# Daniel-Lin-S/decode_tonal_langauge

Hardware: AMD Instinct MI355X
Metric: mel-frames/sec (train step) SynthesisModelCNN, 128ch x 400t batch256 (higher is better)
Workload: dtype f32; 1 GPU; SynthesisModelCNN 128ch x 400t -> 80 mel, 4 tones x 2 syllables, L=5, global batch 256 (strong scaling: 256 windows on rank 0), dropout 0.5, NAdam, 1,376,768,720 params; per_gpu_batch=256, global_batch=256, parallelism=dp1, init=drawn on every rank

## Files before the change

decode_tonal_langauge_amd/_cnn_engine.py:

```python
from __future__ import annotations

import ctypes as C
import os
import math
from typing import Dict, List, Optional

import torch

from . import _kernels, _lib
from ._lib import (EPI_C1WGRAD, EPI_GY, EPI_LRELU, EPI_MASK, EPI_MASKY, EPI_POOL, EPI_POOLV, EPI_STORE, LOAD_DIRECT, LOAD_UNPOOL, LOAD_V,
                   LOAD_Y, NtParams, TnParams, check, ptr)


def _r4(n: int) -> int:
    return (n + 3) // 4 * 4


class _Stage:

    def __init__(self, idx, cin, cout, k, pool, tin, tp_in):
        self.idx, self.cin, self.cout, self.k, self.pool = idx, cin, cout, k, pool
        self.tin, self.tp_in = tin, tp_in
        self.tc = tin - k + 1
        self.tout = self.tc // 2 if pool else self.tc
        self.tp_out = tp_in // 2 if pool else tp_in


class CnnEngine:
    F63_CAPABLE = True

    def __init__(self, output_dim: int, n_channels: int, n_timepoints: int, lstm_channels: int,
                 conv_channels: int, dropout: float, negative_slope: float, stage_defs, concat_widths):
        if negative_slope < 0:
            raise ValueError("the MI355X path needs negative_slope >= 0 (max-pool / LeakyReLU are fused)")
        self.lib = _lib.load()
        self.out_dim = output_dim
        self.C = n_channels
        self.T = n_timepoints
        self.Lc = lstm_channels
        self.Cc = conv_channels
        self.p_drop = float(dropout)
        self.slope = float(negative_slope)
        self.cslope = 0.1
        k1 = stage_defs[0][1]
        npool_after = sum(1 for s in stage_defs[1:] if s[2])
        tc1 = n_timepoints - k1 + 1
        self.k1 = k1
        self.c1 = stage_defs[0][0]
        self.tout1 = tc1 // 2
        if not stage_defs[0][2]:
            raise ValueError("first stage must pool")
        align = 1 << npool_after
        self.tp1 = max(align, (self.tout1 + align - 1) // align * align)
        _kernels.validate()
        self.wino63 = (self.F63_CAPABLE and _kernels.get("wino") == "6"
                       and self._f63_covers(stage_defs, n_timepoints))
        tp1_default = self.tp1
        if self.wino63:
            self.tp1 = (self.tout1 + 11) // 12 * 12
        self.f63_yprod = (self.wino63 and _kernels.get("f63_yprod") != "0" and stage_defs[0][0] % 256 == 0
                          and self.tp1 >= 12)
        self.f63_yprod3 = (self.wino63 and _kernels.get("f63_yprod") != "0" and stage_defs[1][0] % 256 == 0)
        self.stages: List[_Stage] = []
        cin, tin, tp = self.c1, self.tout1, self.tp1
        for i, (cout, k, pool) in enumerate(stage_defs[1:], start=2):
            st = _Stage(i, cin, cout, k, pool, tin, tp)
            if st.tout < 1:
                raise ValueError("n_timepoints too small for the conv stack")
            if self.wino63 and i == 3:
                st.tp_out = tp1_default // 4
            self.stages.append(st)
            cin, tin, tp = cout, st.tout, st.tp_out
        self.gy4 = self._gy_applies()
        self.lat = tin
        self.tp5 = tp
        self.H = self.lat * n_channels * lstm_channels
        self.ld5 = _r4(conv_channels)
        self.ldx = _r4(conv_channels + lstm_channels)
        self.concat_dims = []
        cin_t, cin_ld = conv_channels + lstm_channels, self.ldx
        for w in concat_widths:
            self.concat_dims.append((cin_t, cin_ld, w, _r4(w)))
            cin_t, cin_ld = w, _r4(w)
        self.ldy5 = self.concat_dims[-1][3]
        self.kflat = n_channels * self.tp5 * self.ldy5
        self.ldd = _r4(output_dim)
        self.lowrank_param = "label_lstm.weight_hh_l0"
        self.lstm_shard = None
        self._sh = None
        self.timers = None
        mode = _kernels.get("wino")
        self.wino43 = mode != "0"
        self.store_p1 = _kernels.get("store_p1") == "1"
        self.fuse_c1 = True
        self.wino_vout = True
        self.tn_bm = 0
        self._side = None
        self._B = None
        self.generation = 0
        self._saved_generation = -1

    def _alloc(self, B: int, dev):
        if self._B == B and self._dev == dev:
            return
        self._B, self._dev = B, dev
        S = B * self.C
        self.S = S
        f32 = dict(dtype=torch.float32, device=dev)
        z = lambda *s: torch.zeros(*s, **f32)
        zi = lambda *s: torch.zeros(*s, dtype=torch.int32, device=dev)
        self._v_ready = {}
        self._gy_A = None
        self._vhalo = {}
        self.P = {}
        if not (self.wino63 or self._conv1_writes_v()) or self.store_p1:
            self.P[1] = z(S * self.tp1, self.c1)
        self.bits = {1: zi(S * self.tp1, self.c1 // 32)}
        self.sbits = {1: zi(S * self.tp1, self.c1 // 32)}
        for st in self.stages:
            rows = S * st.tp_out
            ld = st.cout if st.pool else self.ld5
            no_rows = (self.wino63 and st.idx == 2) or (self._writes_v(st) and not self._f63(st))
            if not no_rows or self.store_p1:
                self.P[st.idx] = z(rows, ld)
            if st.pool:
                self.bits[st.idx] = zi(rows, st.cout // 32)
                self.sbits[st.idx] = zi(rows, st.cout // 32)
        rows5 = S * self.tp5
        self.rows5 = rows5
        self.Xc = z(rows5, self.ldx)
        self.Y = [z(rows5, d[3]) for d in self.concat_dims]
        self.out_slab = None
        self.Yt = {}
        self._y_ready = {}
        self.V = {}
        self.Vd = {}
        self._vd_ready = {}
        self.G = None

    def _alloc_bwd(self):
        if self.G is not None:
            return
        dev = self._dev
        f32 = dict(dtype=torch.float32, device=dev)
        z = lambda *s: torch.zeros(*s, **f32)
        S = self.S
        self.G = {}
        if not self.wino63 and not (self.fuse_c1 and self._c1_fusable() and self._v43(self.stages[0])):
            self.G[1] = z(S * self.tp1, self.c1)
        for st in self.stages:
            if not (self.f63_yprod and st.idx == 2) and not (self.gy4 and st.idx == 3):
                self.G[st.idx] = z(S * st.tp_out, st.cout if st.pool else self.ld5)
        self.GY = [z(self.rows5, d[3]) for d in self.concat_dims]
        self.dXc = z(self.rows5, self.ldx)

    def _side_stream(self, dev):
        if self._side is None or self._side.device != dev:
            self._side = torch.cuda.Stream(device=dev)
        return self._side

    def _stream(self):
        return torch.cuda.current_stream().cuda_stream

    def enable_timers(self, on: bool = True):
        self.timers = {} if on else None

    def _tick(self, name):
        if getattr(self, "timers", None) is None or name is None:
            return None
        ev = (torch.cuda.Event(enable_timing=True), torch.cuda.Event(enable_timing=True))
        self.timers.setdefault(name, []).append(ev)
        ev[0].record()
        return ev

    def timer_summary(self):
        torch.cuda.synchronize()
        out = {}
        for k, evs in (self.timers or {}).items():
            ms = [a.elapsed_time(b) for a, b in evs]
            out[k] = (len(ms), sum(ms) / max(len(ms), 1))
        return out

    def _permute(self, src, dst, dims, strides, lims=None, nz=1, zs=0, src_off=0, bias=None):
        d = (C.c_int64 * 4)(*dims)
        s = (C.c_int64 * 4)(*strides)
        l = (C.c_int64 * 4)(*(lims if lims is not None else dims))
        check(self.lib.tl_permute_reduce(src.data_ptr() + 4 * src_off, dst.data_ptr(), d, s, l, nz, zs, ptr(bias),
                                         self._stream()), "tl_permute_reduce")

    def _nt(self, tag=None, fn="tl_gemm_nt_window", **kw):
        p = NtParams()
        p.splitk, p.bm, p.J, p.Tp, p.slope = 1, 128, 1, 1, 0.0
        for k, v in kw.items():
            setattr(p, k, v)
        ev = self._tick(tag)
        check(getattr(self.lib, fn)(C.byref(p), self._stream()), fn)
        if ev:
            ev[1].record()

    def _tn(self, tag=None, fn="tl_gemm_tn_window", **kw):
        p = TnParams()
        p.splitk, p.J, p.Tp, p.Tvalid = 1, 1, 1, 1
        for k, v in kw.items():
            setattr(p, k, v)
        ev = self._tick(tag)
        check(getattr(self.lib, fn)(C.byref(p), self._stream()), fn)
        if ev:
            ev[1].record()

    @staticmethod
    def _splitk(tiles: int, ksteps: int, target: int = 2048) -> int:
        return int(max(1, min(ksteps, (target + tiles - 1) // tiles, 1024)))

    @staticmethod
    def _splitk_rounds(tiles: int, ksteps: int, slots: int = 512, max_sk: int = 32, min_rounds: float = 1.9) -> int:
        cands = []
        for sk in range(1, max(1, min(max_sk, ksteps)) + 1):
            n = tiles * sk
            cands.append((sk, n, n / (-(-n // slots) * slots)))
        full = [c for c in cands if c[2] >= 0.95]
        for sk, n, _ in full:
            if n >= min_rounds * slots:
                return sk
        if full:
            return full[-1][0]
        return max(cands, key=lambda c: c[2])[0]

    def _pack_conv(self, w, cin_ld, flip_for_dgrad):
        O, I, J, _ = w.shape
        if not flip_for_dgrad:
            dst = torch.empty(J, O, cin_ld, dtype=torch.float32, device=w.device)
            self._permute(w, dst, (1, J, O, cin_ld), (0, 1, I * J, J), (1, J, O, I))
            return dst
        old = _r4(O)
        dst = torch.empty(J, cin_ld, old, dtype=torch.float32, device=w.device)
        self._permute(w, dst, (1, J, cin_ld, old), (0, -1, J, I * J), (1, J, I, O), src_off=J - 1)
        return dst


    @staticmethod
    def _f63_covers(stage_defs, T) -> bool:
        if len(stage_defs) < 4:
            return False
        (c1, k1, p1), (c2, k2, p2), (c3, k3, p3) = stage_defs[0], stage_defs[1], stage_defs[2]
        tout1 = (T - k1 + 1) // 2
        tout2 = (tout1 - 2) // 2
        tout3 = (tout2 - 2) // 2
        return (p1 and p2 and p3 and k2 == 3 and k3 == 3 and 1 <= k1 <= 3 and c1 in (128, 256, 512, 1024)
                and c2 % 128 == 0 and c3 % 64 == 0 and tout3 >= 1 and T >= 2 * tout1 + 2)

    def _f63(self, st) -> bool:
        return self.wino63 and st.idx in (2, 3)

    def _nt63_rows(self) -> int:
        return int(self.lib.tl_wino63_nt_tile_rows())

    def _v_hex_buffer(self, store, idx, rows, cin):
        nh = rows // 6
        nh_pad = (nh + 24 + 127) // 128 * 128
        V = store.get(idx)
        if V is None or V.shape[0] != nh_pad or V.shape[1] != 8 or V.shape[2] != cin:
            V = store[idx] = torch.zeros(nh_pad, 8, cin, dtype=torch.float32, device=self._dev)
        return V

    def _pack_wino63(self, w, forward: bool):
        O, I = w.shape[0], w.shape[1]
        dst = torch.empty(8, O, I, dtype=torch.float32, device=w.device) if forward else \
            torch.empty(8, I, O, dtype=torch.float32, device=w.device)
        check(self.lib.tl_wino63_weights(ptr(w), ptr(dst) if forward else None, None if forward else ptr(dst), O, I, I, O,
                                         self._stream()), "tl_wino63_weights")
        return dst

    def f63_issue_factor(self, st) -> float:
        return (st.tp_in // 6) * 8.0 / (st.tc * 3.0)

    def _stage_forward63(self, st, w, bia) -> None:
        S = self.S
        wp = self._pack_wino63(w, True)
        V = self._v_ready[st.idx - 1]
        if st.idx == 2 and self.store_p1 and 2 not in self.P:
            self.P[2] = torch.zeros(S * st.tp_out, st.cout, dtype=torch.float32, device=self._dev)
        Pout = self.P.get(st.idx) if (st.idx != 2 or self.store_p1) else None
        kw = dict(A=ptr(V), A_rows=V.shape[0], lda=V.shape[2], loader=LOAD_V, Bw=ptr(wp), bias=ptr(bia), out=ptr(Pout),
                  M=S * st.tp_in, N=st.cout, K=st.cin, ldb=st.cin, ldo=Pout.shape[1] if Pout is not None else st.cout, J=3,
                  row_shift=0, Tp=st.tp_in, slope=self.slope, obits=ptr(self.bits[st.idx]), osign=ptr(self.sbits[st.idx]),
                  ld_obits=st.cout // 32, Tvalid=2 * st.tout)
        if st.idx == 2:
            rows_out = S * st.tp_out
            Vn = self._v_hex_buffer(self.V, 2, rows_out, st.cout)
            ntm = -(-(S * st.tp_in) // self._nt63_rows())
            if not hasattr(self, "_vhalo"):
                self._vhalo = {}
            halo = self._vhalo.get(2)
            if halo is None or halo.shape[0] != ntm or halo.shape[2] != st.cout:
                halo = self._vhalo[2] = torch.zeros(ntm, 2, st.cout, dtype=torch.float32, device=self._dev)
            kw.update(epilogue=EPI_POOLV, vout=ptr(Vn), vhalo=ptr(halo), vout_quads=Vn.shape[0], ld_vout=Vn.shape[2])
            self._nt(tag="conv2_fwd", fn="tl_conv3_wino63v_nt", **kw)
            check(self.lib.tl_wino63_v_fixup(ptr(Vn), ptr(halo), rows_out // 6, ntm, st.tp_out, st.cout, Vn.shape[2],
                                             self._stream()), "tl_wino63_v_fixup")
            self._v_ready[2] = Vn
        else:
            if Pout is None:
                raise RuntimeError("F(6,3) stage 3 writes pooled rows: its output buffer was not allocated")
            kw.update(epilogue=EPI_POOL, out_tp=st.tp_out)
            self._nt(tag="conv3_fwd", fn="tl_conv3_wino63v_nt", **kw)

    def _stage_wgrad63(self, st, gw, gb) -> None:
        S = self.S
        f32 = dict(dtype=torch.float32, device=self._dev)
        rows_in = S * st.tp_in
        nd = st.cout
        ldg = nd
        V = self._v_ready[st.idx - 1]
        tiles = (st.cin // 64) * (nd // 64)
        sk = self._splitk(tiles, (rows_in + 35) // 36, 4096)
        slab = torch.empty(sk, 8 * st.cin, ldg, **f32)
        bias_part = torch.empty(sk, nd, **f32)
        if (st.idx == 3 and self.f63_yprod3 and self._y_ready.get(3) != self.generation):
            Gs = self.G[3]
            Y3 = self._v_hex_buffer(self.Yt, 3, rows_in, nd)
            Vd3 = self._v_hex_buffer(self.Vd, 3, rows_in, nd)
            ev = self._tick("conv3_yvd")
            check(self.lib.tl_wino63_unpool_yvd(ptr(Gs), ptr(self.bits[3]), ptr(Y3), ptr(Vd3), rows_in, Gs.shape[0], st.tp_in,
                                                st.tp_out, 2 * st.tout, nd, Gs.shape[1], st.cout // 32, nd, self._stream()),
                  "tl_wino63_unpool_yvd")
            if ev:
                ev[1].record()
            self._y_ready[3] = self.generation
            self._vd_ready[3] = self.generation
        if self._y_ready.get(st.idx) == self.generation:
            Y = self.Yt[st.idx]
            self._y_ready[st.idx] = -1
            self._tn(tag=f"conv{st.idx}_wgrad", fn="tl_conv3_wino63v_tn", A=ptr(V), B=ptr(Y), slab=ptr(slab), Krows=rows_in,
                     A_rows=V.shape[0], B_rows=Y.shape[0], Mdim=st.cin, Ndim=nd, lda=V.shape[2], ldb=Y.shape[2], ldc=ldg, J=3,
                     Tp=st.tp_in, splitk=sk, slab_stride=8 * st.cin * ldg, loader=LOAD_Y, Tvalid=2 * st.tout,
                     colsum=ptr(bias_part))
        else:
            Gs = self.G[st.idx]
            Vd = self._v_hex_buffer(self.Vd, st.idx, rows_in, nd)
            self._tn(tag=f"conv{st.idx}_wgrad", fn="tl_conv3_wino63v_tn", A=ptr(V), B=ptr(Gs), slab=ptr(slab), Krows=rows_in,
                     A_rows=V.shape[0], B_rows=Gs.shape[0], Mdim=st.cin, Ndim=nd, lda=V.shape[2], ldb=Gs.shape[1], ldc=ldg, J=3,
                     Tp=st.tp_in, splitk=sk, slab_stride=8 * st.cin * ldg, loader=LOAD_UNPOOL, bbits=ptr(self.bits[st.idx]),
                     ld_bbits=st.cout // 32, Tvalid=2 * st.tout, colsum=ptr(bias_part), vd=ptr(Vd), ld_vd=nd, g_tp=st.tp_out)
            self._vd_ready[st.idx] = self.generation
        if sk > 1:
            red = torch.empty(8 * st.cin, ldg, **f32)
            n = 8 * st.cin * ldg
            self._permute(slab, red, (1, 1, 1, n), (0, 0, 0, 1), nz=sk, zs=n)
        else:
            red = slab
        check(self.lib.tl_wino63_wgrad_finalize(ptr(red), ptr(gw), st.cout, st.cin, ldg, self._stream()),
              "tl_wino63_wgrad_finalize")
        self._permute(bias_part, gb, (1, 1, 1, st.cout), (0, 0, 0, 1), nz=sk, zs=nd)

    def _gy_stage(self, st) -> bool:
        return self.gy4 and st.idx == 4

    def _gy_applies(self) -> bool:
        if not (self.wino63 and self.f63_yprod3 and len(self.stages) >= 3):
            return False
        below, st = self.stages[1], self.stages[2]
        return (_kernels.get("conv4_dgrad") == "nt63" and st.k == 1 and st.pool and self._f63(below)
                and st.cout % 32 == 0 and st.cout >= 40 and st.cin % 32 == 0 and (below.tp_in // 2) % 3 == 0)

    def _stage_dgrad_gy(self, st, w):
        S = self.S
        below = self.stages[1]
        tpg = below.tp_in // 2
        rows = S * tpg
        f32 = dict(dtype=torch.float32, device=self._dev)
        nh = -(-rows // 6)
        nh_pad = (nh + 127) // 128 * 128
        A = getattr(self, "_gy_A", None)
        if A is None or A.shape[0] != nh_pad or A.shape[2] != st.cout:
            A = self._gy_A = torch.zeros(nh_pad, 8, st.cout, **f32)
        Gs = self.G[st.idx]
        ev = self._tick(f"conv{st.idx}_dgrad")
        check(self.lib.tl_wino63_unpool_rows6(ptr(Gs), ptr(self.bits[st.idx]), ptr(A), rows, Gs.shape[0], tpg, st.tp_out,
                                              2 * st.tout, st.cout, Gs.shape[1], st.cout // 32, st.cout, 0, self._stream()),
              "tl_wino63_unpool_rows6")
        taps = torch.empty(st.cout // 8, 8, st.cin, 8, **f32)
        check(self.lib.tl_wino63_weights1(ptr(w), ptr(taps), st.cout, st.cin, st.cout, self._stream()), "tl_wino63_weights1")
        rows3 = S * below.tp_in
        Y3 = self._v_hex_buffer(self.Yt, below.idx, rows3, below.cout)
        Vd3 = self._v_hex_buffer(self.Vd, below.idx, rows3, below.cout)
        ntm = -(-rows // self._nt63_rows())
        if not hasattr(self, "_vhalo"):
            self._vhalo = {}
        halo = self._vhalo.get("d3")
        if halo is None or halo.shape[0] != ntm or halo.shape[2] != below.cout:
            halo = self._vhalo["d3"] = torch.zeros(ntm, 2, below.cout, **f32)
        self._nt(tag=None, fn="tl_conv1_wino63v_dgrad_nt", A=ptr(A), A_rows=A.shape[0], lda=A.shape[2], loader=LOAD_V,
                 Bw=ptr(taps), M=rows, N=st.cin, K=st.cout, ldb=st.cout, ldo=st.cin, J=1, row_shift=0, Tp=tpg, slope=self.slope,
                 auxbits=ptr(self.sbits[below.idx]), ld_auxbits=self.sbits[below.idx].shape[1], abits=ptr(self.bits[below.idx]),
                 ld_abits=below.cout // 32, out_tp=below.tp_out, Tvalid_in=2 * below.tout, epilogue=EPI_GY, out=None,
                 vout=ptr(Y3), vout2=ptr(Vd3), vhalo=ptr(halo), vout_quads=Y3.shape[0], ld_vout=Y3.shape[2])
        check(self.lib.tl_wino63_vd_fixup(ptr(Vd3), ptr(halo), rows // 3, ntm, below.tp_in // 6, below.cout, Vd3.shape[2],
                                          self._stream()), "tl_wino63_vd_fixup")
        if ev:
            ev[1].record()
        self._y_ready[below.idx] = self.generation
        self._vd_ready[below.idx] = self.generation
        return None

    def _stage_dgrad63(self, st, w):
        S = self.S
        rows_in = S * st.tp_in
        if self._vd_ready.get(st.idx) != self.generation:
            raise RuntimeError("F(6,3) input gradient: the stage's weight-gradient pass (which writes Vd) must run first")
        self._vd_ready[st.idx] = -1
        Vd = self.Vd[st.idx]
        wd = self._pack_wino63(w, False)
        kw = dict(A=ptr(Vd), A_rows=Vd.shape[0], lda=Vd.shape[2], loader=LOAD_V, Bw=ptr(wd), M=rows_in, N=st.cin,
                  K=st.cout, ldb=st.cout, ldo=st.cin, J=3, row_shift=-2, Tp=st.tp_in, slope=self.slope,
                  auxbits=ptr(self.sbits[st.idx - 1]), ld_auxbits=self.sbits[st.idx - 1].shape[1])
        if st.idx == 3 and self.f63_yprod:
            below = self.stages[0]
            rows2 = S * below.tp_in
            Y2 = self._v_hex_buffer(self.Yt, 2, rows2, below.cout)
            Vd2 = self._v_hex_buffer(self.Vd, 2, rows2, below.cout)
            ntm = -(-rows_in // self._nt63_rows())
            if not hasattr(self, "_vhalo"):
                self._vhalo = {}
            halo = self._vhalo.get("d2")
            if halo is None or halo.shape[0] != ntm or halo.shape[2] != below.cout:
                halo = self._vhalo["d2"] = torch.zeros(ntm, 2, below.cout, dtype=torch.float32, device=self._dev)
            self._nt(tag="conv3_dgrad", fn="tl_conv3_wino63v_nt", epilogue=EPI_MASKY, out=None, vout=ptr(Y2), vout2=ptr(Vd2),
                     vhalo=ptr(halo), vout_quads=Y2.shape[0], ld_vout=Y2.shape[2], abits=ptr(self.bits[2]),
                     ld_abits=below.cout // 32, Tvalid_in=2 * below.tout, **kw)
            check(self.lib.tl_wino63_vd_fixup(ptr(Vd2), ptr(halo), rows_in // 3, ntm, below.tp_in // 6, below.cout, Vd2.shape[2],
                                              self._stream()), "tl_wino63_vd_fixup")
            self._y_ready[2] = self.generation
            self._vd_ready[2] = self.generation
            return None
        if st.idx == 3:
            self._nt(tag="conv3_dgrad", fn="tl_conv3_wino63v_nt", epilogue=EPI_MASK, out=ptr(self.G[2]), **kw)
            return None
        ntm = -(-rows_in // self._nt63_rows())
        part = torch.empty(ntm, (self.k1 + 1) * self.c1, dtype=torch.float32, device=self._dev)
        self._nt(tag="conv2_dgrad", fn="tl_conv3_wino63v_nt", epilogue=EPI_C1WGRAD, out=None, c1x=ptr(self._x),
                 c1bits=ptr(self.bits[1]), c1partial=ptr(part), c1T=self.T, c1kt=self.k1, Tvalid=self.tout1, **kw)
        return part

    def _c1_fusable(self) -> bool:
        return self.k1 <= 3 and self.T >= 2 * self.tout1 + 2

    def _v43(self, st) -> bool:
        return (self.wino43 and st.k == 3 and st.pool and st.cin % 64 == 0 and st.cout % 32 == 0 and st.tp_in % 4 == 0
                and _r4(st.cout) % 16 == 0)

    def _tn_bm(self, st) -> int:
        wide = st.cin % 128 == 0
        dma8 = wide and _r4(st.cout) % 64 == 0 and (st.cout // 32) % 2 == 0
        if self.tn_bm == 127:
            return 127 if wide else 64
        if self.tn_bm in (0, 128):
            return 128 if dma8 else 64
        return 64

    def _conv1_writes_v(self) -> bool:
        return (self._v43(self.stages[0]) and self.tp1 % 4 == 0 and self.c1 in (128, 256, 512, 1024)
                and (self.fuse_c1 and self._c1_fusable()))

    def _writes_v(self, st) -> bool:
        if not (self.wino_vout and st.pool and st.idx - 1 < len(self.stages)):
            return False
        nxt = self.stages[st.idx - 1]
        return self._v43(st) and self._v43(nxt) and st.tp_in % 8 == 0 and nxt.cin == st.cout

    def _pin(self, st):
        return self.P.get(st.idx - 1)

    def _v_buffer(self, idx, rows, cin):
        nq = rows // 4
        nq_pad = (nq + 127) // 128 * 128
        V = self.V.get(idx)
        if V is None or V.shape[0] != nq_pad or V.shape[2] != cin:
            V = self.V[idx] = torch.zeros(nq_pad, 6, cin, dtype=torch.float32, device=self._dev)
        return V

    def _input_transform(self, st):
        src = self.P[st.idx - 1]
        V = self._v_buffer(st.idx - 1, src.shape[0], st.cin)
        ev = self._tick(f"conv{st.idx}_xform")
        check(self.lib.tl_wino43_input_transform(ptr(src), ptr(V), src.shape[0], st.tp_in, st.cin, src.shape[1], st.cin,
                                                 self._stream()), "tl_wino43_input_transform")
        if ev:
            ev[1].record()
        return V

    def wgrad_issue_factor(self, st) -> float:
        if self._f63(st):
            return self.f63_issue_factor(st)
        return 0.5 if self._v43(st) else 1.0

    def kernel_families(self):
        if self.wino63:
            self._fam_share = {}
            st2, st3 = self.stages[0], self.stages[1]
            f6 = "Winograd F(6,3) on pre-transformed operands, LDS-DMA"
            tn = "wino63v_tn4_kernel<true>" if st3.cin % 256 == 0 and st3.tp_in >= 12 else "wino63v_tn_kernel<true>"
            tn2 = "wino63v_tn4_kernel<true>" if st2.cin % 256 == 0 else "wino63v_tn_kernel<true>"
            fams = {f"wino63v_nt_kernel<POOLV> (conv2 forward, {f6}; writes V of its pooled output for conv3)": ["conv2_fwd"],
                    f"wino63v_nt_kernel<POOL> (conv3 forward, {f6})": ["conv3_fwd"],
                    f"wino63v_nt_kernel<C1WGRAD> (conv2 input gradient + conv1 weight gradient, {f6})": ["conv2_dgrad"],
                    }
            if self.f63_yprod3:
                gy = self.gy4
                src = "the epilogue of conv4's input gradient" if gy else "wino63_unpool_yvd_kernel"
                fams[f"wino63v_tn4y_kernel (conv3 weight gradient, {f6}: both operands by LDS-DMA, no transform in the kernel; Y3 / Vd3 "
                     f"from {src})"] = ["conv3_wgrad"]
            else:
                fams[f"{tn} (conv3 weight gradient, {f6}; also writes Vd)"] = ["conv3_wgrad"]
            if self.f63_yprod:
                fams[f"wino63v_nt_kernel<MASKY> (conv3 input gradient, {f6}; writes Y and Vd of conv2 instead of the gradient rows)"] = ["conv3_dgrad"]
                fams[f"wino63v_tn4y_kernel (conv2 weight gradient, {f6}: both operands by LDS-DMA, no transform in the kernel)"] = ["conv2_wgrad"]
            else:
                fams[f"wino63v_nt_kernel<MASK> (conv3 input gradient, {f6})"] = ["conv3_dgrad"]
                fams[f"{tn2} (conv2 weight gradient, {f6}; also writes Vd)"] = ["conv2_wgrad"]
            issued = {k: self.f63_issue_factor(st2 if "conv2" in k else st3) for k in fams}
            return fams, issued
        self._fam_share = {}
        if not all(self._v43(st) for st in self.stages[:2]):
            fams = {"nt_window_kernel<128,UNPOOL,MASK> (conv input-gradient)": ["conv2_dgrad", "conv3_dgrad", "conv4_dgrad"],
                    "nt_window_kernel<128,DIRECT,POOL> (conv forward)": ["conv2_fwd", "conv3_fwd", "conv4_fwd"],
                    "tn3_kernel<UNPOOL> (conv weight-gradient)": ["conv2_wgrad", "conv3_wgrad"]}
            return fams, {k: 1.0 for k in fams}
        form = "Winograd F(4,3) on pre-transformed operands, LDS-DMA"
        fused = self.fuse_c1 and self._c1_fusable()
        bm = self._tn_bm(self.stages[0])
        extra = {}
        if bm == 128:
            tn = f"wino43v_tn8_kernel<true> (conv2/conv3 weight gradient, {form}; also writes Vd for the input gradient)"
        else:
            ntm = (self.stages[0].cin + 63) // 64
            tn = f"wino43v_tn_kernel<false, 2> (conv2/conv3 weight gradient, C_in tiles 1..{ntm - 1} of {ntm}, {form})"
            vdn = f"wino43v_tn_kernel<true, 2> (conv2/conv3 weight gradient, C_in tile 0 of {ntm}, {form}, + writes Vd for the input gradient)"
            extra[vdn] = ["conv2_wgrad_vd", "conv3_wgrad_vd"]
            self._fam_share = {tn: (ntm - 1) / ntm, vdn: 1.0 / ntm}
        fams = {tn: ["conv2_wgrad", "conv3_wgrad"]}
        if self._writes_v(self.stages[0]):
            fams[f"wino43v_nt_kernel<POOLV> (conv2 forward, {form}; writes V of its pooled output for conv3 instead of the raw rows)"] = ["conv2_fwd"]
            fams[f"wino43v_nt_kernel<POOL> (conv3 forward, {form})"] = ["conv3_fwd"]
        else:
            fams[f"wino43v_nt_kernel<POOL> (conv2/conv3 forward, {form})"] = ["conv2_fwd", "conv3_fwd"]
        fams.update(extra)
        if fused:
            fams[f"wino43v_nt_kernel<UNPOOL,C1WGRAD> (conv2 input gradient + conv1 weight gradient, {form})"] = ["conv2_dgrad"]
            fams[f"wino43v_nt_kernel<UNPOOL,MASK> (conv3 input gradient, {form})"] = ["conv3_dgrad"]
        else:
            fams[f"wino43v_nt_kernel<UNPOOL,MASK> (conv2/conv3 input gradient, {form})"] = ["conv2_dgrad", "conv3_dgrad"]
        return fams, {k: 0.5 for k in fams}

    def _pack_wino43(self, w, forward: bool):
        O, I = w.shape[0], w.shape[1]
        dst = torch.empty(6, O, I, dtype=torch.float32, device=w.device) if forward else \
            torch.empty(6, I, O, dtype=torch.float32, device=w.device)
        check(self.lib.tl_wino43_weights(ptr(w), ptr(dst) if forward else None, None if forward else ptr(dst), O, I, I, O,
                                         self._stream()), "tl_wino43_weights")
        return dst

    STAGE_NAMES = {2: "ecog_conv_block.3", 3: "ecog_conv_block.6", 4: "ecog_conv_block.9", 5: "ecog_conv_block.12"}

    def stage_forward(self, st: _Stage, w: torch.Tensor, bia: torch.Tensor) -> None:
        if self._f63(st):
            return self._stage_forward63(st, w, bia)
        S = self.S
        v43 = self._v43(st)
        wp = self._pack_wino43(w, True) if v43 else self._pack_conv(w, st.cin, False)
        src = self._pin(st)
        vout = self._writes_v(st)
        if vout and self.store_p1 and st.idx not in self.P:
            self.P[st.idx] = torch.zeros(S * st.tp_out, st.cout, dtype=torch.float32, device=self._dev)
        Pout = self.P.get(st.idx) if (not vout or self.store_p1) else None
        kw = dict(A=ptr(src), Bw=ptr(wp), bias=ptr(bia), out=ptr(Pout), M=S * st.tp_in,
                  A_rows=S * st.tp_in, N=st.cout, K=st.cin, lda=st.cin, ldb=st.cin,
                  ldo=Pout.shape[1] if Pout is not None else st.cout, J=st.k, row_shift=0, Tp=st.tp_in, slope=self.slope,
                  loader=LOAD_DIRECT)
        if st.pool:
            kw.update(epilogue=EPI_POOL, obits=ptr(self.bits[st.idx]), osign=ptr(self.sbits[st.idx]),
                      ld_obits=st.cout // 32, Tvalid=2 * st.tout)
        else:
            kw.update(epilogue=EPI_LRELU, Tvalid=st.tout)
        if not v43:
            self._nt(tag=f"conv{st.idx}_fwd", fn="tl_gemm_nt_window", **kw)
            return
        V = self._v_ready.get(st.idx - 1)
        if V is None:
            V = self._v_ready[st.idx - 1] = self._input_transform(st)
        kw.update(A=ptr(V), A_rows=V.shape[0], lda=V.shape[2], loader=LOAD_V)
        if vout:
            rows_out = S * st.tp_out
            Vn = self._v_buffer(st.idx, rows_out, st.cout)
            ntm = (S * st.tp_in + 511) // 512
            halo = self._vhalo.get(st.idx)
            if halo is None or halo.shape[0] != ntm or halo.shape[2] != st.cout:
                halo = self._vhalo[st.idx] = torch.zeros(ntm, 2, st.cout, dtype=torch.float32, device=self._dev)
# ... 22 lines not shown
            flat = part.view(-1)
            for c0 in range(0, zs, 1024):
                nc = min(1024, zs - c0)
                self._colsum(flat[c0:], nblk, nc, zs, 1, 1, red[c0:c0 + nc])
            self._permute(red, gw, (1, 1, self.c1, self.k1), (0, 0, 1, self.c1))
            self._permute(red, gb, (1, 1, 1, self.c1), (0, 0, 0, 1), src_off=self.k1 * self.c1)
        else:
            self._permute(part, gw, (1, 1, self.c1, self.k1), (0, 0, 1, self.c1), nz=nblk, zs=zs)
            self._permute(part, gb, (1, 1, 1, self.c1), (0, 0, 0, 1), nz=nblk, zs=zs, src_off=self.k1 * self.c1)

    def stage_wgrad(self, st: _Stage, gw: torch.Tensor, gb: torch.Tensor) -> None:
        if self._f63(st):
            return self._stage_wgrad63(st, gw, gb)
        S = self.S
        f32 = dict(dtype=torch.float32, device=self._dev)
        Xin = self._pin(st)
        Gs = self.G[st.idx]
        rows_in = S * st.tp_in
        ldg = Gs.shape[1]
        nd = _r4(st.cout)
        if self._v43(st):
            tiles = ((st.cin + 63) // 64) * ((nd + 63) // 64)
            bm = self._tn_bm(st)
            sk = self._splitk(tiles, (rows_in + 31) // 32, 4096 if bm in (127, 128) else 8192)
            slab = torch.empty(sk, 6 * st.cin, ldg, **f32)
            bias_part = torch.empty(sk, nd, **f32)
            V = self._v_ready.get(st.idx - 1)
            if V is None:
                V = self._v_ready[st.idx - 1] = self._input_transform(st)
            nq_pad = (rows_in // 4 + 127) // 128 * 128
            Vd = self.Vd.get(st.idx)
            if Vd is None or Vd.shape[0] != nq_pad or Vd.shape[2] != nd:
                Vd = self.Vd[st.idx] = torch.zeros(nq_pad, 6, nd, **f32)
            kw = dict(A=ptr(V), B=ptr(Gs), slab=ptr(slab), Krows=rows_in, A_rows=V.shape[0], B_rows=Gs.shape[0],
                      Mdim=st.cin, Ndim=nd, lda=V.shape[2], ldb=ldg, ldc=ldg, J=3, Tp=st.tp_in, splitk=sk,
                      slab_stride=6 * st.cin * ldg, loader=LOAD_UNPOOL, bbits=ptr(self.bits[st.idx]),
                      ld_bbits=st.cout // 32, Tvalid=2 * st.tout, colsum=ptr(bias_part), bm=bm, vd=ptr(Vd), ld_vd=nd)
            self._vd_ready[st.idx] = self.generation
            if self.timers is not None and bm != 128:
                self._tn(tag=f"conv{st.idx}_wgrad_vd", fn="tl_conv3_wino43v_tn", part=1, **kw)
                self._tn(tag=f"conv{st.idx}_wgrad", fn="tl_conv3_wino43v_tn", part=2, **kw)
            else:
                self._tn(tag=f"conv{st.idx}_wgrad", fn="tl_conv3_wino43v_tn", **kw)
            if sk > 1:
                red = torch.empty(6 * st.cin, ldg, **f32)
                n = 6 * st.cin * ldg
                self._permute(slab, red, (1, 1, 1, n), (0, 0, 0, 1), nz=sk, zs=n)
            else:
                red = slab
            check(self.lib.tl_wino43_wgrad_finalize(ptr(red), ptr(gw), st.cout, st.cin, ldg, self._stream()),
                  "tl_wino43_wgrad_finalize")
            self._permute(bias_part, gb, (1, 1, 1, st.cout), (0, 0, 0, 1), nz=sk, zs=nd)
            return
        if st.k == 3:
            tiles = ((st.cin + 127) // 128) * ((nd + 63) // 64)
        else:
            tiles = st.k * ((st.cin + 127) // 128) * ((nd + 127) // 128)
        sk = self._splitk(tiles, (rows_in + 31) // 32, 1024)
        slab = torch.empty(sk, st.k * st.cin, ldg, **f32)
        kw = dict(A=ptr(Xin), B=ptr(Gs), slab=ptr(slab), Krows=rows_in, A_rows=Xin.shape[0], B_rows=Gs.shape[0],
                  Mdim=st.cin, Ndim=nd, lda=st.cin, ldb=ldg, ldc=ldg, J=st.k, Tp=st.tp_in, splitk=sk,
                  slab_stride=st.k * st.cin * ldg)
        if st.pool:
            kw.update(loader=LOAD_UNPOOL, bbits=ptr(self.bits[st.idx]), ld_bbits=st.cout // 32, Tvalid=2 * st.tout)
        else:
            kw.update(loader=LOAD_DIRECT, Tvalid=st.tout)
        fold = (not st.pool) and st.k == 1 and rows_in > 512 and st.cin > 32
        bpart = torch.empty(sk, nd, **f32) if fold else None
        if fold:
            kw.update(colsum=ptr(bpart))
        self._tn(tag=f"conv{st.idx}_wgrad", **kw)
        if sk > 1:
            red = torch.empty(st.k * st.cin, ldg, **f32)
            n = st.k * st.cin * ldg
            self._permute(slab, red, (1, 1, 1, n), (0, 0, 0, 1), nz=sk, zs=n)
        else:
            red = slab
        self._permute(red, gw, (1, st.cout, st.cin, st.k), (0, 1, ldg, st.cin * ldg))
        if fold:
            self._permute(bpart, gb, (1, 1, 1, st.cout), (0, 0, 0, 1), nz=sk, zs=nd)
        else:
            self._colsum(Gs, Gs.shape[0], st.cout, ldg, st.tp_out, st.tout, gb)

    def stage_dgrad(self, st: _Stage, w: torch.Tensor):
        if self._f63(st):
            return self._stage_dgrad63(st, w)
        if self._gy_stage(st):
            return self._stage_dgrad_gy(st, w)
        S = self.S
        Xin = self._pin(st)
        Gs = self.G[st.idx]
        rows_in = S * st.tp_in
        ldg = Gs.shape[1]
        v43 = self._v43(st)
        wd = self._pack_wino43(w, False) if v43 else self._pack_conv(w, st.cin, True)
        kd = wd.shape[2]
        fuse = st.idx == 2 and v43 and self.fuse_c1 and self._c1_fusable()
        kw = dict(A=ptr(Gs), Bw=ptr(wd), aux=ptr(Xin), out=None if fuse else ptr(self.G[st.idx - 1]), M=rows_in,
                  A_rows=Gs.shape[0], N=st.cin, K=kd, lda=ldg, ldb=kd, ldo=st.cin, ldaux=st.cin, J=st.k,
                  row_shift=-(st.k - 1), Tp=st.tp_in, epilogue=EPI_MASK, slope=self.slope)
        if (st.idx - 1) in self.sbits:
            kw.update(auxbits=ptr(self.sbits[st.idx - 1]), ld_auxbits=self.sbits[st.idx - 1].shape[1])
        if st.pool:
            kw.update(loader=LOAD_UNPOOL, abits=ptr(self.bits[st.idx]), ld_abits=st.cout // 32,
                      Tvalid_in=2 * st.tout)
        else:
            kw.update(loader=LOAD_DIRECT)
        if not v43:
            self._nt(tag=f"conv{st.idx}_dgrad", fn="tl_gemm_nt_window", **kw)
            return None
        part = None
        if fuse:
            ntm = (rows_in + 511) // 512
            part = torch.empty(ntm, (self.k1 + 1) * self.c1, dtype=torch.float32, device=self._dev)
            kw.update(epilogue=EPI_C1WGRAD, out=None, c1x=ptr(self._x), c1bits=ptr(self.bits[1]), c1partial=ptr(part),
                      c1T=self.T, c1kt=self.k1, Tvalid=self.tout1)
        if self._vd_ready.get(st.idx) != self.generation or st.idx not in self.Vd:
            raise RuntimeError("F(4,3) input gradient: the stage's weight-gradient pass (which writes Vd) must run first")
        Vd = self.Vd[st.idx]
        kw.update(A=ptr(Vd), A_rows=Vd.shape[0], lda=Vd.shape[2], loader=LOAD_V)
        self._vd_ready[st.idx] = -1
        self._nt(tag=f"conv{st.idx}_dgrad", fn="tl_conv3_wino43v_nt", **kw)
        return part

    def _lstm_forward(self, prm, xu, U, L, dev, training, label_table) -> None:
        lib, st_ = self.lib, self._stream()
        H = self.H
        f32 = dict(dtype=torch.float32, device=dev)
        self._act = torch.empty(L, U, 4 * H, **f32)
        self._c = torch.empty(L, U, H, **f32)
        self._h = torch.empty(L, U, H, **f32)
        hh = torch.empty(U, 4 * H, **f32) if L > 1 else None
        w_ih, w_hh = prm["label_lstm.weight_ih_l0"], prm["label_lstm.weight_hh_l0"]
        b_ih, b_hh = prm["label_lstm.bias_ih_l0"], prm["label_lstm.bias_hh_l0"]
        bm = 32 if U <= 64 else 128
        self._sh = None
        if (self.lstm_shard is not None and label_table is not None and training and L > 1 and (L - 1) * U <= 64
                and (4 * H) % (4 * self.lstm_shard[1]) == 0):
            rk, wd = self.lstm_shard
            self._sh = (rk * (4 * H // wd), 4 * H // wd, wd)
        nloc = self._sh[1] if self._sh else 4 * H
        sk_f = self._splitk_rounds(((U + bm - 1) // bm) * ((nloc + 127) // 128), (H + 31) // 32, min_rounds=8.9) if L > 1 else 1
        slab_f = torch.empty(sk_f, U, nloc, **f32) if sk_f > 1 else None
        if self._sh:
            from . import parallel
            hh_loc = torch.empty(U, nloc, **f32)
            hh_all = torch.empty(self._sh[2], U, nloc, **f32)
        for t in range(L):
            if t > 0 and self._sh:
                r0, R, wd = self._sh
                self._nt(A=ptr(self._h[t - 1]), Bw=w_hh.data_ptr() + 4 * r0 * H, out=ptr(slab_f if sk_f > 1 else hh_loc),
                         M=U, A_rows=U, N=R, K=H, lda=H, ldb=H, ldo=R, loader=LOAD_DIRECT, epilogue=EPI_STORE, bm=bm,
                         splitk=sk_f, slab_stride=U * R)
                if sk_f > 1:
                    self._permute(slab_f, hh_loc, (1, 1, 1, U * R), (0, 0, 0, 1), nz=sk_f, zs=U * R)
                parallel.all_gather_blocks(hh_all, hh_loc)
                self._permute(hh_all, hh, (1, U, wd, R), (0, R, U * R, 1))
            elif t > 0:
                self._nt(A=ptr(self._h[t - 1]), Bw=ptr(w_hh), out=ptr(slab_f if sk_f > 1 else hh), M=U, A_rows=U,
                         N=4 * H, K=H, lda=H, ldb=H, ldo=4 * H, loader=LOAD_DIRECT, epilogue=EPI_STORE, bm=bm,
                         splitk=sk_f, slab_stride=U * 4 * H)
                if sk_f > 1:
                    n = U * 4 * H
                    self._permute(slab_f, hh, (1, 1, 1, n), (0, 0, 0, 1), nz=sk_f, zs=n)
            check(lib.tl_lstm_cell_fwd(ptr(hh) if t > 0 else None, ptr(xu[t]), ptr(w_ih), ptr(b_ih), ptr(b_hh),
                                       ptr(self._c[t - 1]) if t > 0 else None, ptr(self._act[t]), ptr(self._c[t]),
                                       ptr(self._h[t]), U, H, 2, 4 * H, st_), "tl_lstm_cell_fwd")

    def forward(self, prm: Dict[str, torch.Tensor], x: torch.Tensor, labels: torch.Tensor, training: bool,
# ... 212 lines not shown
        for i in range(len(self.concat_dims) - 1, -1, -1):
            order += [f"concat_conv_block.{2 * i}.weight", f"concat_conv_block.{2 * i}.bias"]
        order += ["label_lstm.weight_ih_l0", "label_lstm.bias_ih_l0", "label_lstm.bias_hh_l0"]
        for st in reversed(self.stages):
            order += [self.STAGE_NAMES[st.idx] + ".weight", self.STAGE_NAMES[st.idx] + ".bias"]
        order += ["ecog_conv_block.0.weight", "ecog_conv_block.0.bias"]
        return order

    def backward(self, prm: Dict[str, torch.Tensor], dout: torch.Tensor, grads: Dict[str, torch.Tensor],
                 gather_whh=None, whh_factors: bool = False, reduce_rows=None, on_factors=None, on_grad_ready=None) -> None:
        self.whh_factors = None
        if self._saved_generation != self.generation:
            raise RuntimeError("SynthesisModelCNN backward: the forward intermediates were overwritten by a later "
                               "forward pass (one forward/backward pair at a time per model)")
        self._alloc_bwd()
        lib, st_ = self.lib, self._stream()
        B, S, dev = self._B, self.S, self._dev
        f32 = dict(dtype=torch.float32, device=dev)
        H, U, L = self.H, self._U, self._L
        rows5 = self.rows5

        colsum = self._colsum

        gw = grads["output_layer.weight"]
        slab = torch.empty(self.ldd, self.kflat, **f32)
        self._tn(A=ptr(dout), B=ptr(self.Y[-1]), slab=ptr(slab), Krows=B, A_rows=B, B_rows=B, Mdim=self.ldd,
                 Ndim=self.kflat, lda=self.ldd, ldb=self.kflat, ldc=self.kflat, loader=LOAD_DIRECT)
        latC = self.lat * self.C
        self._permute(slab, gw, (self.out_dim, self.Cc, self.lat, self.C),
                      (self.kflat, 1, self.ldy5, self.tp5 * self.ldy5))
        colsum(dout, B, self.out_dim, self.ldd, 1, 1, grads["output_layer.bias"])
        if on_grad_ready is not None:
            on_grad_ready("output_layer")
        wpt = torch.empty(self.kflat, self.ldd, **f32)
        self._permute(prm["output_layer.weight"], wpt, (self.C, self.tp5, self.ldy5, self.ldd),
                      (1, self.C, latC, self.Cc * latC), (self.C, self.lat, self.Cc, self.out_dim))
        self._nt(A=ptr(dout), Bw=ptr(wpt), aux=ptr(self.Y[-1]), out=ptr(self.GY[-1]), M=B, A_rows=B, N=self.kflat,
                 K=self.ldd, lda=self.ldd, ldb=self.ldd, ldo=self.kflat, ldaux=self.kflat, loader=LOAD_DIRECT,
                 epilogue=EPI_MASK, slope=self.cslope)
        del wpt
        for i in range(len(self.concat_dims) - 1, -1, -1):
            cin_t, cin_ld, cout_t, cout_ld = self.concat_dims[i]
            src = self.Xc if i == 0 else self.Y[i - 1]
            Gi = self.GY[i]
            name = f"concat_conv_block.{2 * i}"
            tiles = ((cin_ld + 127) // 128) * ((cout_ld + 127) // 128)
            sk = self._splitk(tiles, (rows5 + 31) // 32, 512)
            slab = torch.empty(sk, cin_ld, cout_ld, **f32)
            fold = rows5 > 512 and cin_ld > 32
            bpart = torch.empty(sk, cout_ld, **f32) if fold else None
            self._tn(A=ptr(src), B=ptr(Gi), slab=ptr(slab), Krows=rows5, A_rows=rows5, B_rows=rows5, Mdim=cin_ld,
                     Ndim=cout_ld, lda=cin_ld, ldb=cout_ld, ldc=cout_ld, loader=LOAD_DIRECT, Tp=self.tp5,
                     Tvalid=self.lat, splitk=sk, slab_stride=cin_ld * cout_ld, colsum=ptr(bpart))
            self._permute(slab, grads[name + ".weight"], (1, 1, cout_t, cin_t), (0, 0, 1, cout_ld), nz=sk,
                          zs=cin_ld * cout_ld)
            if fold:
                self._permute(bpart, grads[name + ".bias"], (1, 1, 1, cout_t), (0, 0, 0, 1), nz=sk, zs=cout_ld)
            else:
                colsum(Gi, rows5, cout_t, cout_ld, self.tp5, self.lat, grads[name + ".bias"])
            wd = self._pack_conv(prm[name + ".weight"], cin_ld, True)
            if i > 0:
                self._nt(A=ptr(Gi), Bw=ptr(wd), aux=ptr(src), out=ptr(self.GY[i - 1]), M=rows5, A_rows=rows5,
                         N=cin_ld, K=cout_ld, lda=cout_ld, ldb=cout_ld, ldo=cin_ld, ldaux=cin_ld, loader=LOAD_DIRECT,
                         epilogue=EPI_MASK, slope=self.cslope)
            else:
                self._nt(A=ptr(Gi), Bw=ptr(wd), out=ptr(self.dXc), M=rows5, A_rows=rows5, N=cin_ld, K=cout_ld,
                         lda=cout_ld, ldb=cout_ld, ldo=cin_ld, loader=LOAD_DIRECT, epilogue=EPI_STORE)
        dh_ext = torch.empty(U, H, **f32)
        check(lib.tl_concat_unpack_bwd(ptr(self.dXc), ptr(self.P[5]), None, ptr(self._uid), ptr(self.G[5]),
                                       ptr(dh_ext), B, U, self.C, self.tp5, self.lat, self.Cc, self.Lc, self.ld5, H,
                                       self.ldx, self.slope, self._p_drop_used, self._seed_used, self._drop_row0,
                                       st_), "tl_concat_unpack_bwd")
        side = None
        if side is not None:
            dh_ext.record_stream(side)
            side.wait_stream(torch.cuda.current_stream())
            with torch.cuda.stream(side):
                self._lstm_backward(prm, grads, dh_ext, gather_whh, whh_factors, reduce_rows, on_factors)
        else:
            self._lstm_backward(prm, grads, dh_ext, gather_whh, whh_factors, reduce_rows, on_factors)
        for st in reversed(self.stages):
            name = self.STAGE_NAMES[st.idx]
            self.stage_wgrad(st, grads[name + ".weight"], grads[name + ".bias"])
            part = self.stage_dgrad(st, prm[name + ".weight"])
        if part is None:
            nblk = int(min(2048, S))
            part = torch.empty(nblk, (self.k1 + 1) * self.c1, **f32)
            check(lib.tl_conv1_wgrad(ptr(self._x), ptr(self.G[1]), ptr(self.bits[1]), ptr(part), nblk, S, self.T, self.k1,
                                     self.c1, self.tp1, self.tout1, st_), "tl_conv1_wgrad")
        self._reduce_c1_partials(part, grads["ecog_conv_block.0.weight"], grads["ecog_conv_block.0.bias"])
        if side is not None:
            torch.cuda.current_stream().wait_stream(side)
```

decode_tonal_langauge_amd/_kernels.py:

```python
from __future__ import annotations

import os
from typing import Callable, Dict, Tuple, Union

_Allowed = Union[frozenset, Callable[[str], bool]]


def _int(lo: int, hi: int) -> Callable[[str], bool]:
    def ok(v: str) -> bool:
        try:
            return lo <= int(v) <= hi
        except ValueError:
            return False
    return ok


_B = frozenset({"0", "1"})
KEYS: Dict[str, Tuple[str, _Allowed, str, str]] = {
    "wino": ("TONAL_WINO", frozenset({"6", "4", "0"}), "6",
             "conv2 / conv3: 6 Winograd F(6,3) on pre-transformed operands (F(4,3) V form where the stack does not allow it), "
             "4 the F(4,3) V form, 0 direct MFMA kernels (also the fallback for every shape neither form covers)"),
    "f63_yprod": ("TONAL_F63_YPROD", _B, "1", "F(6,3): the backward operands Y / Vd of stages 2 and 3 come pre-transformed out of the "
                                              "input-gradient epilogue of the stage above (0: the weight-gradient kernels un-pool and "
                                              "transform the gradient rows themselves)"),
    "conv4_dgrad": ("TONAL_CONV4_DGRAD", frozenset({"nt63", "gemm"}), "nt63",
                    "F(6,3): the one-tap stage behind conv3 - nt63: its input gradient on the NT63 kernel, writing Y3 / Vd3 "
                    "(no gradient rows, no tl_wino63_unpool_yvd); gemm: one-tap GEMM + tl_wino63_unpool_yvd"),
    "store_p1": ("TONAL_STORE_P1", _B, "0", "keep the raw pooled rows of stages 1 / 2 beside V (tests)"),
    "conv7": ("TONAL_CONV7", frozenset({"wino63", "direct"}), "wino63", "the CNN-RNN classifier's 7-tap convolutions"),
    "whh_dh": ("TONAL_WHH_DH", _B, "1", "single process: the W_hh NAdam pass also produces the last BPTT product dh_1 = dgates_2 . W_hh "
                                        "(0: a W_hh stream of its own for it)"),
    "whh_stream": ("TONAL_WHH_STREAM", _B, "1", "label LSTM backward: dgates . W_hh as a pure stream of the weight (tl_lstm_gw; 0: the skinny "
                                                "MFMA GEMM with split-K slabs, also the form for more than 8 distinct label rows)"),
    "graph": ("TONAL_GRAPH", _B, "1", "SynthesisLite step replayed as a HIP graph"),
    "lstm_shard": ("TONAL_LSTM_SHARD", _B, "1", "data parallel: label LSTM sharded by gate rows"),
    "hilbert": ("TONAL_HILBERT", frozenset({"auto", "ols", "ols_full", "sym", "taps", "fft"}), "auto",
                "Hilbert bank: force a path (ols band-limited overlap-save, ols_full all 1024 bins per band, sym / taps the "
                "time-domain kernels with / without Hermitian symmetry, fft the DFT-domain form)"),
    "hilbert_f32": ("TONAL_HILBERT_F32", _B, "0", "float32 recordings: fp32 transforms end to end (default: fp64 math)"),
    "butter": ("TONAL_BUTTER", frozenset({"seq", "scan"}), "seq",
               "zero-phase Butterworth: seq the sequential recurrence (bit-identical to scipy's loop), scan the time-parallel "
               "block scan (2e-8 - 5e-8 from it: the size of the reference's own rounding; ~20 x faster)"),
}
_LEGACY = {v[0]: k for k, v in KEYS.items()}
_cache: Tuple[str, Dict[str, str]] = ("", {})


def _check(key: str, value: str) -> str:
    allowed = KEYS[key][1]
    ok = allowed(value) if callable(allowed) else value in allowed
    if not ok:
        what = "an integer in range" if callable(allowed) else "one of " + ", ".join(sorted(allowed))
        raise ValueError(f"TONAL_KERNELS: {key}={value!r} is not a value this switch takes ({what})")
    return value


def _parsed() -> Dict[str, str]:
    global _cache
    raw = os.environ.get("TONAL_KERNELS", "")
    if raw == _cache[0]:
        return _cache[1]
    out: Dict[str, str] = {}
    for item in raw.split(","):
        item = item.strip()
        if not item:
            continue
        key, sep, value = item.partition("=")
        key, value = key.strip(), value.strip()
        if not sep or key not in KEYS:
            raise ValueError(f"TONAL_KERNELS: unknown setting {item!r}; keys: " + ", ".join(sorted(KEYS)))
        out[key] = _check(key, value)
    _cache = (raw, out)
    return out


def get(key: str, default: str = None) -> str:
    legacy, _allowed, table_default, _doc = KEYS[key]
    spec = _parsed()
    if key in spec:
        return spec[key]
    if legacy in os.environ:
        if os.environ.get("TONAL_AB") != "1":
            raise RuntimeError(f"{legacy} is an A/B switch of the test suite and is ignored by the product: use "
                               f"TONAL_KERNELS={key}={os.environ[legacy]} (or set TONAL_AB=1 to run an A/B comparison)")
        return _check(key, os.environ[legacy])
    return table_default if default is None else default


def validate() -> None:
    _parsed()
    if os.environ.get("TONAL_AB") != "1":
        for legacy, key in _LEGACY.items():
            if legacy in os.environ:
                get(key)
```

decode_tonal_langauge_amd/_lib.py:

```python
from __future__ import annotations

import ctypes as C
import os
from typing import Optional

_HERE = os.path.dirname(os.path.abspath(__file__))
LIB_PATH = os.environ.get("TONAL_HIP_LIB", os.path.join(_HERE, "libtonal_hip.so"))

LOAD_DIRECT, LOAD_UNPOOL, LOAD_V = 0, 1, 2
EPI_STORE, EPI_LRELU, EPI_POOL, EPI_MASK, EPI_C1WGRAD, EPI_POOLV, EPI_MASKY, EPI_GY = 0, 1, 2, 3, 4, 5, 6, 7
LOAD_Y = 3


class NtParams(C.Structure):
    _fields_ = [
        ("A", C.c_void_p), ("abits", C.c_void_p), ("Bw", C.c_void_p), ("bias", C.c_void_p), ("aux", C.c_void_p),
        ("out", C.c_void_p), ("obits", C.c_void_p),
        ("M", C.c_int64), ("A_rows", C.c_int64),
        ("N", C.c_int), ("K", C.c_int),
        ("lda", C.c_int), ("ldb", C.c_int), ("ldo", C.c_int), ("ldaux", C.c_int), ("ld_abits", C.c_int),
        ("ld_obits", C.c_int),
        ("J", C.c_int), ("row_shift", C.c_int),
        ("Tp", C.c_int), ("Tvalid", C.c_int), ("Tvalid_in", C.c_int),
        ("slope", C.c_float),
        ("loader", C.c_int), ("epilogue", C.c_int),
        ("splitk", C.c_int), ("slab_stride", C.c_int64),
        ("bm", C.c_int),
        ("osign", C.c_void_p), ("auxbits", C.c_void_p), ("ld_auxbits", C.c_int),
        ("c1x", C.c_void_p), ("c1bits", C.c_void_p), ("c1partial", C.c_void_p), ("c1T", C.c_int), ("c1kt", C.c_int),
        ("vout", C.c_void_p), ("vhalo", C.c_void_p), ("vout_quads", C.c_int64), ("ld_vout", C.c_int),
        ("out_tp", C.c_int), ("vout2", C.c_void_p),
    ]


class TnParams(C.Structure):
    _fields_ = [
        ("A", C.c_void_p), ("B", C.c_void_p), ("bbits", C.c_void_p), ("slab", C.c_void_p),
        ("Krows", C.c_int64), ("A_rows", C.c_int64), ("B_rows", C.c_int64),
        ("Mdim", C.c_int), ("Ndim", C.c_int),
        ("lda", C.c_int), ("ldb", C.c_int), ("ldc", C.c_int), ("ld_bbits", C.c_int),
        ("J", C.c_int), ("Tp", C.c_int), ("Tvalid", C.c_int), ("loader", C.c_int),
        ("splitk", C.c_int), ("slab_stride", C.c_int64),
        ("colsum", C.c_void_p),
        ("vd", C.c_void_p), ("ld_vd", C.c_int), ("part", C.c_int), ("bm", C.c_int), ("g_tp", C.c_int),
    ]


_P = C.c_void_p
_I = C.c_int
_L = C.c_int64
_F = C.c_float

SIGNATURES = {
    "tl_last_error": (C.c_char_p, []),
    "tl_version": (_I, []),
    "tl_device_count": (_I, []),
    "tl_gemm_nt_window": (_I, [C.POINTER(NtParams), _P]),
    "tl_gemm_tn_window": (_I, [C.POINTER(TnParams), _P]),
    "tl_wino43_weights": (_I, [_P, _P, _P, _I, _I, _I, _I, _P]),
    "tl_wino63_xform2": (_I, [_P, _P, _P, _L, _I, _I, _I, _I, _I, _P]),
    "tl_wino63_weights7": (_I, [_P, _P, _I, _I, _I, _P]),
    "tl_conv7_wino63v_nt": (_I, [C.POINTER(NtParams), _P]),
    "tl_wino63_unpool_rows6": (_I, [_P, _P, _P, _L, _L, _I, _I, _I, _I, _I, _I, _I, _I, _P]),
    "tl_wino63_weights1": (_I, [_P, _P, _I, _I, _I, _P]),
    "tl_conv1_wino63v_dgrad_nt": (_I, [C.POINTER(NtParams), _P]),
    "tl_comm_unique_id": (_I, [_P]),
    "tl_comm_init": (_I, [C.POINTER(C.c_void_p), _I, _I, _P]),
    "tl_comm_destroy": (_I, [_P]),
    "tl_allreduce": (_I, [_P, _P, _P, _L, _I, _P]),
    "tl_reduce_scatter": (_I, [_P, _P, _P, _L, _P]),
    "tl_all_gather": (_I, [_P, _P, _P, _L, _P]),
    "tl_wino43_wgrad_finalize": (_I, [_P, _P, _I, _I, _I, _P]),
    "tl_wino43_input_transform": (_I, [_P, _P, _L, _I, _I, _I, _I, _P]),
    "tl_conv3_wino43v_nt": (_I, [C.POINTER(NtParams), _P]),
    "tl_wino43_v_fixup": (_I, [_P, _P, _L, _L, _I, _I, _I, _P]),
    "tl_wino43_unpool_transform": (_I, [_P, _P, _P, _L, _L, _I, _I, _I, _I, _I, _I, _P]),
    "tl_conv3_wino43v_tn": (_I, [C.POINTER(TnParams), _P]),
    "tl_wino63_weights": (_I, [_P, _P, _P, _I, _I, _I, _I, _P]),
    "tl_conv3_wino63v_nt": (_I, [C.POINTER(NtParams), _P]),
    "tl_wino63_nt_tile_rows": (_I, []),
    "tl_wino63_v_fixup": (_I, [_P, _P, _L, _L, _I, _I, _I, _P]),
    "tl_conv3_wino63v_tn": (_I, [C.POINTER(TnParams), _P]),
    "tl_wino63_wgrad_finalize": (_I, [_P, _P, _I, _I, _I, _P]),
    "tl_wino63_vd_fixup": (_I, [_P, _P, _L, _L, _I, _I, _I, _P]),
    "tl_wino63_unpool_yvd": (_I, [_P, _P, _P, _P, _L, _L, _I, _I, _I, _I, _I, _I, _I, _P]),
    "tl_conv1_fwd_v6": (_I, [_P, _P, _P, _P, _P, _P, _P, _L, _I, _I, _I, _I, _I, _F, _P]),
    "tl_sizeof_nt_params": (_I, []),
    "tl_sizeof_tn_params": (_I, []),
    "tl_conv1_fwd": (_I, [_P, _P, _P, _P, _P, _P, _L, _I, _I, _I, _I, _I, _F, _P]),
    "tl_conv1_fwd_v": (_I, [_P, _P, _P, _P, _P, _P, _P, _L, _I, _I, _I, _I, _I, _F, _P]),
    "tl_dropout_scale": (_I, [_P, _L, _F, C.c_uint64, _P]),
    "tl_conv1_wgrad": (_I, [_P, _P, _P, _P, _I, _L, _I, _I, _I, _I, _I, _P]),
    "tl_permute_reduce": (_I, [_P, _P, C.POINTER(_L), C.POINTER(_L), C.POINTER(_L), _I, _L, _P, _P]),
    "tl_colsum": (_I, [_P, _P, _I, _L, _I, _I, _I, _I, _P]),
    "tl_lstm_cell_fwd": (_I, [_P, _P, _P, _P, _P, _P, _P, _P, _P, _I, _I, _I, _I, _P]),
    "tl_lstm_gw": (_I, [_P, _P, _P, _I, _L, _I, _L, _L, _I, _P]),
    "tl_lstm_infer_seq_fused": (_I, [_P, _L, _P, _P, _P, _P, _I, _I, _I, C.POINTER(C.c_int), _P]),
    "tl_lstm_cell_bwd": (_I, [_P, _P, _P, _P, _P, _P, _P, _P, _P, _I, _I, _I, _P]),
    "tl_lstm_ih_grad": (_I, [_P, _P, _P, _P, _P, _I, _I, _I, _I, _P]),
    "tl_concat_pack": (_I, [_P, _P, _P, _P, _I, _I, _I, _I, _I, _I, _I, _I, _I, _F, C.c_uint64, _L, _P]),
    "tl_concat_unpack_bwd": (_I, [_P, _P, _P, _P, _P, _P, _I, _I, _I, _I, _I, _I, _I, _I, _I, _I, _F, _F,
                                  C.c_uint64, _L, _P]),
    "tl_l1_mcd": (_I, [_P, _P, _P, _P, _I, _I, _I, _I, _F, _P]),
    "tl_nadam": (_I, [_P, _P, _P, _P, _L, _F, _F, _F, _F, _F, _F, _F, _F, _P]),
    "tl_nadam_multi": (_I, [_P, _I, _L, _F, _F, _F, _F, _F, _F, _F, _F, _P]),
    "tl_nadam_multi_chunk": (_I, []),
    "tl_sum_slabs2": (_I, [_P, _P, _L, _P, _P, _L, _I, _P]),
    "tl_set_step_scalars": (_I, [_P, _P, _F, _F, _F, C.c_uint64, _P]),
    "tl_stage_step": (_I, [_P, _P, _F, _F, _F, C.c_uint64, _P, _P, _P, _I, _P]),
    "tl_nadam_multi_dev": (_I, [_P, _I, _L, _P, _F, _F, _F, _F, _F, _P]),
    "tl_nadam_lowrank": (_I, [_P, _P, _P, _P, _P, _I, _I, _I, _I, _I, _F, _F, _F, _F, _F, _F, _F, _F, _P]),
    "tl_nadam_lowrank_dh": (_I, [_P, _P, _P, _P, _P, _I, _I, _I, _I, _I, _F, _F, _F, _F, _F, _F, _F, _F, _P, _I, _I, _P]),
    "tl_tone_dynamics": (_I, [_P, _P, _P, _P, _P, _I, _I, _I, _P]),
    "tl_splitk_bias_lrelu": (_I, [_P, _P, _P, _I, _L, _I, _F, _P]),
    "tl_labels_from_scores": (_I, [_P, _P, _P, _P, _P, _P, _P, _P, _I, _I, _I, _I, _I, _I, _P]),
    "tl_lite_conv_fwd": (_I, [_P, _P, _P, _P, _P, _I, _I, _I, _I, _I, _I, _P]),
    "tl_lite_bn_finalize": (_I, [_P, _P, _P, _P, _P, _I, _I, _L, _I, _F, _F, _I, _P, _P]),
    "tl_lite_bn_act_pool_fwd": (_I, [_P, _P, _P, _P, _P, _P, _I, _I, _I, _F, _P]),
    "tl_lite_bn_act_pool_bwd": (_I, [_P, _P, _P, _P, _P, _P, _P, _P, _P, _P, _I, _I, _I, _F, _I, _P]),
    "tl_lite_conv_bwd": (_I, [_P, _P, _P, _P, _P, _P, _I, _I, _I, _I, _I, _I, _P]),
    "tl_lite_lstm_fwd": (_I, [_P, _P, _P, _P, _P, _P, _P, _P, _I, _I, _I, _I, _P]),
    "tl_lite_lstm_bwd": (_I, [_P, _P, _P, _P, _P, _I, _I, _I, _I, _P]),
    "tl_lite_cat": (_I, [_P, _P, _P, _I, _I, _I, _I, _I, _F, C.c_uint64, _P]),
    "tl_lite_uncat": (_I, [_P, _P, _P, _I, _I, _I, _I, _F, C.c_uint64, _P]),
    "tl_lite_cat_dev": (_I, [_P, _P, _P, _I, _I, _I, _I, _I, _F, _P, _P]),
    "tl_lite_uncat_dev": (_I, [_P, _P, _P, _I, _I, _I, _I, _F, _P, _P]),
    "tl_row_zscore": (_I, [_P, _I, _P, _P, _I, _L, _L, _L, _I, _P]),
    "tl_car": (_I, [_P, _I, _P, _P, _I, _L, _I, _P]),
    "tl_rolling_zscore": (_I, [_P, _I, _P, _I, _L, _I, _I, _P]),
    "tl_fft_resample": (_I, [_P, _I, _P, _I, _L, _L, _P, _P, _P, _I, _P, _P, _P, _I, _P, _P]),
    "tl_gauss_envelope": (_I, [_P, _I, _P, _P, _I, _L, _I, _I, _I, _I, _P]),
    "tl_gauss_envelope_sym": (_I, [_P, _I, _P, _P, _I, _L, _I, _I, _I, _P]),
    "tl_linear_rows": (_I, [_P, _P, _P, _P, _I, _I, _I, _L, _I, _P]),
    "tl_hilbert_ols": (_I, [_P, _I, _P, _P, _P, _I, _L, _I, _I, _I, _I, _P]),
    "tl_hilbert_ols_bl": (_I, [_P, _I, _P, _P, _P, _P, _I, _L, _I, _I, _I, _I, _P]),
    "tl_hilbert_fft": (_I, [_P, _I, _P, _I, _L, _P, _I, _P, _P, _P, _I, _I, _P, _P]),
    "tl_filtfilt_f64": (_I, [_P, _I, _P, _P, _P, _P, _P, _I, _L, _I, _P]),
    "tl_filtfilt_scan_f64": (_I, [_P, _I, _P, _P, _P, _P, _I, _P, _P, _P, _I, _L, _I, _I, _P]),
    "tl_sosfilt_f64": (_I, [_P, _I, _P, _P, _I, _L, _I, _P]),
    "tl_fir_bank": (_I, [_P, _I, _P, _P, _I, _I, _L, _I, _I, _P]),
    "tl_fir_bank_ols": (_I, [_P, _I, _P, _P, _P, _I, _I, _L, _I, _I, _P]),
}

_lib: Optional[C.CDLL] = None


def load() -> C.CDLL:
    global _lib
    if _lib is not None:
        return _lib
    import torch
    if not os.path.exists(LIB_PATH):
        raise RuntimeError(
            f"{LIB_PATH} not found: build it with `python -c 'import __graft_entry__ as g; g.build()'` "
            "(or `make -C decode_tonal_langauge_amd/csrc`). This package has no CPU fallback.")
    lib = C.CDLL(LIB_PATH)
    for name, (res, args) in SIGNATURES.items():
        fn = getattr(lib, name)
        fn.restype = res
        fn.argtypes = args
    if lib.tl_sizeof_nt_params() != C.sizeof(NtParams) or lib.tl_sizeof_tn_params() != C.sizeof(TnParams):
# ... 26 lines not shown
```

decode_tonal_langauge_amd/csrc/tonal_wino43_epi.h:

```cpp
#pragma once
#include "tonal_common.h"

namespace tl {

enum { W_LOAD_DIRECT = 0, W_LOAD_UNPOOL = 1, W_LOAD_V = 2 };
enum { W_EPI_LRELU = 1, W_EPI_POOL = 2, W_EPI_MASK = 3, W_EPI_C1W = 4, W_EPI_POOLV = 5, W_EPI_MASKY = 6, W_EPI_GY = 7 };

struct c1w_acc {
  float s[3], b;
  __device__ __forceinline__ void clear() { s[0] = s[1] = s[2] = b = 0.f; }
};
struct c1w_cursor {
  long long wofs, xo;
  int t;
  __device__ __forceinline__ void init(const tl_nt_params& p, long long R, int colbase) {
    const long long seq = R / p.Tp;
    t = (int)(R - seq * p.Tp);
    wofs = R * (long long)p.ld_auxbits + (colbase >> 5);
    xo = seq * (long long)p.c1T + 2 * t;
  }
  __device__ __forceinline__ void advance(const tl_nt_params& p, int rows) {
    t += rows;
    wofs += (long long)rows * p.ld_auxbits;
    xo += 2 * rows;
    while (t >= p.Tp) {
      t -= p.Tp;
      xo += p.c1T - 2 * p.Tp;
    }
  }
};
__device__ __forceinline__ void c1w_row(c1w_acc& a, const tl_nt_params& p, const c1w_cursor& c, int h, float y, int lr) {
  const long long w = c.wofs + (long long)h * p.ld_auxbits;
  const bool pos = (p.auxbits[w] >> lr) & 1u;
  const bool am = (p.c1bits[w] >> lr) & 1u;
  const float* xp = p.c1x + c.xo + 2 * h;
  const float x0 = xp[0], x1 = xp[1], x2 = xp[2], x3 = xp[3];
  const float dz = pos ? y : y * p.slope;
  a.s[0] = fmaf(dz, am ? x1 : x0, a.s[0]);
  if (p.c1kt > 1) a.s[1] = fmaf(dz, am ? x2 : x1, a.s[1]);
  if (p.c1kt > 2) a.s[2] = fmaf(dz, am ? x3 : x2, a.s[2]);
  a.b += dz;
}
__device__ __forceinline__ void c1w_row_vals(c1w_acc& a, const tl_nt_params& p, uint32_t sword, uint32_t cword, float x0,
                                             float x1, float x2, float x3, float y, int lr) {
  const bool pos = (sword >> lr) & 1u;
  const bool am = (cword >> lr) & 1u;
  const float dz = pos ? y : y * p.slope;
  a.s[0] = fmaf(dz, am ? x1 : x0, a.s[0]);
  if (p.c1kt > 1) a.s[1] = fmaf(dz, am ? x2 : x1, a.s[1]);
  if (p.c1kt > 2) a.s[2] = fmaf(dz, am ? x3 : x2, a.s[2]);
  a.b += dz;
}
template <int NWM, int NCOL>
__device__ __forceinline__ void c1w_reduce_store(const tl_nt_params& p, float* red, const c1w_acc& a, int wm, int cl,
                                                 int lh, long long tile, int col, bool colok) {
  float v[4] = {a.s[0], a.s[1], a.s[2], a.b};
#pragma unroll
  for (int j = 0; j < 4; ++j) v[j] += __shfl_xor(v[j], 32);
  if (lh == 0) {
#pragma unroll
    for (int j = 0; j < 4; ++j) red[(wm * NCOL + cl) * 4 + j] = v[j];
  }
  __syncthreads();
  if (wm == 0 && lh == 0 && colok) {
#pragma unroll
    for (int j = 0; j < 4; ++j) {
      float t = 0.f;
#pragma unroll
      for (int w = 0; w < NWM; ++w) t += red[(w * NCOL + cl) * 4 + j];
      v[j] = t;
    }
    float* dst = p.c1partial + tile * (long long)(p.c1kt + 1) * p.N;
    for (int j = 0; j < p.c1kt; ++j) dst[(long long)j * p.N + col] = v[j];
    dst[(long long)p.c1kt * p.N + col] = v[3];
  }
  __syncthreads();
}


template <int EPI, bool FULL = false>
__device__ __forceinline__ void wino43_epilogue(const tl_nt_params& p, const f32x16 (&acc)[6], float* lds, long long R0,
                                                int n0, int wm, int wn, int lr, int lh, long long tm) {
  const long long Q0 = (R0 >> 2) + wm * 32 + 4 * lh;
  const int col = n0 + wn * 32 + lr;
  const int colbase = n0 + wn * 32;
  const bool colok = FULL || col < p.N;
  float bv = 0.f;
  if constexpr (EPI == W_EPI_POOL || EPI == W_EPI_LRELU) bv = (colok && p.bias) ? p.bias[col] : 0.f;
  uint32_t wbits = 0, wsign = 0;
// ... 115 lines not shown
```

decode_tonal_langauge_amd/csrc/tonal_wino63.hip:

```cpp
#include "tonal_common.h"
#include "tonal_wino43_epi.h"
#include "tonal_wino43v_epi.h"
#include "tonal_wino63_epi.h"
#include "tonal_wino63_kloop.h"
#include <type_traits>

namespace tl {

typedef __attribute__((address_space(3))) void lds_void6_t;
__device__ __forceinline__ void dma16h(__amdgpu_buffer_rsrc_t rs, char* lds_dst, unsigned voff, unsigned soff) {
  __builtin_amdgcn_raw_ptr_buffer_load_lds(rs, (lds_void6_t*)lds_dst, 16, voff, soff, 0, 0);
}

typedef int v6_i32x4 __attribute__((ext_vector_type(4)));
__device__ __forceinline__ v6_i32x4 v6_rsrc_words(const void* base, long long bytes) {
  const unsigned long long a = (unsigned long long)base;
  const long long n = bytes < 0 ? 0 : (bytes < 0x7fffffffLL ? bytes : 0x7fffffffLL);
  return v6_i32x4{(int)(unsigned)a, (int)(unsigned)((a >> 32) & 0xffffu), (int)n, 0x00020000};
}

__device__ __forceinline__ long long v6_at(long long hex, int i, int c, int kc8) {
  return ((((hex >> 1) * kc8 + (c >> 3)) * 8 + i) * 2 + (hex & 1)) * 8 + (c & 7);
}

__global__ void wino63_weights_kernel(const float* __restrict__ w, float* __restrict__ fwd, float* __restrict__ dgr, int O,
                                      int I, int ld_f, int ld_d) {
  const long long n_f = (long long)O * ld_f, n_d = (long long)I * ld_d;
  const long long idx = (long long)blockIdx.x * blockDim.x + threadIdx.x;
  auto emit = [](float* dst, int R, int r, int k, float g0, float g1, float g2) {
    float* d0 = dst + (((long long)(k >> 3) * 8) * R + r) * 8 + (k & 7);
    const long long n = (long long)R * 8;
    const float s = g0 + g2;
    d0[0] = -g0;
    d0[n] = (-2.f / 9.f) * (s + g1);
    d0[2 * n] = (-2.f / 9.f) * (s - g1);
    const float a = fmaf(4.f, g2, g0), b = 2.f * g1;
    d0[3 * n] = (1.f / 90.f) * (a + b);
    d0[4 * n] = (1.f / 90.f) * (a - b);
    const float c = fmaf(4.f, g0, g2), d = 2.f * g1;
    d0[5 * n] = (8.f / 45.f) * (c + d);
    d0[6 * n] = (8.f / 45.f) * (c - d);
    d0[7 * n] = g2;
  };
  if (fwd != nullptr && idx < n_f) {
    const int o = (int)(idx / ld_f), i = (int)(idx % ld_f);
    float g0 = 0.f, g1 = 0.f, g2 = 0.f;
    if (i < I) {
      const float* s = w + ((long long)o * I + i) * 3;
      g0 = s[0], g1 = s[1], g2 = s[2];
    }
    emit(fwd, O, o, i, g0, g1, g2);
  }
  if (dgr != nullptr && idx < n_d) {
    const int i = (int)(idx / ld_d), o = (int)(idx % ld_d);
    float g0 = 0.f, g1 = 0.f, g2 = 0.f;
    if (o < O) {
      const float* s = w + ((long long)o * I + i) * 3;
      g0 = s[2], g1 = s[1], g2 = s[0];
    }
    emit(dgr, I, i, o, g0, g1, g2);
  }
}

__global__ void wino63_wgrad_finalize_kernel(const float* __restrict__ red, float* __restrict__ gw, int O, int I, int ld) {
  const long long idx = (long long)blockIdx.x * blockDim.x + threadIdx.x;
  if (idx >= (long long)O * I) return;
  const int i = (int)(idx / O), o = (int)(idx % O);
  const long long plane = (long long)I * ld;
  const float* s = red + (long long)i * ld + o;
  float m[8];
#pragma unroll
  for (int t = 0; t < 8; ++t) m[t] = s[t * plane];
  const float a12 = m[1] + m[2], s12 = m[1] - m[2], a34 = m[3] + m[4], s34 = m[3] - m[4], a56 = m[5] + m[6], s56 = m[5] - m[6];
  float* d = gw + ((long long)o * I + i) * 3;
  d[0] = -m[0] - (2.f / 9.f) * a12 + (1.f / 90.f) * a34 + (32.f / 45.f) * a56;
  d[1] = -(2.f / 9.f) * s12 + (1.f / 45.f) * s34 + (16.f / 45.f) * s56;
  d[2] = -(2.f / 9.f) * a12 + (2.f / 45.f) * a34 + (8.f / 45.f) * a56 + m[7];
}

__global__ void wino63_weights7_kernel(const float* __restrict__ w, float* __restrict__ fwd, int O, int I, int taps) {
  const long long idx = (long long)blockIdx.x * blockDim.x + threadIdx.x;
  if (idx >= 3LL * O * I) return;
  const int k = (int)(idx % (3LL * I)), o = (int)(idx / (3LL * I));
  const int seg = k / I, i = k - seg * I;
  const float* s = w + ((long long)o * I + i) * taps + 3 * seg;
  const float g0 = 3 * seg < taps ? s[0] : 0.f, g1 = 3 * seg + 1 < taps ? s[1] : 0.f, g2 = 3 * seg + 2 < taps ? s[2] : 0.f;
  float* d0 = fwd + (((long long)(k >> 3) * 8) * O + o) * 8 + (k & 7);
  const long long n = (long long)O * 8;
  const float sm = g0 + g2;
  d0[0] = -g0;
  d0[n] = (-2.f / 9.f) * (sm + g1);
  d0[2 * n] = (-2.f / 9.f) * (sm - g1);
  const float a = fmaf(4.f, g2, g0), b = 2.f * g1;
  d0[3 * n] = (1.f / 90.f) * (a + b);
  d0[4 * n] = (1.f / 90.f) * (a - b);
  const float c = fmaf(4.f, g0, g2), d = 2.f * g1;
  d0[5 * n] = (8.f / 45.f) * (c + d);
  d0[6 * n] = (8.f / 45.f) * (c - d);
  d0[7 * n] = g2;
}

__global__ __launch_bounds__(256, 4) void wino63_xform2_kernel(const float* __restrict__ P, float* __restrict__ V0, float* __restrict__ V1,
                                                             long long nhex, int hps, int Tp, int Tvalid, int C, int ldp, int ldv) {
  const int tpp = C >> 1;
  const long long idx = (long long)blockIdx.x * blockDim.x + threadIdx.x;
  const long long pair = idx / tpp;
  const int tl_ = (int)(idx - pair * tpp);
  const int half = tl_ & 1, hpar = (tl_ >> 1) & 1, kc = tl_ >> 2;
  const int c = 8 * kc + 4 * half;
  const long long hg = 2 * pair + hpar;
  if (hg >= nhex) return;
  const long long seq = hg / hps;
  const int hs = (int)(hg - seq * hps);
  const float* src = P + (seq * Tp + 6LL * hs) * (long long)ldp + c;
  f32x4 d[11];
#pragma unroll
  for (int j = 0; j < 11; ++j) {
    d[j] = f32x4{0.f, 0.f, 0.f, 0.f};
    if (6 * hs + j < Tvalid) d[j] = *reinterpret_cast<const f32x4*>(src + (long long)j * ldp);
  }
  f32x4 o0[8], o1[8];
#pragma unroll
  for (int k = 0; k < 4; ++k) {
    float a[8], b[8], va[8], vb[8];
#pragma unroll
    for (int j = 0; j < 8; ++j) {
      a[j] = d[j][k];
      b[j] = d[j + 3][k];
    }
    wino63_bt(a, va);
    wino63_bt(b, vb);
#pragma unroll
    for (int j = 0; j < 8; ++j) {
      o0[j][k] = va[j];
      o1[j][k] = vb[j];
    }
  }
  const long long at = v6_at(hg, 0, c, ldv >> 3);
#pragma unroll
  for (int j = 0; j < 8; ++j) *reinterpret_cast<f32x4*>(V0 + at + 16 * j) = o0[j];
#pragma unroll
  for (int j = 0; j < 8; ++j) *reinterpret_cast<f32x4*>(V1 + at + 16 * j) = o1[j];
}

__global__ __launch_bounds__(256, 4) void wino63_v_fixup_kernel(float* __restrict__ V, const float* __restrict__ halo, long long hexes,
                                                              long long tiles, int Tq, int C, int ldv) {
  const int c4n = C >> 2;
  const long long idx = (long long)blockIdx.x * blockDim.x + threadIdx.x;
  if (idx >= tiles * c4n) return;
  const long long t = idx / c4n;
  const int c = (int)(idx - t * c4n) * 4;
  const long long q = t * 64 + 63;
  if (q >= hexes) return;
  float* v = V + v6_at(q, 0, c, ldv >> 3);
  f32x4 d[8];
#pragma unroll
  for (int j = 0; j < 6; ++j) d[j] = *reinterpret_cast<const f32x4*>(v + 16 * j);
  const int tq = (int)((6 * q) % Tq);
  if (tq + 6 < Tq && t + 1 < tiles) {
    d[6] = *reinterpret_cast<const f32x4*>(halo + ((t + 1) * 2) * (long long)C + c);
    d[7] = *reinterpret_cast<const f32x4*>(halo + ((t + 1) * 2 + 1) * (long long)C + c);
  } else {
    d[6] = d[7] = f32x4{0.f, 0.f, 0.f, 0.f};
  }
  f32x4 o[8];
#pragma unroll
  for (int k = 0; k < 4; ++k) {
    float dd[8], vv[8];
#pragma unroll
    for (int j = 0; j < 8; ++j) dd[j] = d[j][k];
    wino63_bt(dd, vv);
#pragma unroll
    for (int j = 0; j < 8; ++j) o[j][k] = vv[j];
  }
#pragma unroll
  for (int j = 0; j < 8; ++j) *reinterpret_cast<f32x4*>(v + 16 * j) = o[j];
}

constexpr int V6_BH = 128, V6_BN = 64, V6_BK = 8;
constexpr int V6_ROWB = V6_BK * 4;
constexpr int V6_A_BYTES = 8 * V6_BH * V6_ROWB;
constexpr int V6_B_BYTES = 8 * V6_BN * V6_ROWB;
constexpr int V6_STAGE = V6_A_BYTES + V6_B_BYTES;
constexpr int V6_ROWS = 6 * V6_BH;
#ifndef V6_PRIO
#define V6_PRIO 0
#endif
#ifndef V6_RDSCHED
#define V6_RDSCHED -1
#endif
#ifndef V6_ABL
#define V6_ABL 0
#endif
#ifndef V6_STAMP
#define V6_STAMP 0
#endif
#if V6_STAMP
constexpr int V6_STAMP_TILES = 96, V6_STAMP_SLOTS = 16;
__device__ unsigned long long v6_stamp_buf[256 * V6_STAMP_TILES * V6_STAMP_SLOTS];
#define V6_STAMP_AT(k)                                                                                                         \
  do {                                                                                                                         \
    if (tid == 0 && stamp_tile < V6_STAMP_TILES && blockIdx.x < 256)                                                           \
      v6_stamp_buf[((long long)blockIdx.x * V6_STAMP_TILES + stamp_tile) * V6_STAMP_SLOTS + (k)] =                             \
          ((k) == 0 || (k) == 7) ? __builtin_amdgcn_s_memrealtime() : __builtin_amdgcn_s_memtime();                           \
  } while (0)
#else
#define V6_STAMP_AT(k) do { } while (0)
#endif

#ifndef V6_GY_SIX
#define V6_GY_SIX 1
#endif
template <int EPI>
__global__ __launch_bounds__(512, 2) void wino63v_nt_kernel(const tl_nt_params p) {
  __shared__ __attribute__((aligned(1024))) char lds[3 * V6_STAGE + ((EPI == W_EPI_POOLV || EPI == W_EPI_MASKY || EPI == W_EPI_GY) ? 4096 : EPI == W_EPI_C1W ? 16384 : 0)];
  const int tid = threadIdx.x;
  const int lane = tid & 63;
  const int wave = __builtin_amdgcn_readfirstlane(tid >> 6);
  const int wm = wave >> 1, wn = wave & 1;
  const int lr = lane & 31, lh = lane >> 5;

#if V6_PRIO
  if (wave >= 4) __builtin_amdgcn_s_setprio(1);
#endif
  const int ntn = (p.N + V6_BN - 1) / V6_BN;
  const long long ntm = (p.M + V6_ROWS - 1) / V6_ROWS;
  const long long nwg = ntm * ntn;
  constexpr bool SEG3 = EPI == W_EPI_LRELU;
  constexpr bool SIX = EPI == W_EPI_GY && V6_GY_SIX;
  const int kseg = p.K / V6_BK;
  const int nsteps = SEG3 ? 3 * kseg : kseg;
  f32x16 acc[8];
  f32x4 faL[4], fbL[4], faH[4], fbH[4];

  const int prow = lane >> 1;
  const int src_chunk = (lane & 1) ^ ((lane >> 4) & 1);
  const v6_i32x4 rsB = v6_rsrc_words(p.Bw, (SIX && wave >= 6) ? 0 : 8LL * p.N * p.ldb * 4);
  const unsigned lds0 = (unsigned)(unsigned long long)(lds_void6_t*)lds;
  const unsigned dst_a0 = lds0 + (unsigned)(wave * V6_BH * V6_ROWB);
  const unsigned dst_b0 = lds0 + (unsigned)(V6_A_BYTES + wave * V6_BN * V6_ROWB);
  const int hex_of_row = (prow & 3) | ((prow >> 3) << 2) | (((prow >> 2) & 1) << 4);
  const int kc8 = p.lda >> 3;
  unsigned avoff[4], bv_lane[2];
#pragma unroll
  for (int t = 0; t < 4; ++t) avoff[t] = (unsigned)(v6_at(t * 32 + hex_of_row, wave, src_chunk * 4, kc8) * 4);
  unsigned avoff1[4];
#pragma unroll
  for (int t = 0; t < 4; ++t) avoff1[t] = SEG3 ? (unsigned)(v6_at(t * 32 + hex_of_row + 1, wave, src_chunk * 4, kc8) * 4) : avoff[t];
#pragma unroll
  for (int t = 0; t < 2; ++t) bv_lane[t] = (unsigned)((((long long)wave * p.N + t * 32 + prow) * 8 + src_chunk * 4) * 4);
  const unsigned b_step = (unsigned)p.N * 256u;

  struct tile_t {
    long long tm, R0;
    int n0;
    v6_i32x4 rsA, rsA1;
    unsigned bvoff[2];
  };
  const long long a_tile_bytes = (long long)V6_BH * 8 * p.lda * 4, a_total_bytes = p.A_rows * 8LL * p.lda * 4;
  auto place = [&](tile_t& t, long long tm, int tn) {
    t.tm = tm;
    t.R0 = tm * V6_ROWS;
    t.n0 = tn * V6_BN;
    const long long ab = tm * a_tile_bytes;
    t.rsA = v6_rsrc_words(reinterpret_cast<const char*>(p.A) + ab, (SIX && wave >= 6) ? 0 : a_total_bytes - ab);
    t.rsA1 = SEG3 ? v6_rsrc_words(reinterpret_cast<const char*>(p.aux) + ab, a_total_bytes - ab) : t.rsA;
    if (t.n0 + V6_BN <= p.N) {
      const unsigned nb4 = (unsigned)t.n0 * 32u;
#pragma unroll
      for (int k = 0; k < 2; ++k) t.bvoff[k] = bv_lane[k] + nb4;
    } else {
#pragma unroll
      for (int k = 0; k < 2; ++k) {
        int n = t.n0 + k * 32 + prow;
        if (n > p.N - 1) n = p.N - 1;
        t.bvoff[k] = (unsigned)((((long long)wave * p.N + n) * 8 + src_chunk * 4) * 4);
      }
    }
  };
  tile_t cur;
  {
    long long bid = blockIdx.x;
    const long long q = nwg / 8, r = nwg % 8, x = bid % 8, i = bid / 8;
    bid = (x < r ? x * (q + 1) : r * (q + 1) + (x - r) * q) + i;
    place(cur, bid / ntn, (int)(bid % ntn));
  }
  const int walk = (int)(gridDim.x >> 3), walk_q = walk / ntn, walk_r = walk - walk_q * ntn;
  auto advance = [&](const tile_t& c) -> tile_t {
    tile_t t = c;
    int tn = c.n0 / V6_BN + walk_r;
    long long tm = c.tm + walk_q;
    if (tn >= ntn) {
      tn -= ntn;
      ++tm;
    }
    place(t, tm, tn);
    return t;
  };
  auto next3 = [](int s) { return s == 2 ? 0 : s + 1; };

  const int cphys = (lh ^ ((lr >> 3) & 1)) << 4;
  const unsigned a_row = lds0 + (unsigned)((wm * 32 + lr) * V6_ROWB + cphys);
  const unsigned b_row = lds0 + (unsigned)((wn * 32 + lr) * V6_ROWB + cphys);
  int stg = 0;

  struct dma_src {
    v6_i32x4 ra;
    unsigned va[4], vb[2], sa, sb;
  };
  auto src_of = [&](const tile_t& t, int step) {
    dma_src d;
    int ks = step;
    if constexpr (SEG3) {
      const int seg = (step >= kseg ? 1 : 0) + (step >= 2 * kseg ? 1 : 0);
      ks = step - seg * kseg;
#pragma unroll
      for (int k = 0; k < 4; ++k) {
        d.ra[k] = seg == 1 ? t.rsA1[k] : t.rsA[k];
        d.va[k] = seg == 2 ? avoff1[k] : avoff[k];
      }
    } else {
      d.ra = t.rsA;
#pragma unroll
      for (int k = 0; k < 4; ++k) d.va[k] = avoff[k];
    }
    d.vb[0] = t.bvoff[0];
    d.vb[1] = t.bvoff[1];
#pragma unroll
    for (int k = 0; k < 4; ++k) d.ra[k] = __builtin_amdgcn_readfirstlane(d.ra[k]);
    d.sa = (unsigned)__builtin_amdgcn_readfirstlane(ks * 512);
    d.sb = (unsigned)__builtin_amdgcn_readfirstlane((int)((unsigned)step * b_step));
    return d;
  };
#define V6K_INPUTS(src, dst, wimm)                                                                                             \
  [a] "v"(a_row + (unsigned)stg * (unsigned)V6_STAGE), [b] "v"(b_row + (unsigned)stg * (unsigned)V6_STAGE),                    \
      [va0] "v"((src).va[0]), [va1] "v"((src).va[1]), [va2] "v"((src).va[2]), [va3] "v"((src).va[3]), [vb0] "v"((src).vb[0]), \
      [vb1] "v"((src).vb[1]), [ra] "s"((src).ra), [rb] "s"(rsB), [m0a] "s"(dst_a0 + (unsigned)(dst) * (unsigned)V6_STAGE),     \
      [m0b] "s"(dst_b0 + (unsigned)(dst) * (unsigned)V6_STAGE), [sa] "s"((src).sa), [sb] "s"((src).sb), [w] "n"(wimm)
#pragma clang diagnostic ignored "-Winline-asm"
#define V6K_STMT_R(REGS, TEXT, tl_, step, dst, wimm)                                                                     \
  do {                                                                                                                   \
    const dma_src src_ = src_of(tl_, step);                                                                              \
    asm volatile(TEXT : REGS(acc, faL, fbL, faH, fbH) : V6K_INPUTS(src_, dst, wimm) : "memory", "scc", "m0");                  \
  } while (0)
#define V6K_STMT(TEXT, tl_, step, dst, wimm) V6K_STMT_R(V6K_REGS, TEXT, tl_, step, dst, wimm)
  auto issue = [&](const tile_t& tl_, int step, int dst) {
    const dma_src src_ = src_of(tl_, step);
    asm volatile(V6K_ISSUE : : V6K_INPUTS(src_, dst, 0) : "memory", "scc", "m0");
  };
  constexpr bool early = V6_RDSCHED == 1 || (V6_RDSCHED < 0 && (EPI == W_EPI_POOLV || EPI == W_EPI_C1W));
  constexpr int NST = v6_stores<EPI>();
  constexpr int first_n = NST + 6 > 63 ? 63 : NST + 6;
  constexpr int first_wait = (first_n & 15) | (7 << 4) | (0 << 8) | ((first_n >> 4) << 14);

  issue(cur, 0, 0);
  issue(cur, 1, 1);
  __builtin_amdgcn_s_waitcnt(0x0f70);
#if V6_STAMP
  int stamp_tile = 0;
#endif
  for (long long vb = blockIdx.x; vb < nwg; vb += gridDim.x) {
    __builtin_amdgcn_s_barrier();
    asm volatile("" ::: "memory");
    V6_STAMP_AT(0);
    V6_STAMP_AT(1);
    auto prefetch = [&] {
      if constexpr (EPI == W_EPI_POOL || EPI == W_EPI_POOLV || EPI == W_EPI_LRELU) return v5_prefetch_pool(p, cur.n0, wn, lr);
      else if constexpr (EPI == W_EPI_MASK) return v6_prefetch_mask(p, cur.R0, cur.n0, wm, wn, lr, lh);
      else if constexpr (EPI == W_EPI_MASKY) return v6_prefetch_masky(p, cur.R0, cur.n0, wm, wn, lr, lh);
      else if constexpr (EPI == W_EPI_GY) return v6_prefetch_masky<true>(p, cur.R0, cur.n0, wm, wn, lr, lh);
      else return v6_prefetch_c1w(p, cur.R0, cur.n0, wm, wn, lr, lh);
    };
    decltype(prefetch()) pre;
#define V6K_RUN(KIND, RSFX, tl_, step, dst, wimm)                                                                              \
  do {                                                                                                                         \
    if constexpr (SIX) V6K_STMT_R(V6K6_REGS##RSFX, V6K6_##KIND##_L, tl_, step, dst, wimm);                                     \
    else if constexpr (early) V6K_STMT_R(V6K_REGS##RSFX, V6K_##KIND##_E, tl_, step, dst, wimm);                                \
    else V6K_STMT_R(V6K_REGS##RSFX, V6K_##KIND##_L, tl_, step, dst, wimm);                                                     \
  } while (0)
    if constexpr (SIX) V6K_STMT_R(V6K6_REGS_FIRST, V6K6_FIRST, cur, 2, stg == 0 ? 2 : stg - 1, first_wait);
    else V6K_STMT_R(V6K_REGS_FIRST, V6K_FIRST, cur, 2, stg == 0 ? 2 : stg - 1, first_wait);
    stg = next3(stg);
    V6K_RUN(STEP1, _STEP1, cur, 3, stg == 0 ? 2 : stg - 1, 0);
    stg = next3(stg);
    V6_STAMP_AT(2);
    {
      int s = 2;
      do {
        V6K_RUN(NORM, , cur, s + 2, stg == 0 ? 2 : stg - 1, 0);
        stg = next3(stg);
      } while (++s + 2 < nsteps);
    }
    V6_STAMP_AT(3);
    V6K_RUN(PRELAST, , cur, 0, 0, 0);
    stg = next3(stg);
    pre = prefetch();
    V6K_RUN(LAST, , cur, 0, 0, 0);
    stg = next3(stg);
#undef V6K_RUN
    V6_STAMP_AT(4);

#if V6_ABL & 2
    {
      float t = 0.f;
#pragma unroll
      for (int i = 0; i < 8; ++i)
#pragma unroll
        for (int e = 0; e < 16; ++e) t += acc[i][e];
      if (t == 12345.678f) p.out[tid] = t;
    }
#endif
    const tile_t done = cur;
    const long long nb = vb + gridDim.x;
    const int last_stage = stg == 0 ? 2 : stg - 1;
    __builtin_amdgcn_s_waitcnt(0x0f70);
    if (nb < nwg) {
      cur = advance(cur);
      issue(cur, 0, stg);
      issue(cur, 1, next3(stg));
    }
    __builtin_amdgcn_sched_barrier(0);
#if V6_STAMP
    unsigned long long* est = (tid == 0 && stamp_tile < V6_STAMP_TILES && blockIdx.x < 256)
                                  ? v6_stamp_buf + ((long long)blockIdx.x * V6_STAMP_TILES + stamp_tile) * V6_STAMP_SLOTS : nullptr;
#else
    constexpr unsigned long long* est = nullptr;
#endif
#if !(V6_ABL & 2)
    float* scratch = reinterpret_cast<float*>(lds + last_stage * V6_STAGE);
    (void)scratch;
    const bool full = done.R0 + V6_ROWS <= p.M && done.n0 + V6_BN <= p.N;
    if constexpr (EPI == W_EPI_POOL) {
      if (full) v6_epilogue_pool<false, true>(p, acc, pre, nullptr, done.R0, done.n0, wm, wn, lr, lh, done.tm, est);
      else v6_epilogue_pool<false, false>(p, acc, pre, nullptr, done.R0, done.n0, wm, wn, lr, lh, done.tm, est);
    } else if constexpr (EPI == W_EPI_POOLV) {
      float* xch = reinterpret_cast<float*>(lds + 3 * V6_STAGE);
      if (full) v6_epilogue_pool<true, true>(p, acc, pre, xch, done.R0, done.n0, wm, wn, lr, lh, done.tm, est);
      else v6_epilogue_pool<true, false>(p, acc, pre, xch, done.R0, done.n0, wm, wn, lr, lh, done.tm, est);
    } else if constexpr (EPI == W_EPI_LRELU) {
      if (full) v6_epilogue_lrelu<true>(p, acc, pre, done.R0, done.n0, wm, wn, lr, lh);
      else v6_epilogue_lrelu<false>(p, acc, pre, done.R0, done.n0, wm, wn, lr, lh);
    } else if constexpr (EPI == W_EPI_MASK) {
      if (full) v6_epilogue_mask<true>(p, acc, pre, done.R0, done.n0, wm, wn, lr, lh);
      else v6_epilogue_mask<false>(p, acc, pre, done.R0, done.n0, wm, wn, lr, lh);
    } else if constexpr (EPI == W_EPI_MASKY) {
      float* xch = reinterpret_cast<float*>(lds + 3 * V6_STAGE);
      if (full) v6_epilogue_masky<true>(p, acc, pre, xch, done.R0, done.n0, wm, wn, lr, lh, done.tm, est);
      else v6_epilogue_masky<false>(p, acc, pre, xch, done.R0, done.n0, wm, wn, lr, lh, done.tm, est);
    } else if constexpr (EPI == W_EPI_GY) {
      float* xch = reinterpret_cast<float*>(lds + 3 * V6_STAGE);
      if (full) v6_epilogue_masky<true, true>(p, acc, pre, xch, done.R0, done.n0, wm, wn, lr, lh, done.tm, est);
      else v6_epilogue_masky<false, true>(p, acc, pre, xch, done.R0, done.n0, wm, wn, lr, lh, done.tm, est);
    } else {
      v6_epilogue_c1w(p, acc, pre, reinterpret_cast<float*>(lds + 3 * V6_STAGE) + wave * 512, scratch, done.R0, done.n0, wm, wn,
                      lr, lh, done.tm);
    }
#endif
    V6_STAMP_AT(5);
    {
      constexpr int n = NST + 6 > 63 ? 63 : NST + 6;
      __builtin_amdgcn_s_waitcnt((n & 15) | (7 << 4) | (15 << 8) | ((n >> 4) << 14));
    }
    V6_STAMP_AT(6);
    V6_STAMP_AT(7);
#if V6_STAMP
    ++stamp_tile;
#endif
  }
}

#if V6_STAMP
}
extern "C" int tl_debug_v6_stamps(unsigned long long* dst, int clear) {
  if (dst && hipMemcpyFromSymbol(dst, HIP_SYMBOL(tl::v6_stamp_buf), sizeof(tl::v6_stamp_buf)) != hipSuccess) return -1;
  if (clear) {
    void* p = nullptr;
    if (hipGetSymbolAddress(&p, HIP_SYMBOL(tl::v6_stamp_buf)) != hipSuccess) return -1;
    if (hipMemset(p, 0, sizeof(tl::v6_stamp_buf)) != hipSuccess) return -1;
  }
  return 0;
}
namespace tl {
#endif


constexpr int T6_BN = 64, T6_H = 6;
constexpr int T6_PLANE = T6_H * 64;
constexpr int T6_TILE = 8 * T6_PLANE;
constexpr int T6_NA = 4, T6_NG = 6;
constexpr int T6_GW = T6_H * 4 * 64;
constexpr int T6_GT = T6_GW + 64;
#ifndef T6_ABL
#define T6_ABL 0
#endif

template <bool WVD>
__global__ __launch_bounds__(512, 1) void wino63v_tn_kernel(const tl_tn_params p, int mtn) {
  constexpr int NA = T6_NA, NG = T6_NG, GW = T6_GW, GT = T6_GT;
  __shared__ __attribute__((aligned(1024))) float lds[(NA * 2 + 2) * T6_TILE + NG * GT];
  float* As = lds;
  float* Bs = lds + NA * 2 * T6_TILE;
  float* Gs = Bs + 2 * T6_TILE;
  const int tid = threadIdx.x, lane = tid & 63;
  const int wave = __builtin_amdgcn_readfirstlane(tid >> 6);
  const int wm = wave >> 1, wn = wave & 1, lr = lane & 31, lh = lane >> 5;
  const int ntn = p.Ndim / T6_BN;
  const long long tiles = (long long)mtn * ntn;
  const long long nwg = tiles * p.splitk;
  long long bid = (long long)blockIdx.y * gridDim.x + blockIdx.x;
  {
    const long long q = nwg / 8, r = nwg % 8, x = bid % 8, i = bid / 8;
    bid = (x < r ? x * (q + 1) : r * (q + 1) + (x - r) * q) + i;
  }
  const int z = __builtin_amdgcn_readfirstlane((int)(bid / tiles));
  const int tt = __builtin_amdgcn_readfirstlane((int)(bid % tiles));
  const int mi = __builtin_amdgcn_readfirstlane(tt / ntn);
  const int m0 = mi * 128, n0 = __builtin_amdgcn_readfirstlane((tt % ntn) * T6_BN);

  const long long hexes_all = p.Krows / 6;
  const long long ksteps_all = (hexes_all + T6_H - 1) / T6_H;
  const long long per = __builtin_amdgcn_readfirstlane((int)((ksteps_all + p.splitk - 1) / p.splitk));
  const long long ks_begin = z * per;
  long long ks_end = ks_begin + per;
  if (ks_end > ksteps_all) ks_end = ksteps_all;
  const int nsteps = ks_end > ks_begin ? (int)(ks_end - ks_begin) : 0;

  f32x16 acc[8];
#pragma unroll
  for (int i = 0; i < 8; ++i)
#pragma unroll
    for (int e = 0; e < 16; ++e) acc[i][e] = 0.f;
// ... 1015 lines not shown
    };
    wb = or8(nib << sh);
    ws = or8(nsg << sh);
  };
  const long long h0 = seq * Th;
  const int q0 = (int)((hpar - h0) & 1) + 2 * psub;
  const int trips = (Th + 2 * ppp - 1) / (2 * ppp) + 1;
  const bool word_writer = sh == 0;
  for (int i = 0; i < trips; ++i) {
    const int q = q0 + 2 * ppp * i;
    const bool live = q < Th;
    f32x4 d[8];
    uint32_t wb[8], ws[8];
#pragma unroll
    for (int j = 0; j < 8; ++j) row(6 * q + j, live && 6 * q + j < Tp, d[j], wb[j], ws[j]);
    if (live) {
      const long long row0 = seq * Tp + 6 * q;
#pragma unroll
      for (int j = 0; j < 6; ++j) {
        if (P != nullptr) *reinterpret_cast<f32x4*>(P + (row0 + j) * C1 + o) = d[j];
        if (word_writer) {
          bits[(row0 + j) * (C1 >> 5) + (o >> 5)] = wb[j];
          if (sign != nullptr) sign[(row0 + j) * (C1 >> 5) + (o >> 5)] = ws[j];
        }
      }
      f32x4 ov[8];
#pragma unroll
      for (int k = 0; k < 4; ++k) {
        float dd[8], vv[8];
#pragma unroll
        for (int j = 0; j < 8; ++j) dd[j] = d[j][k];
        wino63_bt(dd, vv);
#pragma unroll
        for (int j = 0; j < 8; ++j) ov[j][k] = vv[j];
      }
#if C1V_TEST == 1
      float* dst = V + (h0 + q) * 8LL * C1 + o;
#pragma unroll
      for (int j = 0; j < 8; ++j) *reinterpret_cast<f32x4*>(dst + (long long)j * C1) = ov[j];
#elif C1V_TEST == 2
      float* dst = V + v6_at(h0 + q, 0, o, C1 >> 3);
#pragma unroll
      for (int j = 0; j < 8; ++j) __builtin_nontemporal_store(ov[j], reinterpret_cast<f32x4*>(dst + 16 * j));
#elif C1V_TEST == 3
      (void)ov;
      if (o == 12345) V[0] = ov[0][0] + ov[7][3];
#elif C1V_TEST == 4
      const int upper = (tl_ >> 2) & 1;
      const int om = 8 * (kc ^ 1) + 4 * (half ^ 1);
      float* dst = V + v6_at(h0 + q, 0, o, C1 >> 3) + 16 * upper;
      float* mdst = V + v6_at((h0 + q) ^ 1, 0, om, C1 >> 3) + 16 * upper;
#pragma unroll
      for (int s2 = 0; s2 < 4; ++s2) {
        f32x4 own, got;
#pragma unroll
        for (int k = 0; k < 4; ++k) {
          const float send = upper ? ov[2 * s2][k] : ov[2 * s2 + 1][k];
          own[k] = upper ? ov[2 * s2 + 1][k] : ov[2 * s2][k];
          got[k] = __builtin_bit_cast(float, __builtin_amdgcn_update_dpp(0, __builtin_bit_cast(int, send), 0x141, 0xf, 0xf, false));
        }
        *reinterpret_cast<f32x4*>((upper ? mdst : dst) + 32 * s2) = upper ? got : own;
        *reinterpret_cast<f32x4*>((upper ? dst : mdst) + 32 * s2) = upper ? own : got;
      }
#else
      float* dst = V + v6_at(h0 + q, 0, o, C1 >> 3);
#pragma unroll
      for (int j = 0; j < 8; ++j) *reinterpret_cast<f32x4*>(dst + 16 * j) = ov[j];
#endif
    }
  }
}

}

extern "C" int tl_wino63_weights(const float* w, float* fwd, float* dgr, int O, int I, int ld_f, int ld_d, void* stream) {
  using namespace tl;
  TL_REQUIRE(w != nullptr && (fwd != nullptr || dgr != nullptr), "wino63_weights: null pointer");
  TL_REQUIRE(O > 0 && I > 0, "wino63_weights: bad sizes");
  TL_REQUIRE((fwd == nullptr || (ld_f >= I && ld_f % 8 == 0)) && (dgr == nullptr || (ld_d >= O && ld_d % 8 == 0)),
             "wino63_weights: leading dimensions must cover the reduction length and be multiples of 8");
  const long long nf = (long long)O * ld_f, nd = (long long)I * ld_d;
  const long long n = nf > nd ? nf : nd;
  TL_REQUIRE((n + 255) / 256 < (1LL << 31), "wino63_weights: too large");
  hipLaunchKernelGGL(wino63_weights_kernel, dim3((unsigned)((n + 255) / 256)), dim3(256), 0, (hipStream_t)stream, w, fwd, dgr, O,
                     I, ld_f, ld_d);
  return check_launch("wino63_weights");
}

extern "C" int tl_wino63_wgrad_finalize(const float* red, float* gw, int O, int I, int ld, void* stream) {
  using namespace tl;
  TL_REQUIRE(red && gw && O > 0 && I > 0 && ld >= O, "wino63_wgrad_finalize: bad arguments");
  const long long n = (long long)O * I;
  hipLaunchKernelGGL(wino63_wgrad_finalize_kernel, dim3((unsigned)((n + 255) / 256)), dim3(256), 0, (hipStream_t)stream, red, gw,
                     O, I, ld);
  return check_launch("wino63_wgrad_finalize");
}

extern "C" int tl_wino63_v_fixup(float* V, const float* vhalo, int64_t hexes, int64_t tiles, int Tq, int C, int ldv, void* stream) {
  using namespace tl;
  TL_REQUIRE(V && vhalo, "wino63_v_fixup: null pointer");
  TL_REQUIRE(hexes > 0 && tiles > 0 && Tq > 0 && Tq % 6 == 0, "wino63_v_fixup: hexes, tiles > 0 and Tq %% 6 == 0 needed");
  TL_REQUIRE(C > 0 && C % 4 == 0 && ldv >= C && ldv % 8 == 0, "wino63_v_fixup: C %% 4 and ldv %% 8 needed");
  const long long n = (long long)tiles * (C / 4);
  TL_REQUIRE((n + 255) / 256 < (1LL << 31), "wino63_v_fixup: grid too large");
  hipLaunchKernelGGL(wino63_v_fixup_kernel, dim3((unsigned)((n + 255) / 256)), dim3(256), 0, (hipStream_t)stream, V, vhalo,
                     (long long)hexes, (long long)tiles, Tq, C, ldv);
  return check_launch("wino63_v_fixup");
}

extern "C" int tl_wino63_vd_fixup(float* Vd, const float* vhalo, int64_t hexes, int64_t tiles, int hexes_per_seq, int C, int ldv,
                                  void* stream) {
  using namespace tl;
  TL_REQUIRE(Vd && vhalo, "wino63_vd_fixup: null pointer");
  TL_REQUIRE(hexes > 0 && tiles > 0 && hexes_per_seq > 0, "wino63_vd_fixup: hexes, tiles, hexes per sequence > 0 needed");
  TL_REQUIRE(C > 0 && C % 4 == 0 && ldv >= C && ldv % 8 == 0, "wino63_vd_fixup: C %% 4 and ldv %% 8 needed");
  const long long n = (long long)tiles * (C / 4);
  TL_REQUIRE((n + 255) / 256 < (1LL << 31), "wino63_vd_fixup: grid too large");
  hipLaunchKernelGGL(wino63_vd_fixup_kernel, dim3((unsigned)((n + 255) / 256)), dim3(256), 0, (hipStream_t)stream, Vd, vhalo,
                     (long long)hexes, (long long)tiles, hexes_per_seq, C, ldv);
  return check_launch("wino63_vd_fixup");
}

extern "C" int tl_wino63_unpool_yvd(const float* G, const uint32_t* bits, float* Y, float* Vd, int64_t conv_rows, int64_t g_rows,
                                    int Tp, int g_tp, int Tvalid, int C, int ldg, int ld_bits, int ldv, void* stream) {
  using namespace tl;
  TL_REQUIRE(G && bits && Y && Vd, "wino63_unpool_yvd: null pointer");
  TL_REQUIRE(Tp > 0 && Tp % 6 == 0 && conv_rows > 0 && conv_rows % Tp == 0 && Tvalid % 2 == 0 && Tvalid <= Tp,
             "wino63_unpool_yvd: Tp %% 6 == 0, whole sequences, an even Tvalid <= Tp needed");
  TL_REQUIRE(g_tp > 0 && 2 * g_tp >= Tvalid && g_rows >= (conv_rows / Tp) * (long long)g_tp, "wino63_unpool_yvd: G holds fewer rows than sequences x g_tp");
  TL_REQUIRE(C > 0 && C % 8 == 0 && ldg >= C && ldg % 4 == 0 && ldv >= C && ldv % 8 == 0 && ld_bits * 32 >= C,
             "wino63_unpool_yvd: C %% 8, ldg %% 4, ldv %% 8 needed, bits row must cover C");
  const long long nhex = conv_rows / 6;
  const long long n = ((nhex + 1) / 2) * (C / 2);
  TL_REQUIRE((n + 255) / 256 < (1LL << 31), "wino63_unpool_yvd: grid too large");
  hipLaunchKernelGGL(wino63_unpool_yvd_kernel, dim3((unsigned)((n + 255) / 256)), dim3(256), 0, (hipStream_t)stream, G, bits, Y, Vd,
                     nhex, (long long)g_rows, Tp / 6, g_tp, Tvalid, C, ldg, ld_bits, ldv);
  return check_launch("wino63_unpool_yvd");
}

extern "C" int tl_wino63_weights7(const float* w, float* fwd, int O, int I, int taps, void* stream) {
  using namespace tl;
  TL_REQUIRE(w && fwd && O > 0 && I > 0 && I % 8 == 0 && taps >= 7 && taps <= 9, "wino63_weights7: I %% 8 == 0 and 7..9 taps needed");
  const long long n = 3LL * O * I;
  TL_REQUIRE((n + 255) / 256 < (1LL << 31), "wino63_weights7: grid too large");
  hipLaunchKernelGGL(wino63_weights7_kernel, dim3((unsigned)((n + 255) / 256)), dim3(256), 0, (hipStream_t)stream, w, fwd, O, I, taps);
  return check_launch("wino63_weights7");
}

extern "C" int tl_wino63_xform2(const float* P, float* V0, float* V1, int64_t rows, int Tp, int Tvalid, int C, int ldp, int ldv,
                                void* stream) {
  using namespace tl;
  TL_REQUIRE(P && V0 && V1, "wino63_xform2: null pointer");
  TL_REQUIRE(Tp > 0 && Tp % 6 == 0 && rows > 0 && rows % Tp == 0 && Tvalid >= 0 && Tvalid <= Tp, "wino63_xform2: Tp %% 6 == 0, whole sequences, Tvalid <= Tp needed");
  TL_REQUIRE(C > 0 && C % 8 == 0 && ldp >= C && ldp % 4 == 0 && ldv >= C && ldv % 8 == 0, "wino63_xform2: C %% 8, ldp %% 4, ldv %% 8 needed");
  const long long nhex = rows / 6;
  const long long n = ((nhex + 1) / 2) * (C / 2);
  TL_REQUIRE((n + 255) / 256 < (1LL << 31), "wino63_xform2: grid too large");
  hipLaunchKernelGGL(wino63_xform2_kernel, dim3((unsigned)((n + 255) / 256)), dim3(256), 0, (hipStream_t)stream, P, V0, V1, nhex,
                     Tp / 6, Tp, Tvalid, C, ldp, ldv);
  return check_launch("wino63_xform2");
}

extern "C" int tl_conv7_wino63v_nt(const tl_nt_params* pp, void* stream) {
  using namespace tl;
  TL_REQUIRE(pp != nullptr, "conv7_wino63: null params");
  const tl_nt_params& p = *pp;
  TL_REQUIRE(p.A && p.aux && p.Bw && p.out, "conv7_wino63: null V0 (A) / V1 (aux) / Bw / out");
  TL_REQUIRE(p.loader == W_LOAD_V && p.epilogue == W_EPI_LRELU && p.row_shift == 0 && p.splitk <= 1,
             "conv7_wino63: loader 2 (pre-transformed operands), LRELU epilogue, row_shift 0, no split-K");
  TL_REQUIRE(p.J >= 7 && p.J <= 9, "conv7_wino63: 7..9 taps (three segments)");
  TL_REQUIRE(p.M > 0 && p.M % 6 == 0 && p.N > 0 && p.N % 32 == 0 && p.K >= 16 && p.K % 8 == 0, "conv7_wino63: M %% 6, N %% 32, K %% 8, K >= 16 needed");
  TL_REQUIRE(p.lda >= p.K && p.lda % 8 == 0 && p.ldb >= 3 * p.K && p.ldb % 8 == 0 && p.ldo >= p.N, "conv7_wino63: bad leading dimensions");
  TL_REQUIRE(p.A_rows % 2 == 0 && p.Tp > 0 && p.Tp % 6 == 0 && p.M % p.Tp == 0, "conv7_wino63: V holds hex pairs; Tp %% 6, whole sequences");
  TL_REQUIRE(8LL * p.N * p.ldb * 4 < (1LL << 31), "conv7_wino63: tap set larger than a buffer resource");
  TL_REQUIRE(128LL * 8 * p.lda * 4 + 4LL * p.K < (1LL << 31) && p.M + V6_ROWS < (1LL << 31), "conv7_wino63: tile span / M too large");
  TL_REQUIRE(p.slope >= 0.f && p.slope <= 1.f, "conv7_wino63: LeakyReLU slope must lie in [0, 1]");
  const long long ntm = (p.M + V6_ROWS - 1) / V6_ROWS;
  const long long nwg = ntm * ((p.N + V6_BN - 1) / V6_BN);
  TL_REQUIRE(nwg < (1LL << 31), "conv7_wino63: grid too large");
  TL_REQUIRE(p.A_rows >= ntm * V6_BH, "conv7_wino63: V0 / V1 must hold whole 128-hex tiles (pad them with zero hexes)");
  const long long ngrid = nwg < 256 ? nwg : 256;
  hipLaunchKernelGGL((wino63v_nt_kernel<W_EPI_LRELU>), dim3((unsigned)ngrid), dim3(512), 0, (hipStream_t)stream, p);
  return check_launch("conv7_wino63");
}

extern "C" int tl_wino63_nt_tile_rows(void) { return tl::V6_ROWS; }

extern "C" int tl_conv3_wino63v_nt(const tl_nt_params* pp, void* stream) {
  using namespace tl;
  TL_REQUIRE(pp != nullptr, "wino63v_nt: null params");
  const tl_nt_params& p = *pp;
  TL_REQUIRE(p.A && p.Bw && (p.out || p.epilogue == W_EPI_C1W || p.epilogue == W_EPI_POOLV || p.epilogue == W_EPI_MASKY), "wino63v_nt: null V/Bw/out");
  TL_REQUIRE(p.loader == W_LOAD_V, "wino63v_nt: loader 2 (pre-transformed operand) only");
  TL_REQUIRE(p.J == 3 && p.splitk <= 1, "wino63v_nt: 3 taps, no split-K");
  TL_REQUIRE(p.M > 0 && p.M % 6 == 0 && p.N > 0 && p.K >= 40 && p.K % 8 == 0, "wino63v_nt: M %% 6, K %% 8, K >= 40 needed");
  TL_REQUIRE(p.lda >= p.K && p.ldb >= p.K && p.lda % 8 == 0 && p.ldb % 8 == 0, "wino63v_nt: bad leading dimensions (multiples of 8)");
  TL_REQUIRE(p.A_rows % 2 == 0, "wino63v_nt: V holds hex pairs");
  TL_REQUIRE(p.Tp > 0 && p.Tp % 6 == 0 && p.M % p.Tp == 0, "wino63v_nt: Tp must be a positive multiple of 6, M whole sequences");
  TL_REQUIRE(8LL * p.N * p.ldb * 4 < (1LL << 31), "wino63v_nt: tap set larger than a buffer resource");
  TL_REQUIRE(128LL * 8 * p.lda * 4 + 4LL * p.K < (1LL << 31), "wino63v_nt: tile span too large");
  const long long ntm = (p.M + V6_ROWS - 1) / V6_ROWS;
  const long long nwg = ntm * ((p.N + V6_BN - 1) / V6_BN);
  TL_REQUIRE(nwg < (1LL << 31), "wino63v_nt: grid too large");
  TL_REQUIRE(p.N % 32 == 0 && p.M + V6_ROWS < (1LL << 31), "wino63v_nt: N %% 32 == 0 and M < 2^31 - 768 needed");
  TL_REQUIRE(p.slope >= 0.f && p.slope <= 1.f, "wino63v_nt: LeakyReLU slope must lie in [0, 1]");
  TL_REQUIRE(p.A_rows >= ntm * V6_BH, "wino63v_nt: V must hold whole 128-hex tiles (pad it with zero hexes)");
  hipStream_t st = (hipStream_t)stream;
  const long long ngrid = nwg < 256 ? nwg : 256;
  if (p.epilogue == W_EPI_POOL) {
    TL_REQUIRE(p.row_shift == 0 && p.out && p.ldo >= p.N, "wino63v_nt: forward needs row_shift 0 and an output");
    TL_REQUIRE(p.obits != nullptr && p.Tvalid % 2 == 0 && p.Tvalid <= p.Tp, "wino63v_nt: POOL needs obits and an even Tvalid");
    TL_REQUIRE(p.ld_obits * 32 >= p.N, "wino63v_nt: POOL: ld_obits too small");
    TL_REQUIRE(p.out_tp >= 0 && (p.out_tp == 0 || 2 * p.out_tp >= p.Tvalid), "wino63v_nt: out_tp must cover the valid pooled rows");
    const long long orows = (p.M / p.Tp) * (long long)(p.out_tp > 0 ? p.out_tp : p.Tp / 2);
    TL_REQUIRE(orows * (long long)p.ldo * 4 < (1LL << 40), "wino63v_nt: output too large");
    hipLaunchKernelGGL((wino63v_nt_kernel<W_EPI_POOL>), dim3((unsigned)ngrid), dim3(512), 0, st, p);
  } else if (p.epilogue == W_EPI_POOLV) {
    TL_REQUIRE(p.row_shift == 0 && (p.out == nullptr || p.ldo >= p.N), "wino63v_nt: forward needs row_shift 0");
    TL_REQUIRE(p.obits != nullptr && p.Tvalid % 2 == 0 && p.Tvalid <= p.Tp, "wino63v_nt: POOLV needs obits and an even Tvalid");
    TL_REQUIRE(p.ld_obits * 32 >= p.N && p.Tp % 12 == 0, "wino63v_nt: POOLV needs Tp %% 12 == 0 (output hexes inside one sequence)");
    TL_REQUIRE(p.vout && p.vhalo && p.ld_vout >= p.N && p.ld_vout % 8 == 0 && p.vout_quads >= p.M / 12 && p.vout_quads % 2 == 0,
               "wino63v_nt: POOLV needs vout (>= M / 12 hexes, whole pairs, ld_vout %% 8 == 0) and vhalo");
    TL_REQUIRE(64LL * 8 * p.ld_vout * 4 < (1LL << 31), "wino63v_nt: ld_vout too large");
    hipLaunchKernelGGL((wino63v_nt_kernel<W_EPI_POOLV>), dim3((unsigned)ngrid), dim3(512), 0, st, p);
  } else if (p.epilogue == W_EPI_MASK) {
    TL_REQUIRE(p.row_shift == -2 && p.ldo >= p.N, "wino63v_nt: input gradient needs row_shift -2");
    TL_REQUIRE(p.auxbits != nullptr, "wino63v_nt: MASK needs auxbits (the sign bits of the stage input)");
    hipLaunchKernelGGL((wino63v_nt_kernel<W_EPI_MASK>), dim3((unsigned)ngrid), dim3(512), 0, st, p);
  } else if (p.epilogue == W_EPI_MASKY) {
    TL_REQUIRE(p.row_shift == -2 && p.auxbits != nullptr && p.abits != nullptr, "wino63v_nt: epilogue 6 needs row_shift -2, auxbits and abits");
    TL_REQUIRE(p.ld_abits * 32 >= p.N && p.Tvalid_in % 2 == 0 && p.Tvalid_in <= 2 * p.Tp, "wino63v_nt: epilogue 6: bad abits / Tvalid_in");
    TL_REQUIRE(p.vout && p.vout2 && p.vhalo && p.ld_vout >= p.N && p.ld_vout % 8 == 0 && p.vout_quads >= p.M / 3 && p.vout_quads % 2 == 0,
               "wino63v_nt: epilogue 6 needs vout / vout2 (>= M / 3 hexes, whole pairs, ld_vout %% 8 == 0) and vhalo");
    TL_REQUIRE(128LL * 8 * p.ld_vout * 4 < (1LL << 31), "wino63v_nt: ld_vout too large");
    hipLaunchKernelGGL((wino63v_nt_kernel<W_EPI_MASKY>), dim3((unsigned)ngrid), dim3(512), 0, st, p);
  } else if (p.epilogue == W_EPI_C1W) {
    TL_REQUIRE(p.row_shift == -2, "wino63v_nt: input gradient needs row_shift -2");
    TL_REQUIRE(p.auxbits && p.c1x && p.c1bits && p.c1partial, "wino63v_nt: epilogue 4 needs auxbits, c1x, c1bits, c1partial");
    TL_REQUIRE(p.c1kt >= 1 && p.c1kt <= 3 && p.c1T >= 2 * p.Tvalid + 2, "wino63v_nt: epilogue 4: 1..3 taps, c1T >= 2*Tvalid + 2");
    hipLaunchKernelGGL((wino63v_nt_kernel<W_EPI_C1W>), dim3((unsigned)ngrid), dim3(512), 0, st, p);
  } else {
    set_error("wino63v_nt: unsupported epilogue %d", p.epilogue);
    return TL_EINVAL;
  }
  return check_launch("wino63v_nt");
}

extern "C" int tl_wino63_unpool_rows6(const float* G, const uint32_t* bits, float* A, int64_t rows, int64_t g_rows, int Tp, int g_tp,
                                      int Tvalid, int C, int ldg, int ld_bits, int lda, int pad, void* stream) {
  using namespace tl;
  TL_REQUIRE(G && bits && A, "wino63_unpool_rows6: null pointer");
  TL_REQUIRE(rows > 0 && Tp > 0 && rows % Tp == 0 && Tvalid > 0 && Tvalid <= Tp, "wino63_unpool_rows6: whole sequences of Tp rows, 0 < Tvalid <= Tp needed");
  TL_REQUIRE(g_tp > 0 && 2 * g_tp >= Tvalid && g_rows >= (rows / Tp) * (long long)g_tp, "wino63_unpool_rows6: G holds fewer rows than sequences x g_tp");
  TL_REQUIRE(C > 0 && C % 8 == 0 && ldg >= C && ldg % 4 == 0 && lda >= C && lda % 8 == 0 && ld_bits * 32 >= C,
             "wino63_unpool_rows6: C %% 8, ldg %% 4, lda %% 8 needed, bits row must cover C");
  const long long nhex = (rows + 5) / 6;
  const long long n = (nhex + 1) / 2 * (C >> 1);
  TL_REQUIRE((n + 255) / 256 < (1LL << 31), "wino63_unpool_rows6: grid too large");
  hipLaunchKernelGGL(wino63_unpool_rows6_kernel, dim3((unsigned)((n + 255) / 256)), dim3(256), 0, (hipStream_t)stream, G, bits, A,
                     nhex, (long long)rows, (long long)g_rows, Tp, g_tp, Tvalid, C, ldg, ld_bits, lda, pad);
  return check_launch("wino63_unpool_rows6");
}

extern "C" int tl_wino63_weights1(const float* w, float* taps, int O, int I, int ldb, void* stream) {
  using namespace tl;
  TL_REQUIRE(w && taps && O > 0 && I > 0 && ldb >= O && ldb % 8 == 0, "wino63_weights1: w, taps, O, I > 0 and ldb %% 8 == 0, ldb >= O needed");
  const long long n = (long long)ldb * 8 * I;
  TL_REQUIRE((n + 255) / 256 < (1LL << 31), "wino63_weights1: too large");
  hipLaunchKernelGGL(wino63_weights1_kernel, dim3((unsigned)((n + 255) / 256)), dim3(256), 0, (hipStream_t)stream, w, taps, O, I, ldb);
  return check_launch("wino63_weights1");
}

extern "C" int tl_conv1_wino63v_dgrad_nt(const tl_nt_params* pp, void* stream) {
  using namespace tl;
  TL_REQUIRE(pp != nullptr, "conv1_wino63v_dgrad_nt: null params");
  const tl_nt_params& p = *pp;
  TL_REQUIRE(p.A && p.Bw, "conv1_wino63v_dgrad_nt: null A / taps");
  TL_REQUIRE(p.loader == W_LOAD_V && p.epilogue == W_EPI_GY && p.J == 1 && p.row_shift == 0 && p.splitk <= 1,
             "conv1_wino63v_dgrad_nt: loader 2, epilogue 7, one tap, row_shift 0, no split-K");
  TL_REQUIRE(p.M > 0 && p.N > 0 && p.K >= 40 && p.K % 8 == 0, "conv1_wino63v_dgrad_nt: K %% 8, K >= 40 needed");
  TL_REQUIRE(p.Tp > 0 && p.Tp % 3 == 0 && p.M % p.Tp == 0, "conv1_wino63v_dgrad_nt: Tp (rows per sequence) must be a multiple of 3, M whole sequences");
  TL_REQUIRE(p.lda >= p.K && p.ldb >= p.K && p.lda % 8 == 0 && p.ldb % 8 == 0, "conv1_wino63v_dgrad_nt: bad leading dimensions (multiples of 8)");
  TL_REQUIRE(p.A_rows % 2 == 0, "conv1_wino63v_dgrad_nt: A holds hex pairs");
  TL_REQUIRE(8LL * p.N * p.ldb * 4 < (1LL << 31), "conv1_wino63v_dgrad_nt: tap set larger than a buffer resource");
  TL_REQUIRE(128LL * 8 * p.lda * 4 + 4LL * p.K < (1LL << 31), "conv1_wino63v_dgrad_nt: tile span too large");
  const long long ntm = (p.M + V6_ROWS - 1) / V6_ROWS;
  const long long nwg = ntm * ((p.N + V6_BN - 1) / V6_BN);
  TL_REQUIRE(nwg < (1LL << 31), "conv1_wino63v_dgrad_nt: grid too large");
  TL_REQUIRE(p.N % 32 == 0 && p.M + V6_ROWS < (1LL << 31), "conv1_wino63v_dgrad_nt: N %% 32 == 0 and M < 2^31 - 768 needed");
  TL_REQUIRE(p.slope >= 0.f && p.slope <= 1.f, "conv1_wino63v_dgrad_nt: LeakyReLU slope must lie in [0, 1]");
  TL_REQUIRE(p.A_rows >= ntm * V6_BH, "conv1_wino63v_dgrad_nt: A must hold whole 128-hex tiles (pad it with zero hexes)");
  TL_REQUIRE(p.auxbits != nullptr && p.abits != nullptr, "conv1_wino63v_dgrad_nt: needs auxbits (sign) and abits (arg-max) of the stage below");
  TL_REQUIRE(p.out_tp > 0 && p.out_tp <= p.Tp && 2 * p.out_tp >= p.Tvalid_in, "conv1_wino63v_dgrad_nt: out_tp = rows per sequence of the bit arrays (0 < out_tp <= Tp, covering Tvalid_in / 2)");
  TL_REQUIRE(p.ld_abits * 32 >= p.N && p.ld_auxbits * 32 >= p.N && p.Tvalid_in % 2 == 0 && p.Tvalid_in <= 2 * p.Tp, "conv1_wino63v_dgrad_nt: bad abits / auxbits / Tvalid_in");
  TL_REQUIRE(p.vout && p.vout2 && p.vhalo && p.ld_vout >= p.N && p.ld_vout % 8 == 0 && p.vout_quads >= p.M / 3 && p.vout_quads % 2 == 0,
             "conv1_wino63v_dgrad_nt: needs vout / vout2 (>= M / 3 hexes, whole pairs, ld_vout %% 8 == 0) and vhalo");
  TL_REQUIRE(128LL * 8 * p.ld_vout * 4 < (1LL << 31), "conv1_wino63v_dgrad_nt: ld_vout too large");
  const long long ngrid = nwg < 256 ? nwg : 256;
  hipLaunchKernelGGL((wino63v_nt_kernel<W_EPI_GY>), dim3((unsigned)ngrid), dim3(512), 0, (hipStream_t)stream, p);
  return check_launch("conv1_wino63v_dgrad_nt");
}

extern "C" int tl_conv3_wino63v_tn(const tl_tn_params* pp, void* stream) {
  using namespace tl;
  TL_REQUIRE(pp != nullptr, "wino63v_tn: null params");
  tl_tn_params p = *pp;
  if (p.splitk < 1) p.splitk = 1;
  if (p.loader == 3) {
    TL_REQUIRE(p.A && p.B && p.slab, "wino63v_tn: null V/Y/slab");
    TL_REQUIRE(p.J == 3 && p.Tp > 0 && p.Tp % 6 == 0 && p.Krows > 0 && p.Krows % p.Tp == 0, "wino63v_tn: loader 3: bad Tp / Krows");
    TL_REQUIRE(p.Krows + 64 < (1LL << 31), "wino63v_tn: more than 2^31 reduction rows");
    TL_REQUIRE(p.Mdim % 256 == 0 && p.Ndim % 64 == 0 && p.lda % 8 == 0 && p.ldb % 8 == 0 && p.lda >= p.Mdim && p.ldb >= p.Ndim &&
               p.ldc >= p.Ndim, "wino63v_tn: loader 3 needs Mdim %% 256, Ndim %% 64, lda / ldb %% 8");
    TL_REQUIRE(p.A_rows % 2 == 0 && p.B_rows % 2 == 0 && p.vd == nullptr, "wino63v_tn: loader 3: whole hex pairs in V and Y, no Vd");
    TL_REQUIRE(p.splitk <= 65535 && (p.splitk == 1 || p.slab_stride >= 8LL * p.Mdim * p.ldc), "wino63v_tn: bad splitk / slab_stride");
    const long long ks = (p.Krows / 6 + T6_H - 1) / T6_H;
    TL_REQUIRE(p.A_rows >= ks * T6_H && p.B_rows >= ks * T6_H, "wino63v_tn: V and Y must hold whole 6-hex K-steps (pad with zero hexes)");
    const long long per3 = (ks + p.splitk - 1) / p.splitk;
    TL_REQUIRE((per3 + 4) * (long long)T6_H * 8 * p.lda * 4 < (1LL << 31) && (per3 + 4) * (long long)T6_H * 8 * p.ldb * 4 < (1LL << 31),
               "wino63v_tn: a reduction split spans more than 2 GB of V or Y: raise splitk");
    const int ntm3 = p.Mdim / 256;
    hipLaunchKernelGGL(wino63v_tn4y_kernel, dim3((unsigned)(2 * ntm3 * (p.Ndim / T6_BN)), (unsigned)p.splitk, 1), dim3(512), 0,
                       (hipStream_t)stream, p, ntm3);
// ... 64 lines not shown
```

decode_tonal_langauge_amd/csrc/tonal_wino63_epi.h:

```cpp
#pragma once
#include "tonal_common.h"
#include "tonal_wino43_epi.h"
#include "tonal_wino43v_epi.h"

namespace tl {

__device__ __forceinline__ void v6_stamp(unsigned long long* st, int k) {
  if (st != nullptr) st[k] = __builtin_amdgcn_s_memtime();
}

#ifndef V6_ST_AUX
#define V6_ST_AUX 0
#endif
constexpr unsigned V6_DROP = 0x80000000u;
constexpr unsigned long long V6_HI = 0xffffffff00000000ull;

template <bool IMM>
__device__ __forceinline__ void v6_store_at(float x, __amdgpu_buffer_rsrc_t rs, unsigned vo, unsigned so, unsigned k) {
  if constexpr (IMM) __builtin_amdgcn_raw_buffer_store_b32(__builtin_bit_cast(unsigned, x), rs, vo + k, so, V6_ST_AUX);
  else __builtin_amdgcn_raw_buffer_store_b32(__builtin_bit_cast(unsigned, x), rs, vo, so + k, V6_ST_AUX);
}

__device__ __forceinline__ void v6_pair_swap(float& a, float& b) {
  const auto r = __builtin_amdgcn_permlane32_swap(__float_as_uint(a), __float_as_uint(b), false, false);
  a = __uint_as_float(r[0]);
  b = __uint_as_float(r[1]);
}

template <bool IMM>
__device__ __forceinline__ void v6_store_hex_pair(float (&ha)[8], float (&hb)[8], __amdgpu_buffer_rsrc_t rs, unsigned voAP, unsigned voAQ,
                                                  unsigned voBP, unsigned voBQ, unsigned so) {
#pragma unroll
  for (int i = 0; i < 8; ++i) v6_pair_swap(ha[i], hb[i]);
#pragma unroll
  for (int t = 0; t < 8; t += 2) {
    {
      const auto r = __builtin_amdgcn_permlane16_swap(__float_as_uint(ha[t]), __float_as_uint(ha[t + 1]), false, false);
      v6_store_at<IMM>(__uint_as_float(r[0]), rs, voAP, so, (unsigned)(t * 64));
      v6_store_at<IMM>(__uint_as_float(r[1]), rs, voAQ, so, (unsigned)(t * 64));
    }
    {
      const auto r = __builtin_amdgcn_permlane16_swap(__float_as_uint(hb[t]), __float_as_uint(hb[t + 1]), false, false);
      v6_store_at<IMM>(__uint_as_float(r[0]), rs, voBP, so, (unsigned)(t * 64));
      v6_store_at<IMM>(__uint_as_float(r[1]), rs, voBQ, so, (unsigned)(t * 64));
    }
  }
}
__device__ __forceinline__ unsigned v6_pair_offset(int colbase, int lr, int lh) {
  return (unsigned)((colbase >> 3) + ((lr >> 3) & 1)) * 512u + (unsigned)((lr >> 4) & 1) * 64u + (unsigned)lh * 32u + (unsigned)(lr & 7) * 4u;
}

__device__ __forceinline__ void wino63_rows(const f32x16 (&acc)[8], int e, float (&y)[6]) {
  const float m1 = acc[1][e], m2 = acc[2][e], m3 = acc[3][e], m4 = acc[4][e], m5 = acc[5][e], m6 = acc[6][e];
  const float a12 = m1 + m2, s12 = m1 - m2, a34 = m3 + m4, s34 = m3 - m4, a56 = m5 + m6, s56 = m5 - m6;
  y[0] = ((acc[0][e] + a12) + a34) + a56;
  y[1] = fmaf(0.5f, s56, fmaf(2.f, s34, s12));
  y[2] = fmaf(0.25f, a56, fmaf(4.f, a34, a12));
  y[3] = fmaf(0.125f, s56, fmaf(8.f, s34, s12));
  y[4] = fmaf(0.0625f, a56, fmaf(16.f, a34, a12));
  y[5] = fmaf(0.03125f, s56, fmaf(32.f, s34, s12)) + acc[7][e];
}
__device__ __forceinline__ void wino63_bt(const float (&d)[8], float (&v)[8]) {
  v[0] = fmaf(5.25f, d[2] - d[4], d[6] - d[0]);
  const float e1 = fmaf(-4.25f, d[4], d[2] + d[6]), o1 = fmaf(-4.25f, d[3], d[1] + d[5]);
  v[1] = e1 + o1;
  v[2] = e1 - o1;
  const float e2 = fmaf(0.25f, d[2], fmaf(-1.25f, d[4], d[6])), o2 = fmaf(0.5f, d[1], fmaf(-2.5f, d[3], 2.f * d[5]));
  v[3] = e2 + o2;
  v[4] = e2 - o2;
  const float e3 = fmaf(4.f, d[2], fmaf(-5.f, d[4], d[6])), o3 = fmaf(2.f, d[1], fmaf(-2.5f, d[3], 0.5f * d[5]));
  v[5] = e3 + o3;
  v[6] = e3 - o3;
  v[7] = fmaf(5.25f, d[3] - d[5], d[7] - d[1]);
}

__device__ __forceinline__ float selbit(uint32_t w, int j, float a, float b) {
  const uint32_t m = (uint32_t)__builtin_amdgcn_sbfe((int)w, j, 1);
  return __uint_as_float((__float_as_uint(a) & m) | (__float_as_uint(b) & ~m));
}

struct v6_rows {
  int tA, tB;
  long long seqA, seqB;
};
__device__ __forceinline__ v6_rows v6_rows_of(long long Hw, int Tp) {
  v6_rows r;
  const unsigned R = (unsigned)(6 * Hw);
  const unsigned s = R / (unsigned)Tp;
  r.seqA = (long long)(unsigned)__builtin_amdgcn_readfirstlane((int)s);
  r.tA = __builtin_amdgcn_readfirstlane((int)(R - s * (unsigned)Tp));
  r.tB = r.tA + 96;
  r.seqB = r.seqA;
  while (r.tB >= Tp) {
    r.tB -= Tp;
    ++r.seqB;
  }
  return r;
}
struct bits96 {
  unsigned long long lo;
  uint32_t hi;
};
__device__ __forceinline__ unsigned long long mask96(const bits96& a, const bits96& b, int j) {
  return j < 64 ? mask2l(a.lo, b.lo, j) : mask2(a.hi, b.hi, j - 64);
}
__device__ __forceinline__ bits96 v6_in_bits96(long long R0h, long long M) {
  bits96 r;
  r.lo = v5_in_bits<64, 1>(R0h, M);
  r.hi = (uint32_t)v5_in_bits<32, 1>(R0h + 64, M);
  return r;
}
__device__ __forceinline__ bits96 v6_valid_bits96(int t0, int Tp, int tlim, long long R0h, long long M) {
  bits96 r;
  r.lo = v5_valid_bits<64, 1>(t0, Tp, tlim, R0h, M);
  int t1 = t0 + 64;
  while (t1 >= Tp) t1 -= Tp;
  r.hi = (uint32_t)v5_valid_bits<32, 1>(t1, Tp, tlim, R0h + 64, M);
  return r;
}

template <bool VOUT, bool FULL>
__device__ __forceinline__ void v6_epilogue_pool(const tl_nt_params& p, const f32x16 (&acc)[8], const v5_pre_pool& pre, float* xch,
                                                 long long R0, int n0, int wm, int wn, int lr_in, int lh, long long tm,
                                                 unsigned long long* st = nullptr) {
  int lr = lr_in;
  asm volatile("" : "+v"(lr));
  const int colbase = n0 + wn * 32;
  const bool colok = colbase < p.N;
  const int col = colbase + lr;
  const long long Hw = tm * 128 + wm * 32;
  const int Tp = p.Tp, Tq = Tp >> 1;
  const v6_rows rw = v6_rows_of(Hw, Tp);
  const unsigned long long vA = v5_valid_bits<48, 2>(rw.tA, Tp, p.Tvalid, 6 * Hw, p.M);
  const unsigned long long vB = v5_valid_bits<48, 2>(rw.tB, Tp, p.Tvalid, 6 * Hw + 96, p.M);
  const float bv = pre.bv;
  const long long P0 = 3 * Hw;
  const long long prows = p.M >> 1;
  const int out_tp = (!VOUT && p.out_tp > 0) ? p.out_tp : Tq;
  const int tqa0 = rw.tA >> 1, tqb0 = rw.tB >> 1;
  const unsigned long long kA = v5_valid_bits<48, 1>(tqa0, Tq, out_tp, P0, prows);
  const unsigned long long kB = v5_valid_bits<48, 1>(tqb0, Tq, out_tp, P0 + 48, prows);
  const long long nseq = p.M / Tp;
  const long long obase = rw.seqA * out_tp;
// ... 72 lines not shown
  v6_stamp(st, 10);
  if constexpr (VOUT) {
    if (p.out != nullptr) {
      const __amdgpu_buffer_rsrc_t rsP = rsrc_of(p.out + P0 * (long long)p.ldo, (prows - P0) * (long long)p.ldo * 4);
      const unsigned pvoff = colok ? ((unsigned)(48 * lh) * (unsigned)p.ldo + (unsigned)col) * 4u : V5_OOB;
#pragma unroll
      for (int j = 0; j < 48; ++j) {
        const unsigned vo = selmu(mask2l(kA, kB, j), pvoff, V5_OOB);
        __builtin_amdgcn_raw_buffer_store_b32(__builtin_bit_cast(unsigned, pv[j]), rsP, vo, (unsigned)j * (unsigned)p.ldo * 4u, 0);
      }
    }
    const int slot = wm * 2 + lh;
    {
      float2 v2 = {pv[0], pv[1]};
      *reinterpret_cast<float2*>(xch + (slot * 64 + wn * 32 + lr) * 2) = v2;
    }
    __builtin_amdgcn_s_waitcnt(0xc07f);
    __builtin_amdgcn_s_barrier();
    asm volatile("" ::: "memory");
    v6_stamp(st, 11);
    float nb0 = 0.f, nb1 = 0.f;
    if (slot < 7) {
      const float2 v2 = *reinterpret_cast<const float2*>(xch + ((slot + 1) * 64 + wn * 32 + lr) * 2);
      nb0 = v2.x;
      nb1 = v2.y;
    }
    uint32_t seA = 0, seB = 0, nvA = 0, nvB = 0;
    {
      int t_a = tqa0, t_b = tqb0;
      const long long qa = (Hw >> 1), qb = (Hw >> 1) + 8;
      for (int k = 0; k < 8; ++k) {
        seA |= (uint32_t)(t_a == Tq - 6) << k;
        seB |= (uint32_t)(t_b == Tq - 6) << k;
        nvA |= (uint32_t)(FULL || qa + k < p.vout_quads) << k;
        nvB |= (uint32_t)(FULL || qb + k < p.vout_quads) << k;
        t_a += 6;
        if (t_a >= Tq) t_a -= Tq;
        t_b += 6;
        if (t_b >= Tq) t_b -= Tq;
      }
    }
    const long long Hn = Hw >> 1;
    const __amdgpu_buffer_rsrc_t rsV = rsrc_of(p.vout + Hn * 8 * (long long)p.ld_vout,
                                              (p.vout_quads - Hn) * 8 * (long long)p.ld_vout * 4);
    const unsigned pair4 = (unsigned)p.ld_vout * 64u;
    const unsigned offP = v6_pair_offset(colbase, lr, lh);
    const unsigned vvA = colok ? offP : V6_DROP, vvB = colok ? 4u * pair4 + offP : V6_DROP;
    const unsigned long long mraw = wm == 3 ? V6_HI : 0ull;
#pragma unroll
    for (int qp = 0; qp < 4; ++qp) {
      float vv[2][8];
#pragma unroll
      for (int hq = 0; hq < 2; ++hq) {
        const int q = 2 * qp + hq;
        const unsigned long long mend = mask2(seA, seB, q);
        float d[8];
#pragma unroll
        for (int k = 0; k < 6; ++k) d[k] = pv[6 * q + k];
        d[6] = selm(mend, 0.f, q < 7 ? pv[(6 * q + 6) % 48] : nb0);
        d[7] = selm(mend, 0.f, q < 7 ? pv[(6 * q + 7) % 48] : nb1);
        wino63_bt(d, vv[hq]);
        if (q == 7) {
#pragma unroll
          for (int k = 0; k < 6; ++k) vv[hq][k] = selm(mraw, d[k], vv[hq][k]);
        }
      }
      const int q = 2 * qp;
      const unsigned voA = selmu(mask2(nvA, nvA >> 1, q), vvA, V6_DROP), voB = selmu(mask2(nvB, nvB >> 1, q), vvB, V6_DROP);
      v6_store_hex_pair<FULL>(vv[0], vv[1], rsV, voA, voA + 1024u, voB, voB + 1024u, (unsigned)qp * pair4);
    }
    v6_stamp(st, 12);
    {
      const bool hw = wm == 0 && p.vhalo != nullptr;
      const __amdgpu_buffer_rsrc_t rsH = rsrc_of(hw ? p.vhalo + tm * 2 * (long long)p.N : nullptr, hw ? 2LL * p.N * 4 : 0);
      const unsigned ho = (colok && lh == 0) ? (unsigned)col * 4u : V5_OOB;
      __builtin_amdgcn_raw_buffer_store_b32(__builtin_bit_cast(unsigned, pv[0]), rsH, ho, 0u, 0);
      __builtin_amdgcn_raw_buffer_store_b32(__builtin_bit_cast(unsigned, pv[1]), rsH, ho, (unsigned)p.N * 4u, 0);
    }
  }
}

template <int EPI>
constexpr int v6_stores() {
  return EPI == W_EPI_POOL ? 52 : EPI == W_EPI_POOLV ? 70 : (EPI == W_EPI_MASK || EPI == W_EPI_LRELU) ? 96 : (EPI == W_EPI_MASKY || EPI == W_EPI_GY) ? 63 : 0;
}

struct v6_pre_mask {
  uint32_t s[3];
};
__device__ __forceinline__ v6_pre_mask v6_prefetch_mask(const tl_nt_params& p, long long R0, int n0, int wm, int wn, int lr, int lh) {
  const int colbase = n0 + wn * 32;
  const long long ra = R0 + wm * 192 + 96 * lh + lr;
  v6_pre_mask r = {{0u, 0u, 0u}};
#pragma unroll
  for (int k = 0; k < 3; ++k)
    if (colbase < p.N && ra + 32 * k < p.M) r.s[k] = p.auxbits[(ra + 32 * k) * (long long)p.ld_auxbits + (colbase >> 5)];
  return r;
}
template <bool FULL>
__device__ __forceinline__ void v6_epilogue_mask(const tl_nt_params& p, const f32x16 (&acc)[8], const v6_pre_mask& pre, long long R0,
                                                 int n0, int wm, int wn, int lr_in, int lh) {
  int lr = lr_in;
  asm volatile("" : "+v"(lr));
  const int colbase = n0 + wn * 32;
  const bool colok = colbase < p.N;
  const int col = colbase + lr;
  const long long Rw = R0 + wm * 192;
  const __amdgpu_buffer_rsrc_t rsO = rsrc_of(p.out + Rw * (long long)p.ldo, (p.M - Rw) * (long long)p.ldo * 4);
  const unsigned ovoff = colok ? ((unsigned)(96 * lh) * (unsigned)p.ldo + (unsigned)col) * 4u : V5_OOB;
  const unsigned ldo4 = (unsigned)p.ldo * 4u;
  bits96 inA = {~0ull, ~0u}, inB = inA;
  if (!FULL) {
    inA = v6_in_bits96(Rw, p.M);
    inB = v6_in_bits96(Rw + 96, p.M);
  }
  uint32_t sT[3];
#pragma unroll
  for (int k = 0; k < 3; ++k) sT[k] = bit_transpose32(pre.s[k], lr);
#pragma unroll
  for (int e = 0; e < 16; ++e) {
    float y[6];
    wino63_rows(acc, e, y);
#pragma unroll
    for (int h = 0; h < 6; ++h) {
      const int r = 6 * e + h;
      const float o = y[h] * selbit(sT[r >> 5], r & 31, 1.f, p.slope);
      const unsigned vo = FULL ? ovoff : selmu(mask96(inA, inB, r), ovoff, V5_OOB);
      __builtin_amdgcn_raw_buffer_store_b32(__builtin_bit_cast(unsigned, o), rsO, vo, (unsigned)r * ldo4, 0);
    }
  }
}

template <bool FULL>
__device__ __forceinline__ void v6_epilogue_lrelu(const tl_nt_params& p, const f32x16 (&acc)[8], const v5_pre_pool& pre, long long R0,
                                                  int n0, int wm, int wn, int lr_in, int lh) {
  int lr = lr_in;
  asm volatile("" : "+v"(lr));
  const int colbase = n0 + wn * 32;
  const bool colok = colbase < p.N;
  const int col = colbase + lr;
  const long long Rw = R0 + wm * 192;
  const __amdgpu_buffer_rsrc_t rsO = rsrc_of(p.out + Rw * (long long)p.ldo, (p.M - Rw) * (long long)p.ldo * 4);
  const unsigned ovoff = colok ? ((unsigned)(96 * lh) * (unsigned)p.ldo + (unsigned)col) * 4u : V5_OOB;
  const unsigned ldo4 = (unsigned)p.ldo * 4u;
  bits96 inA = {~0ull, ~0u}, inB = inA;
  if (!FULL) {
    inA = v6_in_bits96(Rw, p.M);
    inB = v6_in_bits96(Rw + 96, p.M);
  }
  const float bv = pre.bv;
#pragma unroll
  for (int e = 0; e < 16; ++e) {
    float y[6];
    wino63_rows(acc, e, y);
#pragma unroll
    for (int h = 0; h < 6; ++h) {
      const int r = 6 * e + h;
      const float o = lrelu01(y[h] + bv, p.slope);
      const unsigned vo = FULL ? ovoff : selmu(mask96(inA, inB, r), ovoff, V5_OOB);
      __builtin_amdgcn_raw_buffer_store_b32(__builtin_bit_cast(unsigned, o), rsO, vo, (unsigned)r * ldo4, 0);
    }
  }
}

struct v6_pre_masky {
  uint32_t s[3], a[3];
};
template <bool GTP = false>
__device__ __forceinline__ v6_pre_masky v6_prefetch_masky(const tl_nt_params& p, long long R0, int n0, int wm, int wn, int lr, int lh) {
  const int colbase = n0 + wn * 32;
  const long long ra = R0 + wm * 192 + 96 * lh + lr;
  v6_pre_masky r;
#pragma unroll
  for (int k = 0; k < 3; ++k) {
    r.s[k] = r.a[k] = 0u;
    if (colbase < p.N && ra + 32 * k < p.M) {
      long long row = ra + 32 * k;
      bool have = true;
      if constexpr (GTP) {
        const unsigned R = (unsigned)row, sq = R / (unsigned)p.Tp, t = R - sq * (unsigned)p.Tp;
        have = t < (unsigned)p.out_tp;
        row = (long long)sq * p.out_tp + t;
      }
      if (have) {
        r.s[k] = p.auxbits[row * (long long)p.ld_auxbits + (colbase >> 5)];
        r.a[k] = p.abits[row * (long long)p.ld_abits + (colbase >> 5)];
      }
    }
  }
  return r;
}
template <bool FULL, bool DIRECT = false>
__device__ __forceinline__ void v6_epilogue_masky(const tl_nt_params& p, const f32x16 (&acc)[8], const v6_pre_masky& pre, float* xch,
                                                  long long R0, int n0, int wm, int wn, int lr_in, int lh, long long tm,
                                                  unsigned long long* st = nullptr) {
  int lr = lr_in;
  asm volatile("" : "+v"(lr));
  const int colbase = n0 + wn * 32;
  const bool colok = colbase < p.N;
  const int col = colbase + lr;
  const long long Rw = R0 + wm * 192;
  const int Tp = p.Tp, hps = Tp / 3;
  const v6_rows rw = v6_rows_of(tm * 128 + wm * 32, Tp);
  uint32_t we[3], wo[3], sT[3], firstw = 0;
  {
    const bits96 okA = v6_valid_bits96(rw.tA, Tp, p.Tvalid_in >> 1, Rw, p.M);
    const bits96 okB = v6_valid_bits96(rw.tB, Tp, p.Tvalid_in >> 1, Rw + 96, p.M);
    const uint32_t okw[3] = {lh ? (uint32_t)okB.lo : (uint32_t)okA.lo, lh ? (uint32_t)(okB.lo >> 32) : (uint32_t)(okA.lo >> 32),
                             lh ? okB.hi : okA.hi};
    uint32_t fA = 0, fB = 0;
    int ha = rw.tA / 3, hb = rw.tB / 3;
    for (int k = 0; k < 32; ++k) {
      fA |= (uint32_t)(ha == 0) << k;
      fB |= (uint32_t)(hb == 0) << k;
      ha = ha + 1 == hps ? 0 : ha + 1;
      hb = hb + 1 == hps ? 0 : hb + 1;
    }
    firstw = lh ? fB : fA;
#pragma unroll
    for (int k = 0; k < 3; ++k) {
      sT[k] = bit_transpose32(pre.s[k], lr);
      const uint32_t aT = bit_transpose32(pre.a[k], lr);
      we[k] = okw[k] & ~aT;
      wo[k] = okw[k] & aT;
    }
  }
  const long long Hb = Rw / 3;
  const unsigned pair4 = (unsigned)p.ld_vout * 64u;
  const __amdgpu_buffer_rsrc_t rsY = rsrc_of(p.vout + Hb * 8 * (long long)p.ld_vout, (p.vout_quads - Hb) * 8 * (long long)p.ld_vout * 4);
  const __amdgpu_buffer_rsrc_t rsD = rsrc_of(p.vout2 + Hb * 8 * (long long)p.ld_vout, (p.vout_quads - Hb) * 8 * (long long)p.ld_vout * 4);
  const unsigned offP = v6_pair_offset(colbase, lr, lh);
  const unsigned vvA = colok ? offP : V6_DROP, vvB = colok ? 16u * pair4 + offP : V6_DROP;
  const int nexA = (int)(p.M / 3 - Hb < 64 ? p.M / 3 - Hb : 64) - lh, nexB = nexA - 32;
  float pe = 0.f, po = 0.f;
  float first_d[6], v1keep[8];
#pragma unroll
  for (int k = 0; k < 6; ++k) first_d[k] = 0.f;
#pragma unroll
  for (int k = 0; k < 8; ++k) v1keep[k] = 0.f;
  auto andf = [](float x, uint32_t m) { return __uint_as_float(__float_as_uint(x) & m); };
  v6_stamp(st, 8);
#pragma unroll
  for (int e = 0; e < 16; ++e) {
    if (e == 1) v6_stamp(st, 9);
    if (e == 4) v6_stamp(st, 10);
    if (e == 8) v6_stamp(st, 11);
    if (e == 12) v6_stamp(st, 12);
    float y[6];
    if constexpr (DIRECT) {
#pragma unroll
      for (int h = 0; h < 6; ++h) y[h] = acc[h][e];
    } else {
      wino63_rows(acc, e, y);
    }
    float dzr[12];
#pragma unroll
    for (int h = 0; h < 6; ++h) {
      const int r = 6 * e + h;
      const float t = y[h] * selbit(sT[r >> 5], r & 31, 1.f, p.slope);
      dzr[2 * h] = andf(t, (uint32_t)__builtin_amdgcn_sbfe((int)we[r >> 5], r & 31, 1));
      dzr[2 * h + 1] = andf(t, (uint32_t)__builtin_amdgcn_sbfe((int)wo[r >> 5], r & 31, 1));
    }
    float Yp[2][8], Vp[2][8];
#pragma unroll
    for (int hh = 0; hh < 2; ++hh) {
      const int j = 2 * e + hh;
      const float* d6 = dzr + 6 * hh;
      const float ev1 = (d6[0] + d6[2]) + d6[4], od1 = (d6[1] + d6[3]) + d6[5];
      const float ev2 = fmaf(16.f, d6[4], fmaf(4.f, d6[2], d6[0])), od2 = fmaf(32.f, d6[5], fmaf(8.f, d6[3], 2.f * d6[1]));
      const float ev3 = fmaf(0.0625f, d6[4], fmaf(0.25f, d6[2], d6[0])), od3 = fmaf(0.03125f, d6[5], fmaf(0.125f, d6[3], 0.5f * d6[1]));
      Yp[hh][0] = d6[0];
      Yp[hh][1] = ev1 + od1;
      Yp[hh][2] = ev1 - od1;
      Yp[hh][3] = ev2 + od2;
      Yp[hh][4] = ev2 - od2;
      Yp[hh][5] = ev3 + od3;
      Yp[hh][6] = ev3 - od3;
      Yp[hh][7] = d6[5];
      if (j == 0) {
#pragma unroll
        for (int k = 0; k < 6; ++k) first_d[k] = d6[k];
      } else {
        const uint32_t keep = ~(uint32_t)__builtin_amdgcn_sbfe((int)firstw, j, 1);
        float d[8];
        d[0] = andf(pe, keep);
        d[1] = andf(po, keep);
#pragma unroll
        for (int k = 0; k < 6; ++k) d[2 + k] = d6[k];
        wino63_bt(d, Vp[hh]);
      }
      pe = d6[4];
      po = d6[5];
    }
    {
      const int j = 2 * e;
      const unsigned so = (unsigned)e * pair4;
      const unsigned voA = FULL ? vvA : (j < nexA ? vvA : V6_DROP), voB = FULL ? vvB : (j < nexB ? vvB : V6_DROP);
      v6_store_hex_pair<FULL>(Yp[0], Yp[1], rsY, voA, voA + 1024u, voB, voB + 1024u, so);
      if (e == 0) {
#pragma unroll
        for (int i = 0; i < 8; ++i) v1keep[i] = Vp[1][i];
      } else {
        v6_store_hex_pair<FULL>(Vp[0], Vp[1], rsD, voA, voA + 1024u, voB, voB + 1024u, so);
      }
    }
    __builtin_amdgcn_sched_barrier(0);
  }
  v6_stamp(st, 13);
  const int slot = wm * 2 + lh;
  {
    float2 v2 = {pe, po};
    *reinterpret_cast<float2*>(xch + (slot * 64 + wn * 32 + lr) * 2) = v2;
  }
  __builtin_amdgcn_s_waitcnt(0xc07f);
  __builtin_amdgcn_s_barrier();
  asm volatile("" ::: "memory");
  {
    float fe = 0.f, fo = 0.f;
    if (slot > 0) {
      const float2 v2 = *reinterpret_cast<const float2*>(xch + ((slot - 1) * 64 + wn * 32 + lr) * 2);
      fe = v2.x;
      fo = v2.y;
    }
    const uint32_t keep = ~(uint32_t)__builtin_amdgcn_sbfe((int)firstw, 0, 1);
    float d[8], v[8];
    d[0] = andf(fe, keep);
    d[1] = andf(fo, keep);
#pragma unroll
    for (int k = 0; k < 6; ++k) d[2 + k] = first_d[k];
    wino63_bt(d, v);
    const bool raw = slot == 0;
#pragma unroll
    for (int k = 0; k < 8; ++k) v[k] = raw ? (k < 2 ? 0.f : d[k]) : v[k];
    const unsigned voA = FULL ? vvA : (0 < nexA ? vvA : V6_DROP), voB = FULL ? vvB : (0 < nexB ? vvB : V6_DROP);
    v6_store_hex_pair<FULL>(v, v1keep, rsD, voA, voA + 1024u, voB, voB + 1024u, 0u);
  }
  {
    const bool hw = wm == 3 && p.vhalo != nullptr;
    const __amdgpu_buffer_rsrc_t rsH = rsrc_of(hw ? p.vhalo + tm * 2 * (long long)p.N : nullptr, hw ? 2LL * p.N * 4 : 0);
    const unsigned ho = (colok && lh == 1) ? (unsigned)col * 4u : V5_OOB;
    __builtin_amdgcn_raw_buffer_store_b32(__builtin_bit_cast(unsigned, pe), rsH, ho, 0u, 0);
    __builtin_amdgcn_raw_buffer_store_b32(__builtin_bit_cast(unsigned, po), rsH, ho, (unsigned)p.N * 4u, 0);
  }
}

struct v6_pre_c1w {
  uint32_t s[3], c[3];
  f32x4 x[2];
};
__device__ __forceinline__ v6_pre_c1w v6_prefetch_c1w(const tl_nt_params& p, long long R0, int n0, int wm, int wn, int lr, int lh) {
  const int colbase = n0 + wn * 32;
  const long long rh = R0 + wm * 192 + 96 * lh;
  v6_pre_c1w r;
  const int Tp = p.Tp;
  const long long nseq = p.M / Tp;
  const unsigned s0 = (unsigned)(R0 / Tp);
  const __amdgpu_buffer_rsrc_t rsX = rsrc_of(p.c1x + (long long)s0 * p.c1T, (nseq - s0) * (long long)p.c1T * 4);
  typedef unsigned v4u __attribute__((ext_vector_type(4)));
#pragma unroll
  for (int k = 0; k < 3; ++k) {
    r.s[k] = r.c[k] = 0u;
    const long long rk = rh + lr + 32 * k;
    if (colbase < p.N && rk < p.M) {
      r.s[k] = p.auxbits[rk * (long long)p.ld_auxbits + (colbase >> 5)];
      r.c[k] = p.c1bits[rk * (long long)p.ld_auxbits + (colbase >> 5)];
    }
  }
  const unsigned Rx = (unsigned)(rh + 3 * lr), sx = Rx / (unsigned)Tp, tx = Rx - sx * (unsigned)Tp;
  const unsigned xo = ((sx - s0) * (unsigned)p.c1T + 2u * tx) * 4u;
  r.x[0] = __builtin_bit_cast(f32x4, (v4u)__builtin_amdgcn_raw_buffer_load_b128(rsX, xo, 0u, 0));
  r.x[1] = __builtin_bit_cast(f32x4, (v4u)__builtin_amdgcn_raw_buffer_load_b128(rsX, xo + 16u, 0u, 0));
  return r;
}
__device__ __forceinline__ void v6_epilogue_c1w(const tl_nt_params& p, const f32x16 (&acc)[8], const v6_pre_c1w& pre, float* xw,
                                                float* red, long long R0, int n0, int wm, int wn, int lr_in, int lh, long long tm) {
  int lr = lr_in;
  asm volatile("" : "+v"(lr));
  const int colbase = n0 + wn * 32;
  const bool colok = colbase < p.N;
  const int col = colbase + lr;
  const long long Hw = tm * 128 + wm * 32;
  const long long Rw = 6 * Hw;
  const int Tp = p.Tp;
  const v6_rows rw = v6_rows_of(Hw, Tp);
  const bits96 okA = v6_valid_bits96(rw.tA, Tp, p.Tvalid, Rw, p.M);
  const bits96 okB = v6_valid_bits96(rw.tB, Tp, p.Tvalid, Rw + 96, p.M);
  float* xh = xw + lh * 256;
  *reinterpret_cast<f32x4*>(xh + 8 * lr) = pre.x[0];
  *reinterpret_cast<f32x4*>(xh + 8 * lr + 4) = pre.x[1];
  c1w_acc ca;
  ca.clear();
  uint32_t sT[3], cT[3];
#pragma unroll
  for (int k = 0; k < 3; ++k) {
    sT[k] = bit_transpose32(pre.s[k], lr);
    cT[k] = bit_transpose32(pre.c[k], lr);
  }
  asm volatile("" ::: "memory");
#pragma unroll
  for (int e = 0; e < 16; ++e) {
    float y[6];
    wino63_rows(acc, e, y);
#pragma unroll
    for (int h = 0; h < 6; ++h) {
      const int r = 6 * e + h;
      const float2 xa = *reinterpret_cast<const float2*>(xh + 8 * (r / 3) + 2 * (r % 3));
      const float2 xb = *reinterpret_cast<const float2*>(xh + 8 * (r / 3) + 2 * (r % 3) + 2);
      const float dz = selm0(mask96(okA, okB, r), y[h] * selbit(sT[r >> 5], r & 31, 1.f, p.slope));
      const uint32_t am = (uint32_t)__builtin_amdgcn_sbfe((int)cT[r >> 5], r & 31, 1);
      auto pick = [am](float a, float b) { return __uint_as_float((__float_as_uint(a) & am) | (__float_as_uint(b) & ~am)); };
      ca.s[0] = fmaf(dz, pick(xa.y, xa.x), ca.s[0]);
      ca.s[1] = fmaf(dz, pick(xb.x, xa.y), ca.s[1]);
      ca.s[2] = fmaf(dz, pick(xb.y, xb.x), ca.s[2]);
      ca.b += dz;
    }
    __builtin_amdgcn_sched_barrier(0);
  }
  __syncthreads();
  c1w_reduce_store<4, 64>(p, red, ca, wm, wn * 32 + lr, lh, tm, col, colok);
}

}
```

include/tonal_hip.h:

```cpp
#ifndef TONAL_HIP_H
#define TONAL_HIP_H
#include <stdint.h>

#ifdef __cplusplus
extern "C" {
#endif

#define TL_OK 0
#define TL_EINVAL (-1)
#define TL_ELAUNCH (-2)
#define TL_ENODEV (-3)

const char* tl_last_error(void);
int tl_version(void);
int tl_device_count(void);

typedef struct {
  const float* A; const uint32_t* abits; const float* Bw; const float* bias; const float* aux;
  float* out; uint32_t* obits;
  int64_t M;
  int64_t A_rows;
  int N, K;
  int lda, ldb, ldo, ldaux, ld_abits, ld_obits;
  int J;
  int row_shift;
  int Tp, Tvalid, Tvalid_in;
  float slope;
  int loader, epilogue;
  int splitk; int64_t slab_stride;
  int bm;
  uint32_t* osign; const uint32_t* auxbits; int ld_auxbits;
  const float* c1x; const uint32_t* c1bits; float* c1partial; int c1T, c1kt;
  float* vout; float* vhalo; int64_t vout_quads; int ld_vout;
  int out_tp;
  float* vout2;
} tl_nt_params;
int tl_gemm_nt_window(const tl_nt_params* p, void* stream);

typedef struct {
  const float* A; const float* B; const uint32_t* bbits; float* slab;
  int64_t Krows;
  int64_t A_rows, B_rows;
  int Mdim, Ndim;
  int lda, ldb, ldc, ld_bbits;
  int J;
  int Tp, Tvalid;
  int loader;
  int splitk; int64_t slab_stride;
  float* colsum;
  float* vd; int ld_vd;
  int part;
  int bm;
  int g_tp;
} tl_tn_params;
int tl_gemm_tn_window(const tl_tn_params* p, void* stream);

int tl_wino43_weights(const float* w, float* fwd, float* dgr, int O, int I, int ld_f, int ld_d, void* stream);
int tl_wino43_wgrad_finalize(const float* red, float* gw, int O, int I, int ld, void* stream);
int tl_wino43_input_transform(const float* P, float* V, int64_t rows, int Tp, int C, int ldp, int ldv, void* stream);
int tl_conv3_wino43v_nt(const tl_nt_params* p, void* stream);
int tl_wino43_v_fixup(float* V, const float* vhalo, int64_t quads, int64_t tiles, int Tq, int C, int ldv, void* stream);
int tl_wino43_unpool_transform(const float* G, const uint32_t* bits, float* V, int64_t conv_rows, int64_t g_rows, int Tp,
                               int Tvalid, int C, int ldg, int ld_bits, int ldv, void* stream);
int tl_conv3_wino43v_tn(const tl_tn_params* p, void* stream);
int tl_wino63_weights(const float* w, float* fwd, float* dgr, int O, int I, int ld_f, int ld_d, void* stream);
int tl_conv3_wino63v_nt(const tl_nt_params* p, void* stream);
int tl_wino63_nt_tile_rows(void);
int tl_wino63_v_fixup(float* V, const float* vhalo, int64_t hexes, int64_t tiles, int Tq, int C, int ldv, void* stream);
int tl_conv3_wino63v_tn(const tl_tn_params* p, void* stream);
int tl_wino63_wgrad_finalize(const float* red, float* gw, int O, int I, int ld, void* stream);
int tl_wino63_vd_fixup(float* Vd, const float* vhalo, int64_t hexes, int64_t tiles, int hexes_per_seq, int C, int ldv, void* stream);
int tl_wino63_unpool_yvd(const float* G, const uint32_t* bits, float* Y, float* Vd, int64_t conv_rows, int64_t g_rows, int Tp,
                         int g_tp, int Tvalid, int C, int ldg, int ld_bits, int ldv, void* stream);
int tl_conv1_fwd_v6(const float* x, const float* w, const float* b, float* P, float* V, uint32_t* bits, uint32_t* sign,
                    int64_t S, int T, int ktaps, int C1, int Tp, int Tout, float slope, void* stream);
int tl_wino63_xform2(const float* P, float* V0, float* V1, int64_t rows, int Tp, int Tvalid, int C, int ldp, int ldv, void* stream);
int tl_wino63_weights7(const float* w, float* fwd, int O, int I, int taps, void* stream);
int tl_conv7_wino63v_nt(const tl_nt_params* p, void* stream);
int tl_wino63_unpool_rows6(const float* G, const uint32_t* bits, float* A, int64_t rows, int64_t g_rows, int Tp, int g_tp, int Tvalid,
                           int C, int ldg, int ld_bits, int lda, int pad, void* stream);
int tl_wino63_weights1(const float* w, float* taps, int O, int I, int ldb, void* stream);
int tl_conv1_wino63v_dgrad_nt(const tl_nt_params* p, void* stream);
int tl_comm_unique_id(void* id128);
int tl_comm_init(void** comm, int rank, int nranks, const void* id128);
int tl_comm_destroy(void* comm);
int tl_allreduce(void* comm, const float* send, float* recv, int64_t count, int op, void* stream);
int tl_reduce_scatter(void* comm, const float* send, float* recv, int64_t recv_count, void* stream);
int tl_all_gather(void* comm, const float* send, float* recv, int64_t send_count, void* stream);
int tl_sizeof_nt_params(void);
int tl_sizeof_tn_params(void);

int tl_conv1_fwd(const float* x, const float* w, const float* b, float* P, uint32_t* bits, uint32_t* sign,
                 int64_t S, int T, int ktaps, int C1, int Tp, int Tout, float slope, void* stream);
int tl_conv1_fwd_v(const float* x, const float* w, const float* b, float* P, float* V, uint32_t* bits, uint32_t* sign,
                   int64_t S, int T, int ktaps, int C1, int Tp, int Tout, float slope, void* stream);
int tl_conv1_wgrad(const float* x, const float* G, const uint32_t* bits, float* partial,
                   int nblk, int64_t S, int T, int ktaps, int C1, int Tp, int Tout, void* stream);

int tl_dropout_scale(float* x, int64_t n, float p, uint64_t seed, void* stream);

int tl_permute_reduce(const float* src, float* dst, const int64_t dims[4], const int64_t strides[4],
                      const int64_t lims[4], int nz, int64_t zs, const float* bias_last, void* stream);
int tl_colsum(const float* G, float* partial, int nblk, int64_t rows, int ncols, int ld,
              int Tp, int Tvalid, void* stream);

int tl_lstm_cell_fwd(const float* hh, const float* x_t, const float* w_ih, const float* b_ih,
                     const float* b_hh, const float* c_prev, float* act, float* c, float* h,
                     int U, int H, int in_dim, int ld_hh, void* stream);
int tl_lstm_gw(const float* g, const float* W, float* slab, int U, int64_t N, int K, int64_t ldg, int64_t ldw, int rows_per_block,
               void* stream);
int tl_lstm_infer_seq_fused(const float* xp, int64_t xp_row_stride, const float* wp, float* h_a, float* h_b, float* c,
                            int B, int H, int T, int* last_in_b, void* stream);
int tl_lstm_cell_bwd(const float* dh, const float* dh_rec, const float* dc_next, const float* act,
                     const float* c, const float* c_prev, float* dgates, float* dgates_t, float* dc_prev,
                     int U, int H, int ldt, void* stream);
int tl_lstm_ih_grad(const float* dgates, const float* x, float* dw_ih, float* db, float* db2 ,
                    int L, int U, int H, int in_dim, void* stream);

int tl_concat_pack(const float* O5, const float* h, const int32_t* uid, float* Xc,
                   int B, int C, int Tp, int lat, int Cc, int Lc, int ld5, int ldh, int ldx,
                   float p_drop, uint64_t seed, int64_t drop_row0, void* stream);
int tl_concat_unpack_bwd(const float* dXc, const float* O5, const int32_t* members, const int32_t* offsets,
                         float* G5, float* dh, int B, int U, int C, int Tp, int lat, int Cc, int Lc,
                         int ld5, int ldh, int ldx, float slope, float p_drop, uint64_t seed, int64_t drop_row0,
                         void* stream);

int tl_l1_mcd(const float* out, const float* targets, float* dout, float* stats,
              int B, int D, int ldd, int trunc_targets, float grad_scale, void* stream);

int tl_nadam(float* p, const float* g, float* m, float* v, int64_t n, float coef_grad, float coef_mom,
             float beta1, float beta2, float bias_corr2, float eps, float weight_decay, float grad_scale,
             void* stream);
typedef struct { float* p; const float* g; float* m; float* v; int64_t n; int64_t block0; } tl_nadam_entry;
int tl_nadam_multi(const tl_nadam_entry* entries_dev, int count, int64_t total_blocks, float coef_grad, float coef_mom,
                   float beta1, float beta2, float bias_corr2, float eps, float weight_decay, float grad_scale,
                   void* stream);
int tl_nadam_multi_chunk(void);
int tl_set_step_scalars(float* scalars_dev, uint64_t* seed_dev, float coef_grad, float coef_mom, float bias_corr2,
                        uint64_t seed, void* stream);
int tl_sum_slabs2(const float* srcA, float* dstA, int64_t nA, const float* srcB, float* dstB, int64_t nB, int nz, void* stream);
int tl_stage_step(float* scalars_dev, uint64_t* seed_dev, float coef_grad, float coef_mom, float bias_corr2, uint64_t seed,
                  const void* const* src, void* const* dst, const int64_t* nbytes, int n, void* stream);
int tl_nadam_multi_dev(const tl_nadam_entry* entries_dev, int count, int64_t total_blocks, const float* scalars_dev,
                       float beta1, float beta2, float eps, float weight_decay, float grad_scale, void* stream);
int tl_nadam_lowrank(float* p, float* m, float* v, const float* fa, const float* fb, int kr, int rows, int cols,
                     int ldfa, int ldfb, float coef_grad, float coef_mom, float beta1, float beta2,
                     float bias_corr2, float eps, float weight_decay, float grad_scale, void* stream);
int tl_nadam_lowrank_dh(float* p, float* m, float* v, const float* fa, const float* fb, int kr, int rows, int cols,
// ... 73 lines not shown
```

Before: 1275 mel-frames/s.

## Run conv2 input gradient on Y2 with un-flipped taps, drop Vd2 production

Conv3's input-gradient epilogue now writes only the transformed Y2 operand and skips computing and storing Vd2. Conv2's input gradient (fused with conv1's weight gradient) then runs on Y2 with transposed, un-flipped Winograd taps. Its new C1WGRAD_Y epilogue does the output-side overlap fixup in registers, carrying boundary values across tiles and reading the extra input rows itself. This removes one transformed buffer's writes and reads and the Vd transform work. In exchange the dgrad epilogue is more complex and needs an extra weight-packing launch and extra prefetches.

New measurement: 1292 mel-frames/s (median of 6 runs). 1.4% higher.

```diff
diff --git a/decode_tonal_langauge_amd/_cnn_engine.py b/decode_tonal_langauge_amd/_cnn_engine.py
--- a/decode_tonal_langauge_amd/_cnn_engine.py
+++ b/decode_tonal_langauge_amd/_cnn_engine.py
@@ -8,7 +8,7 @@
 import torch
 
 from . import _kernels, _lib
-from ._lib import (EPI_C1WGRAD, EPI_GY, EPI_LRELU, EPI_MASK, EPI_MASKY, EPI_POOL, EPI_POOLV, EPI_STORE, LOAD_DIRECT, LOAD_UNPOOL, LOAD_V,
+from ._lib import (EPI_C1WGRAD, EPI_C1WGRAD_Y, EPI_GY, EPI_MASKY_ONLY, EPI_LRELU, EPI_MASK, EPI_MASKY, EPI_POOL, EPI_POOLV, EPI_STORE, LOAD_DIRECT, LOAD_UNPOOL, LOAD_V,
                    LOAD_Y, NtParams, TnParams, check, ptr)
 
 
@@ -60,6 +60,7 @@
             self.tp1 = (self.tout1 + 11) // 12 * 12
         self.f63_yprod = (self.wino63 and _kernels.get("f63_yprod") != "0" and stage_defs[0][0] % 256 == 0
                           and self.tp1 >= 12)
+        self.f63_dgrad2_y = self.f63_yprod and _kernels.get("f63_yprod") != "vd"
         self.f63_yprod3 = (self.wino63 and _kernels.get("f63_yprod") != "0" and stage_defs[1][0] % 256 == 0)
         self.stages: List[_Stage] = []
         cin, tin, tp = self.c1, self.tout1, self.tp1
@@ -136,6 +137,7 @@
         self.V = {}
         self.Vd = {}
         self._vd_ready = {}
+        self._yd_ready = {}
         self.G = None
 
     def _alloc_bwd(self):
@@ -263,8 +265,12 @@
             V = store[idx] = torch.zeros(nh_pad, 8, cin, dtype=torch.float32, device=self._dev)
         return V
 
-    def _pack_wino63(self, w, forward: bool):
+    def _pack_wino63(self, w, forward: bool, transposed: bool = False):
         O, I = w.shape[0], w.shape[1]
+        if transposed:
+            dst = torch.empty(8, I, O, dtype=torch.float32, device=w.device)
+            check(self.lib.tl_wino63_weights_t(ptr(w), ptr(dst), O, I, O, self._stream()), "tl_wino63_weights_t")
+            return dst
         dst = torch.empty(8, O, I, dtype=torch.float32, device=w.device) if forward else \
             torch.empty(8, I, O, dtype=torch.float32, device=w.device)
         check(self.lib.tl_wino63_weights(ptr(w), ptr(dst) if forward else None, None if forward else ptr(dst), O, I, I, O,
@@ -403,12 +409,24 @@
         self._vd_ready[below.idx] = self.generation
         return None
 
-    def _stage_dgrad63(self, st, w):
+    def _stage_dgrad63(self, st, w, y_only=False):
         S = self.S
         rows_in = S * st.tp_in
+        if st.idx == 2 and self._vd_ready.get(2) != self.generation and self._yd_ready.get(2) == self.generation:
+            self._yd_ready[2] = -1
+            Y2 = self.Yt[2]
+            wt = self._pack_wino63(w, False, transposed=True)
+            ntm = -(-rows_in // self._nt63_rows())
+            part = torch.empty(ntm, (self.k1 + 1) * self.c1, dtype=torch.float32, device=self._dev)
+            self._nt(tag="conv2_dgrad", fn="tl_conv3_wino63v_nt", epilogue=EPI_C1WGRAD_Y, out=None, A=ptr(Y2), A_rows=Y2.shape[0],
+                     lda=Y2.shape[2], loader=LOAD_V, Bw=ptr(wt), M=rows_in, N=st.cin, K=st.cout, ldb=st.cout, ldo=st.cin, J=3,
+                     row_shift=0, Tp=st.tp_in, slope=self.slope, auxbits=ptr(self.sbits[1]), ld_auxbits=self.sbits[1].shape[1],
+                     c1x=ptr(self._x), c1bits=ptr(self.bits[1]), c1partial=ptr(part), c1T=self.T, c1kt=self.k1, Tvalid=self.tout1)
+            return part
         if self._vd_ready.get(st.idx) != self.generation:
             raise RuntimeError("F(6,3) input gradient: the stage's weight-gradient pass (which writes Vd) must run first")
         self._vd_ready[st.idx] = -1
+        self._yd_ready[st.idx] = -1
         Vd = self.Vd[st.idx]
         wd = self._pack_wino63(w, False)
         kw = dict(A=ptr(Vd), A_rows=Vd.shape[0], lda=Vd.shape[2], loader=LOAD_V, Bw=ptr(wd), M=rows_in, N=st.cin,
@@ -418,6 +436,14 @@
             below = self.stages[0]
             rows2 = S * below.tp_in
             Y2 = self._v_hex_buffer(self.Yt, 2, rows2, below.cout)
+            if y_only:
+                self._nt(tag="conv3_dgrad", fn="tl_conv3_wino63v_nt", epilogue=EPI_MASKY_ONLY, out=None, vout=ptr(Y2),
+                         vout_quads=Y2.shape[0], ld_vout=Y2.shape[2], abits=ptr(self.bits[2]), ld_abits=below.cout // 32,
+                         Tvalid_in=2 * below.tout, **kw)
+                self._y_ready[2] = self.generation
+                self._yd_ready[2] = self.generation
+                self._vd_ready[2] = -1
+                return None
             Vd2 = self._v_hex_buffer(self.Vd, 2, rows2, below.cout)
             ntm = -(-rows_in // self._nt63_rows())
             if not hasattr(self, "_vhalo"):
@@ -503,8 +529,11 @@
             tn2 = "wino63v_tn4_kernel<true>" if st2.cin % 256 == 0 else "wino63v_tn_kernel<true>"
             fams = {f"wino63v_nt_kernel<POOLV> (conv2 forward, {f6}; writes V of its pooled output for conv3)": ["conv2_fwd"],
                     f"wino63v_nt_kernel<POOL> (conv3 forward, {f6})": ["conv3_fwd"],
-                    f"wino63v_nt_kernel<C1WGRAD> (conv2 input gradient + conv1 weight gradient, {f6})": ["conv2_dgrad"],
                     }
+            if self.f63_dgrad2_y:
+                fams[f"wino63v_nt_kernel<C1WGRAD_Y> (conv2 input gradient on Y2 + conv1 weight gradient, {f6})"] = ["conv2_dgrad"]
+            else:
+                fams[f"wino63v_nt_kernel<C1WGRAD> (conv2 input gradient + conv1 weight gradient, {f6})"] = ["conv2_dgrad"]
             if self.f63_yprod3:
                 gy = self.gy4
                 src = "the epilogue of conv4's input gradient" if gy else "wino63_unpool_yvd_kernel"
@@ -512,7 +541,10 @@
                      f"from {src})"] = ["conv3_wgrad"]
             else:
                 fams[f"{tn} (conv3 weight gradient, {f6}; also writes Vd)"] = ["conv3_wgrad"]
-            if self.f63_yprod:
+            if self.f63_dgrad2_y:
+                fams[f"wino63v_nt_kernel<MASKY_ONLY> (conv3 input gradient, {f6}; writes Y of conv2 instead of the gradient rows)"] = ["conv3_dgrad"]
+                fams[f"wino63v_tn4y_kernel (conv2 weight gradient, {f6}: both operands by LDS-DMA, no transform in the kernel)"] = ["conv2_wgrad"]
+            elif self.f63_yprod:
                 fams[f"wino63v_nt_kernel<MASKY> (conv3 input gradient, {f6}; writes Y and Vd of conv2 instead of the gradient rows)"] = ["conv3_dgrad"]
                 fams[f"wino63v_tn4y_kernel (conv2 weight gradient, {f6}: both operands by LDS-DMA, no transform in the kernel)"] = ["conv2_wgrad"]
             else:
@@ -701,9 +733,9 @@
         else:
             self._colsum(Gs, Gs.shape[0], st.cout, ldg, st.tp_out, st.tout, gb)
 
-    def stage_dgrad(self, st: _Stage, w: torch.Tensor):
+    def stage_dgrad(self, st: _Stage, w: torch.Tensor, y_only: bool = False):
         if self._f63(st):
-            return self._stage_dgrad63(st, w)
+            return self._stage_dgrad63(st, w, y_only=y_only and st.idx == 3 and self.f63_yprod)
         if self._gy_stage(st):
             return self._stage_dgrad_gy(st, w)
         S = self.S
@@ -1082,7 +1114,7 @@
         for st in reversed(self.stages):
             name = self.STAGE_NAMES[st.idx]
             self.stage_wgrad(st, grads[name + ".weight"], grads[name + ".bias"])
-            part = self.stage_dgrad(st, prm[name + ".weight"])
+            part = self.stage_dgrad(st, prm[name + ".weight"], y_only=self.f63_dgrad2_y)
         if part is None:
             nblk = int(min(2048, S))
             part = torch.empty(nblk, (self.k1 + 1) * self.c1, **f32)
diff --git a/decode_tonal_langauge_amd/_kernels.py b/decode_tonal_langauge_amd/_kernels.py
--- a/decode_tonal_langauge_amd/_kernels.py
+++ b/decode_tonal_langauge_amd/_kernels.py
@@ -20,9 +20,12 @@
     "wino": ("TONAL_WINO", frozenset({"6", "4", "0"}), "6",
              "conv2 / conv3: 6 Winograd F(6,3) on pre-transformed operands (F(4,3) V form where the stack does not allow it), "
              "4 the F(4,3) V form, 0 direct MFMA kernels (also the fallback for every shape neither form covers)"),
-    "f63_yprod": ("TONAL_F63_YPROD", _B, "1", "F(6,3): the backward operands Y / Vd of stages 2 and 3 come pre-transformed out of the "
-                                              "input-gradient epilogue of the stage above (0: the weight-gradient kernels un-pool and "
-                                              "transform the gradient rows themselves)"),
+    "f63_yprod": ("TONAL_F63_YPROD", frozenset({"0", "1", "vd"}), "1",
+                  "F(6,3): the backward operands Y / Vd of stages 2 and 3 come pre-transformed out of the input-gradient epilogue "
+                  "of the stage above (0: the weight-gradient kernels un-pool and transform the gradient rows themselves).  1: "
+                  "in backward() conv2's input gradient runs on Y2, the operand of its weight gradient, with the un-flipped "
+                  "taps, and conv3's input gradient writes no Vd2; vd: it writes Y2 and Vd2, conv2's input gradient runs on Vd2 "
+                  "with the flipped taps (the A/B and parity partner)"),
     "conv4_dgrad": ("TONAL_CONV4_DGRAD", frozenset({"nt63", "gemm"}), "nt63",
                     "F(6,3): the one-tap stage behind conv3 - nt63: its input gradient on the NT63 kernel, writing Y3 / Vd3 "
                     "(no gradient rows, no tl_wino63_unpool_yvd); gemm: one-tap GEMM + tl_wino63_unpool_yvd"),
diff --git a/decode_tonal_langauge_amd/_lib.py b/decode_tonal_langauge_amd/_lib.py
--- a/decode_tonal_langauge_amd/_lib.py
+++ b/decode_tonal_langauge_amd/_lib.py
@@ -9,6 +9,7 @@
 
 LOAD_DIRECT, LOAD_UNPOOL, LOAD_V = 0, 1, 2
 EPI_STORE, EPI_LRELU, EPI_POOL, EPI_MASK, EPI_C1WGRAD, EPI_POOLV, EPI_MASKY, EPI_GY = 0, 1, 2, 3, 4, 5, 6, 7
+EPI_C1WGRAD_Y, EPI_MASKY_ONLY = 8, 9
 LOAD_Y = 3
 
 
@@ -77,6 +78,7 @@
     "tl_wino43_unpool_transform": (_I, [_P, _P, _P, _L, _L, _I, _I, _I, _I, _I, _I, _P]),
     "tl_conv3_wino43v_tn": (_I, [C.POINTER(TnParams), _P]),
     "tl_wino63_weights": (_I, [_P, _P, _P, _I, _I, _I, _I, _P]),
+    "tl_wino63_weights_t": (_I, [_P, _P, _I, _I, _I, _P]),
     "tl_conv3_wino63v_nt": (_I, [C.POINTER(NtParams), _P]),
     "tl_wino63_nt_tile_rows": (_I, []),
     "tl_wino63_v_fixup": (_I, [_P, _P, _L, _L, _I, _I, _I, _P]),
diff --git a/decode_tonal_langauge_amd/csrc/tonal_wino43_epi.h b/decode_tonal_langauge_amd/csrc/tonal_wino43_epi.h
--- a/decode_tonal_langauge_amd/csrc/tonal_wino43_epi.h
+++ b/decode_tonal_langauge_amd/csrc/tonal_wino43_epi.h
@@ -4,7 +4,8 @@
 namespace tl {
 
 enum { W_LOAD_DIRECT = 0, W_LOAD_UNPOOL = 1, W_LOAD_V = 2 };
-enum { W_EPI_LRELU = 1, W_EPI_POOL = 2, W_EPI_MASK = 3, W_EPI_C1W = 4, W_EPI_POOLV = 5, W_EPI_MASKY = 6, W_EPI_GY = 7 };
+enum { W_EPI_LRELU = 1, W_EPI_POOL = 2, W_EPI_MASK = 3, W_EPI_C1W = 4, W_EPI_POOLV = 5, W_EPI_MASKY = 6, W_EPI_GY = 7,
+       W_EPI_C1WY = 8, W_EPI_MASKYO = 9 };
 
 struct c1w_acc {
   float s[3], b;
diff --git a/decode_tonal_langauge_amd/csrc/tonal_wino63.hip b/decode_tonal_langauge_amd/csrc/tonal_wino63.hip
--- a/decode_tonal_langauge_amd/csrc/tonal_wino63.hip
+++ b/decode_tonal_langauge_amd/csrc/tonal_wino63.hip
@@ -23,8 +23,8 @@
   return ((((hex >> 1) * kc8 + (c >> 3)) * 8 + i) * 2 + (hex & 1)) * 8 + (c & 7);
 }
 
-__global__ void wino63_weights_kernel(const float* __restrict__ w, float* __restrict__ fwd, float* __restrict__ dgr, int O,
-                                      int I, int ld_f, int ld_d) {
+__global__ void wino63_weights_kernel(const float* __restrict__ w, float* __restrict__ fwd, float* __restrict__ dgr,
+                                      float* __restrict__ dgt, int O, int I, int ld_f, int ld_d) {
   const long long n_f = (long long)O * ld_f, n_d = (long long)I * ld_d;
   const long long idx = (long long)blockIdx.x * blockDim.x + threadIdx.x;
   auto emit = [](float* dst, int R, int r, int k, float g0, float g1, float g2) {
@@ -59,6 +59,15 @@
       g0 = s[2], g1 = s[1], g2 = s[0];
     }
     emit(dgr, I, i, o, g0, g1, g2);
+  }
+  if (dgt != nullptr && idx < n_d) {
+    const int i = (int)(idx / ld_d), o = (int)(idx % ld_d);
+    float g0 = 0.f, g1 = 0.f, g2 = 0.f;
+    if (o < O) {
+      const float* s = w + ((long long)o * I + i) * 3;
+      g0 = s[0], g1 = s[1], g2 = s[2];
+    }
+    emit(dgt, I, i, o, g0, g1, g2);
   }
 }
 
@@ -213,7 +222,7 @@
 #endif
 template <int EPI>
 __global__ __launch_bounds__(512, 2) void wino63v_nt_kernel(const tl_nt_params p) {
-  __shared__ __attribute__((aligned(1024))) char lds[3 * V6_STAGE + ((EPI == W_EPI_POOLV || EPI == W_EPI_MASKY || EPI == W_EPI_GY) ? 4096 : EPI == W_EPI_C1W ? 16384 : 0)];
+  __shared__ __attribute__((aligned(1024))) char lds[3 * V6_STAGE + ((EPI == W_EPI_POOLV || EPI == W_EPI_MASKY || EPI == W_EPI_GY) ? 4096 : (EPI == W_EPI_C1W || EPI == W_EPI_C1WY) ? 16384 : 0)];
   const int tid = threadIdx.x;
   const int lane = tid & 63;
   const int wave = __builtin_amdgcn_readfirstlane(tid >> 6);
@@ -348,7 +357,7 @@
     const dma_src src_ = src_of(tl_, step);
     asm volatile(V6K_ISSUE : : V6K_INPUTS(src_, dst, 0) : "memory", "scc", "m0");
   };
-  constexpr bool early = V6_RDSCHED == 1 || (V6_RDSCHED < 0 && (EPI == W_EPI_POOLV || EPI == W_EPI_C1W));
+  constexpr bool early = V6_RDSCHED == 1 || (V6_RDSCHED < 0 && (EPI == W_EPI_POOLV || EPI == W_EPI_C1W || EPI == W_EPI_C1WY));
   constexpr int NST = v6_stores<EPI>();
   constexpr int first_n = NST + 6 > 63 ? 63 : NST + 6;
   constexpr int first_wait = (first_n & 15) | (7 << 4) | (0 << 8) | ((first_n >> 4) << 14);
@@ -367,8 +376,9 @@
     auto prefetch = [&] {
       if constexpr (EPI == W_EPI_POOL || EPI == W_EPI_POOLV || EPI == W_EPI_LRELU) return v5_prefetch_pool(p, cur.n0, wn, lr);
       else if constexpr (EPI == W_EPI_MASK) return v6_prefetch_mask(p, cur.R0, cur.n0, wm, wn, lr, lh);
-      else if constexpr (EPI == W_EPI_MASKY) return v6_prefetch_masky(p, cur.R0, cur.n0, wm, wn, lr, lh);
+      else if constexpr (EPI == W_EPI_MASKY || EPI == W_EPI_MASKYO) return v6_prefetch_masky(p, cur.R0, cur.n0, wm, wn, lr, lh);
       else if constexpr (EPI == W_EPI_GY) return v6_prefetch_masky<true>(p, cur.R0, cur.n0, wm, wn, lr, lh);
+      else if constexpr (EPI == W_EPI_C1WY) return v6_prefetch_c1wy(p, cur.R0, cur.n0, wm, wn, lr, lh);
       else return v6_prefetch_c1w(p, cur.R0, cur.n0, wm, wn, lr, lh);
     };
     decltype(prefetch()) pre;
@@ -447,6 +457,12 @@
       float* xch = reinterpret_cast<float*>(lds + 3 * V6_STAGE);
       if (full) v6_epilogue_masky<true>(p, acc, pre, xch, done.R0, done.n0, wm, wn, lr, lh, done.tm, est);
       else v6_epilogue_masky<false>(p, acc, pre, xch, done.R0, done.n0, wm, wn, lr, lh, done.tm, est);
+    } else if constexpr (EPI == W_EPI_MASKYO) {
+      if (full) v6_epilogue_masky<true, false, true>(p, acc, pre, nullptr, done.R0, done.n0, wm, wn, lr, lh, done.tm, est);
+      else v6_epilogue_masky<false, false, true>(p, acc, pre, nullptr, done.R0, done.n0, wm, wn, lr, lh, done.tm, est);
+    } else if constexpr (EPI == W_EPI_C1WY) {
+      v6_epilogue_c1wy(p, acc, pre, reinterpret_cast<float*>(lds + 3 * V6_STAGE) + wave * 512, scratch, done.R0, done.n0, wm, wn,
+                       lr, lh, done.tm);
     } else if constexpr (EPI == W_EPI_GY) {
       float* xch = reinterpret_cast<float*>(lds + 3 * V6_STAGE);
       if (full) v6_epilogue_masky<true, true>(p, acc, pre, xch, done.R0, done.n0, wm, wn, lr, lh, done.tm, est);
@@ -1628,9 +1644,21 @@
   const long long nf = (long long)O * ld_f, nd = (long long)I * ld_d;
   const long long n = nf > nd ? nf : nd;
   TL_REQUIRE((n + 255) / 256 < (1LL << 31), "wino63_weights: too large");
-  hipLaunchKernelGGL(wino63_weights_kernel, dim3((unsigned)((n + 255) / 256)), dim3(256), 0, (hipStream_t)stream, w, fwd, dgr, O,
-                     I, ld_f, ld_d);
+  hipLaunchKernelGGL(wino63_weights_kernel, dim3((unsigned)((n + 255) / 256)), dim3(256), 0, (hipStream_t)stream, w, fwd, dgr,
+                     (float*)nullptr, O, I, ld_f, ld_d);
   return check_launch("wino63_weights");
+}
+
+extern "C" int tl_wino63_weights_t(const float* w, float* dgt, int O, int I, int ld_d, void* stream) {
+  using namespace tl;
+  TL_REQUIRE(w != nullptr && dgt != nullptr, "wino63_weights_t: null pointer");
+  TL_REQUIRE(O > 0 && I > 0, "wino63_weights_t: bad sizes");
+  TL_REQUIRE(ld_d >= O && ld_d % 8 == 0, "wino63_weights_t: the leading dimension must cover the reduction length and be a multiple of 8");
+  const long long n = (long long)I * ld_d;
+  TL_REQUIRE((n + 255) / 256 < (1LL << 31), "wino63_weights_t: too large");
+  hipLaunchKernelGGL(wino63_weights_kernel, dim3((unsigned)((n + 255) / 256)), dim3(256), 0, (hipStream_t)stream, w, (float*)nullptr,
+                     (float*)nullptr, dgt, O, I, 0, ld_d);
+  return check_launch("wino63_weights_t");
 }
 
 extern "C" int tl_wino63_wgrad_finalize(const float* red, float* gw, int O, int I, int ld, void* stream) {
@@ -1736,7 +1764,8 @@
   using namespace tl;
   TL_REQUIRE(pp != nullptr, "wino63v_nt: null params");
   const tl_nt_params& p = *pp;
-  TL_REQUIRE(p.A && p.Bw && (p.out || p.epilogue == W_EPI_C1W || p.epilogue == W_EPI_POOLV || p.epilogue == W_EPI_MASKY), "wino63v_nt: null V/Bw/out");
+  TL_REQUIRE(p.A && p.Bw && (p.out || p.epilogue == W_EPI_C1W || p.epilogue == W_EPI_POOLV || p.epilogue == W_EPI_MASKY || p.epilogue == W_EPI_C1WY ||
+                             p.epilogue == W_EPI_MASKYO), "wino63v_nt: null V/Bw/out");
   TL_REQUIRE(p.loader == W_LOAD_V, "wino63v_nt: loader 2 (pre-transformed operand) only");
   TL_REQUIRE(p.J == 3 && p.splitk <= 1, "wino63v_nt: 3 taps, no split-K");
   TL_REQUIRE(p.M > 0 && p.M % 6 == 0 && p.N > 0 && p.K >= 40 && p.K % 8 == 0, "wino63v_nt: M %% 6, K %% 8, K >= 40 needed");
@@ -1780,11 +1809,23 @@
                "wino63v_nt: epilogue 6 needs vout / vout2 (>= M / 3 hexes, whole pairs, ld_vout %% 8 == 0) and vhalo");
     TL_REQUIRE(128LL * 8 * p.ld_vout * 4 < (1LL << 31), "wino63v_nt: ld_vout too large");
     hipLaunchKernelGGL((wino63v_nt_kernel<W_EPI_MASKY>), dim3((unsigned)ngrid), dim3(512), 0, st, p);
+  } else if (p.epilogue == W_EPI_MASKYO) {
+    TL_REQUIRE(p.row_shift == -2 && p.auxbits != nullptr && p.abits != nullptr, "wino63v_nt: epilogue 9 needs row_shift -2, auxbits and abits");
+    TL_REQUIRE(p.ld_abits * 32 >= p.N && p.Tvalid_in % 2 == 0 && p.Tvalid_in <= 2 * p.Tp, "wino63v_nt: epilogue 9: bad abits / Tvalid_in");
+    TL_REQUIRE(p.vout && p.ld_vout >= p.N && p.ld_vout % 8 == 0 && p.vout_quads >= p.M / 3 && p.vout_quads % 2 == 0,
+               "wino63v_nt: epilogue 9 needs vout (>= M / 3 hexes, whole pairs, ld_vout %% 8 == 0)");
+    TL_REQUIRE(128LL * 8 * p.ld_vout * 4 < (1LL << 31), "wino63v_nt: ld_vout too large");
+    hipLaunchKernelGGL((wino63v_nt_kernel<W_EPI_MASKYO>), dim3((unsigned)ngrid), dim3(512), 0, st, p);
   } else if (p.epilogue == W_EPI_C1W) {
     TL_REQUIRE(p.row_shift == -2, "wino63v_nt: input gradient needs row_shift -2");
     TL_REQUIRE(p.auxbits && p.c1x && p.c1bits && p.c1partial, "wino63v_nt: epilogue 4 needs auxbits, c1x, c1bits, c1partial");
     TL_REQUIRE(p.c1kt >= 1 && p.c1kt <= 3 && p.c1T >= 2 * p.Tvalid + 2, "wino63v_nt: epilogue 4: 1..3 taps, c1T >= 2*Tvalid + 2");
     hipLaunchKernelGGL((wino63v_nt_kernel<W_EPI_C1W>), dim3((unsigned)ngrid), dim3(512), 0, st, p);
+  } else if (p.epilogue == W_EPI_C1WY) {
+    TL_REQUIRE(p.row_shift == 0, "wino63v_nt: the input gradient on Y needs row_shift 0");
+    TL_REQUIRE(p.auxbits && p.c1x && p.c1bits && p.c1partial, "wino63v_nt: epilogue 8 needs auxbits, c1x, c1bits, c1partial");
+    TL_REQUIRE(p.c1kt >= 1 && p.c1kt <= 3 && p.c1T >= 2 * p.Tvalid + 2 && p.Tvalid <= p.Tp, "wino63v_nt: epilogue 8: 1..3 taps, c1T >= 2*Tvalid + 2, Tvalid <= Tp");
+    hipLaunchKernelGGL((wino63v_nt_kernel<W_EPI_C1WY>), dim3((unsigned)ngrid), dim3(512), 0, st, p);
   } else {
     set_error("wino63v_nt: unsupported epilogue %d", p.epilogue);
     return TL_EINVAL;
diff --git a/decode_tonal_langauge_amd/csrc/tonal_wino63_epi.h b/decode_tonal_langauge_amd/csrc/tonal_wino63_epi.h
--- a/decode_tonal_langauge_amd/csrc/tonal_wino63_epi.h
+++ b/decode_tonal_langauge_amd/csrc/tonal_wino63_epi.h
@@ -59,6 +59,18 @@
   y[3] = fmaf(0.125f, s56, fmaf(8.f, s34, s12));
   y[4] = fmaf(0.0625f, a56, fmaf(16.f, a34, a12));
   y[5] = fmaf(0.03125f, s56, fmaf(32.f, s34, s12)) + acc[7][e];
+}
+__device__ __forceinline__ void wino63_rows_t(const f32x16 (&acc)[8], int e, float (&r)[8]) {
+  const float m0 = acc[0][e], m1 = acc[1][e], m2 = acc[2][e], m3 = acc[3][e], m4 = acc[4][e], m5 = acc[5][e], m6 = acc[6][e], m7 = acc[7][e];
+  const float a12 = m1 + m2, s12 = m1 - m2, a34 = m3 + m4, s34 = m3 - m4, a56 = m5 + m6, s56 = m5 - m6;
+  r[0] = -m0;
+  r[1] = fmaf(2.f, s56, fmaf(0.5f, s34, s12)) - m7;
+  r[2] = fmaf(5.25f, m0, fmaf(4.f, a56, fmaf(0.25f, a34, a12)));
+  r[3] = fmaf(-4.25f, s12, fmaf(-2.5f, s34 + s56, 5.25f * m7));
+  r[4] = fmaf(-5.25f, m0, fmaf(-4.25f, a12, fmaf(-1.25f, a34, -5.f * a56)));
+  r[5] = fmaf(-5.25f, m7, fmaf(2.f, s34, fmaf(0.5f, s56, s12)));
+  r[6] = ((m0 + a12) + a34) + a56;
+  r[7] = m7;
 }
 __device__ __forceinline__ void wino63_bt(const float (&d)[8], float (&v)[8]) {
   v[0] = fmaf(5.25f, d[2] - d[4], d[6] - d[0]);
@@ -297,7 +309,7 @@
 
 template <int EPI>
 constexpr int v6_stores() {
-  return EPI == W_EPI_POOL ? 52 : EPI == W_EPI_POOLV ? 70 : (EPI == W_EPI_MASK || EPI == W_EPI_LRELU) ? 96 : (EPI == W_EPI_MASKY || EPI == W_EPI_GY) ? 63 : 0;
+  return EPI == W_EPI_POOL ? 52 : EPI == W_EPI_POOLV ? 70 : (EPI == W_EPI_MASK || EPI == W_EPI_LRELU) ? 96 : (EPI == W_EPI_MASKY || EPI == W_EPI_GY || EPI == W_EPI_MASKYO) ? 63 : 0;
 }
 
 struct v6_pre_mask {
@@ -405,7 +417,7 @@
   }
   return r;
 }
-template <bool FULL, bool DIRECT = false>
+template <bool FULL, bool DIRECT = false, bool YONLY = false>
 __device__ __forceinline__ void v6_epilogue_masky(const tl_nt_params& p, const f32x16 (&acc)[8], const v6_pre_masky& pre, float* xch,
                                                   long long R0, int n0, int wm, int wn, int lr_in, int lh, long long tm,
                                                   unsigned long long* st = nullptr) {
@@ -443,7 +455,8 @@
   const long long Hb = Rw / 3;
   const unsigned pair4 = (unsigned)p.ld_vout * 64u;
   const __amdgpu_buffer_rsrc_t rsY = rsrc_of(p.vout + Hb * 8 * (long long)p.ld_vout, (p.vout_quads - Hb) * 8 * (long long)p.ld_vout * 4);
-  const __amdgpu_buffer_rsrc_t rsD = rsrc_of(p.vout2 + Hb * 8 * (long long)p.ld_vout, (p.vout_quads - Hb) * 8 * (long long)p.ld_vout * 4);
+  const __amdgpu_buffer_rsrc_t rsD = rsrc_of(YONLY ? nullptr : p.vout2 + Hb * 8 * (long long)p.ld_vout,
+                                            YONLY ? 0 : (p.vout_quads - Hb) * 8 * (long long)p.ld_vout * 4);
   const unsigned offP = v6_pair_offset(colbase, lr, lh);
   const unsigned vvA = colok ? offP : V6_DROP, vvB = colok ? 16u * pair4 + offP : V6_DROP;
   const int nexA = (int)(p.M / 3 - Hb < 64 ? p.M / 3 - Hb : 64) - lh, nexB = nexA - 32;
@@ -492,36 +505,41 @@
       Yp[hh][5] = ev3 + od3;
       Yp[hh][6] = ev3 - od3;
       Yp[hh][7] = d6[5];
-      if (j == 0) {
-#pragma unroll
-        for (int k = 0; k < 6; ++k) first_d[k] = d6[k];
-      } else {
-        const uint32_t keep = ~(uint32_t)__builtin_amdgcn_sbfe((int)firstw, j, 1);
-        float d[8];
-        d[0] = andf(pe, keep);
-        d[1] = andf(po, keep);
-#pragma unroll
-        for (int k = 0; k < 6; ++k) d[2 + k] = d6[k];
-        wino63_bt(d, Vp[hh]);
-      }
-      pe = d6[4];
-      po = d6[5];
+      if constexpr (!YONLY) {
+        if (j == 0) {
+#pragma unroll
+          for (int k = 0; k < 6; ++k) first_d[k] = d6[k];
+        } else {
+          const uint32_t keep = ~(uint32_t)__builtin_amdgcn_sbfe((int)firstw, j, 1);
+          float d[8];
+          d[0] = andf(pe, keep);
+          d[1] = andf(po, keep);
+#pragma unroll
+          for (int k = 0; k < 6; ++k) d[2 + k] = d6[k];
+          wino63_bt(d, Vp[hh]);
+        }
+        pe = d6[4];
+        po = d6[5];
+      }
     }
     {
       const int j = 2 * e;
       const unsigned so = (unsigned)e * pair4;
       const unsigned voA = FULL ? vvA : (j < nexA ? vvA : V6_DROP), voB = FULL ? vvB : (j < nexB ? vvB : V6_DROP);
       v6_store_hex_pair<FULL>(Yp[0], Yp[1], rsY, voA, voA + 1024u, voB, voB + 1024u, so);
-      if (e == 0) {
-#pragma unroll
-        for (int i = 0; i < 8; ++i) v1keep[i] = Vp[1][i];
-      } else {
-        v6_store_hex_pair<FULL>(Vp[0], Vp[1], rsD, voA, voA + 1024u, voB, voB + 1024u, so);
+      if constexpr (!YONLY) {
+        if (e == 0) {
+#pragma unroll
+          for (int i = 0; i < 8; ++i) v1keep[i] = Vp[1][i];
+        } else {
+          v6_store_hex_pair<FULL>(Vp[0], Vp[1], rsD, voA, voA + 1024u, voB, voB + 1024u, so);
+        }
       }
     }
     __builtin_amdgcn_sched_barrier(0);
   }
   v6_stamp(st, 13);
+  if constexpr (YONLY) return;
   const int slot = wm * 2 + lh;
   {
     float2 v2 = {pe, po};
@@ -635,4 +653,117 @@
   c1w_reduce_store<4, 64>(p, red, ca, wm, wn * 32 + lr, lh, tm, col, colok);
 }
 
-}
+struct v6_pre_c1wy {
+  v6_pre_c1w b;
+  uint32_t s3, c3;
+  f32x4 x2;
+};
+__device__ __forceinline__ v6_pre_c1wy v6_prefetch_c1wy(const tl_nt_params& p, long long R0, int n0, int wm, int wn, int lr, int lh) {
+  v6_pre_c1wy r;
+  r.b = v6_prefetch_c1w(p, R0, n0, wm, wn, lr, lh);
+  const int colbase = n0 + wn * 32;
+  const long long rh = R0 + wm * 192 + 96 * lh;
+  r.s3 = r.c3 = 0u;
+  const long long rk = rh + 96 + lr;
+  if (colbase < p.N && lr < 2 && rk < p.M) {
+    r.s3 = p.auxbits[rk * (long long)p.ld_auxbits + (colbase >> 5)];
+    r.c3 = p.c1bits[rk * (long long)p.ld_auxbits + (colbase >> 5)];
+  }
+  const int Tp = p.Tp;
+  const long long nseq = p.M / Tp;
+  const unsigned s0 = (unsigned)(R0 / Tp);
+  const __amdgpu_buffer_rsrc_t rsX = rsrc_of(p.c1x + (long long)s0 * p.c1T, (nseq - s0) * (long long)p.c1T * 4);
+  typedef unsigned v4u __attribute__((ext_vector_type(4)));
+  const unsigned Rx = (unsigned)(rh + 3 * lr), sx = Rx / (unsigned)Tp, tx = Rx - sx * (unsigned)Tp;
+  const unsigned xo = ((sx - s0) * (unsigned)p.c1T + 2u * tx) * 4u;
+  r.x2 = __builtin_bit_cast(f32x4, (v4u)__builtin_amdgcn_raw_buffer_load_b128(rsX, xo + 32u, 0u, 0));
+  return r;
+}
+__device__ __forceinline__ void v6_epilogue_c1wy(const tl_nt_params& p, const f32x16 (&acc)[8], const v6_pre_c1wy& pre, float* xw,
+                                                 float* red, long long R0, int n0, int wm, int wn, int lr_in, int lh, long long tm) {
+  int lr = lr_in;
+  asm volatile("" : "+v"(lr));
+  const int colbase = n0 + wn * 32;
+  const bool colok = colbase < p.N;
+  const int col = colbase + lr;
+  const long long Hw = tm * 128 + wm * 32;
+  const long long Rw = 6 * Hw;
+  const int Tp = p.Tp;
+  const v6_rows rw = v6_rows_of(Hw, Tp);
+  const bits96 okA = v6_valid_bits96(rw.tA, Tp, p.Tvalid, Rw, p.M);
+  const bits96 okB = v6_valid_bits96(rw.tB, Tp, p.Tvalid, Rw + 96, p.M);
+  uint32_t lastw, spw;
+  {
+    uint32_t lA = 0, lB = 0;
+    int ta = rw.tA, tb = rw.tB;
+    for (int k = 0; k < 16; ++k) {
+      lA |= (uint32_t)(ta == Tp - 6) << k;
+      lB |= (uint32_t)(tb == Tp - 6) << k;
+      ta = ta + 6 >= Tp ? ta + 6 - Tp : ta + 6;
+      tb = tb + 6 >= Tp ? tb + 6 - Tp : tb + 6;
+    }
+    const uint32_t sA = (uint32_t)(ta != 0 && ta < p.Tvalid && Rw + 96 < p.M) | ((uint32_t)(ta != 0 && ta + 1 < p.Tvalid && Rw + 97 < p.M) << 1);
+    const uint32_t sB = (uint32_t)(tb != 0 && tb < p.Tvalid && Rw + 192 < p.M) | ((uint32_t)(tb != 0 && tb + 1 < p.Tvalid && Rw + 193 < p.M) << 1);
+    lastw = lh ? lB : lA;
+    spw = lh ? sB : sA;
+  }
+  float* xh = xw + lh * 256;
+  *reinterpret_cast<f32x4*>(xh + 8 * lr) = pre.b.x[0];
+  *reinterpret_cast<f32x4*>(xh + 8 * lr + 4) = pre.b.x[1];
+  c1w_acc ca;
+  ca.clear();
+  uint32_t sT[3], cT[3];
+#pragma unroll
+  for (int k = 0; k < 3; ++k) {
+    sT[k] = bit_transpose32(pre.b.s[k], lr);
+    cT[k] = bit_transpose32(pre.b.c[k], lr);
+  }
+  const int l0 = 32 * lh;
+  const uint32_t s96 = (uint32_t)__shfl((int)pre.s3, l0), s97 = (uint32_t)__shfl((int)pre.s3, l0 + 1);
+  const uint32_t c96 = (uint32_t)__shfl((int)pre.c3, l0), c97 = (uint32_t)__shfl((int)pre.c3, l0 + 1);
+  float xs[4];
+#pragma unroll
+  for (int k = 0; k < 4; ++k) xs[k] = __shfl(pre.x2[k], l0 + 31);
+  asm volatile("" ::: "memory");
+  auto andf = [](float x, uint32_t m) { return __uint_as_float(__float_as_uint(x) & m); };
+  auto contract = [&ca](float dz, uint32_t am, float x0, float x1, float x2, float x3) {
+    auto pick = [am](float a, float b) { return __uint_as_float((__float_as_uint(a) & am) | (__float_as_uint(b) & ~am)); };
+    ca.s[0] = fmaf(dz, pick(x1, x0), ca.s[0]);
+    ca.s[1] = fmaf(dz, pick(x2, x1), ca.s[1]);
+    ca.s[2] = fmaf(dz, pick(x3, x2), ca.s[2]);
+    ca.b += dz;
+  };
+  float c6 = 0.f, c7 = 0.f;
+#pragma unroll
+  for (int e = 0; e < 16; ++e) {
+    float y[8];
+    wino63_rows_t(acc, e, y);
+    if (e > 0) {
+      y[0] += c6;
+      y[1] += c7;
+    }
+    const uint32_t keep = ~(uint32_t)__builtin_amdgcn_sbfe((int)lastw, e, 1);
+    c6 = andf(y[6], keep);
+    c7 = andf(y[7], keep);
+#pragma unroll
+    for (int h = 0; h < 6; ++h) {
+      const int r = 6 * e + h;
+      const float2 xa = *reinterpret_cast<const float2*>(xh + 8 * (r / 3) + 2 * (r % 3));
+      const float2 xb = *reinterpret_cast<const float2*>(xh + 8 * (r / 3) + 2 * (r % 3) + 2);
+      const float dz = selm0(mask96(okA, okB, r), y[h] * selbit(sT[r >> 5], r & 31, 1.f, p.slope));
+      contract(dz, (uint32_t)__builtin_amdgcn_sbfe((int)cT[r >> 5], r & 31, 1), xa.x, xa.y, xb.x, xb.y);
+    }
+    __builtin_amdgcn_sched_barrier(0);
+  }
+  {
+    const float2 xa = *reinterpret_cast<const float2*>(xh + 8 * 31 + 6);
+    const float d96 = andf(c6 * selbit(s96, lr, 1.f, p.slope), (uint32_t)__builtin_amdgcn_sbfe((int)spw, 0, 1));
+    const float d97 = andf(c7 * selbit(s97, lr, 1.f, p.slope), (uint32_t)__builtin_amdgcn_sbfe((int)spw, 1, 1));
+    contract(d96, (uint32_t)__builtin_amdgcn_sbfe((int)c96, lr, 1), xa.x, xa.y, xs[0], xs[1]);
+    contract(d97, (uint32_t)__builtin_amdgcn_sbfe((int)c97, lr, 1), xs[0], xs[1], xs[2], xs[3]);
+  }
+  __syncthreads();
+  c1w_reduce_store<4, 64>(p, red, ca, wm, wn * 32 + lr, lh, tm, col, colok);
+}
+
+}
diff --git a/include/tonal_hip.h b/include/tonal_hip.h
--- a/include/tonal_hip.h
+++ b/include/tonal_hip.h
@@ -64,6 +64,7 @@
                                int Tvalid, int C, int ldg, int ld_bits, int ldv, void* stream);
 int tl_conv3_wino43v_tn(const tl_tn_params* p, void* stream);
 int tl_wino63_weights(const float* w, float* fwd, float* dgr, int O, int I, int ld_f, int ld_d, void* stream);
+int tl_wino63_weights_t(const float* w, float* dgt, int O, int I, int ld_d, void* stream);
 int tl_conv3_wino63v_nt(const tl_nt_params* p, void* stream);
 int tl_wino63_nt_tile_rows(void);
 int tl_wino63_v_fixup(float* V, const float* vhalo, int64_t hexes, int64_t tiles, int Tq, int C, int ldv, void* stream);
```
